# esq4/nind-denoise

Hardware: AMD Instinct MI355X
Metric: megapixels/sec denoised, UtNet cs=256 on 24 MP frames, 1/2/4/8 MI355X (higher is better)
Workload: dtype f32; 1 GPU; configs[1]: one 6000x4000 (24.0 MP) fp32 frame per step, f32 storage in the conv stack (fp32 accumulate), UtNet(funit=64,PReLU) random-init (seed 123), cs=264 (nearest valid to the named size; the reference rejects 256 / 512) ucs=200 ol=64 -> 1276 tiles/frame, tiles per conv-stack launch 256, crop->infer->stitch device resident (frame and canvas in HBM); every tile's input is the whole cs x cs cro; tiles_per_frame=1276, parallelism=single GPU

## Files before the change

### include/nind_hip.h

```cpp
#ifndef NIND_HIP_H
#define NIND_HIP_H

#include <stddef.h>
#include <stdint.h>

#ifdef __cplusplus
extern "C" {
#endif

typedef enum nd_status {
    ND_OK = 0,
    ND_EINVAL = -1,
    ND_ENOMEM = -2,
    ND_EHIP = -3
} nd_status;

typedef enum nd_act {
    ND_ACT_NONE = 0,
    ND_ACT_PRELU = 1,
    ND_ACT_ELU = 2,
    ND_ACT_HARDSWISH = 3
} nd_act;

typedef enum nd_layer_kind {
    ND_CONV3 = 0,
    ND_CONVT3 = 1,
    ND_CONVT2S2 = 2,
    ND_CONV1 = 3,
    ND_CONV2S2 = 4
} nd_layer_kind;

typedef enum nd_dtype {
    ND_F32 = 0,
    ND_BF16 = 1,
    ND_F16 = 2
} nd_dtype;

typedef enum nd_flags {
    ND_FLAG_NO_SPLITK = 1,
    ND_FLAG_DIRECT_CONV = 2,
    ND_FLAG_W1D_REGS = 4,
    ND_FLAG_UNFUSED_POOL = 16,
    ND_FLAG_TILE_ENCODER = 32,
    ND_FLAG_TILE_LEVEL2 = 64,
    ND_FLAG_FIND_NOISE = 128,
    ND_FLAG_TILE_SKIPS = 256,
    ND_FLAG_FULL_TILES = 8
} nd_flags;

int nd_version(void);
const char *nd_last_error(void);

int nd_tile_grid(int width, int height, int cs, int ucs, int ol, int *cols, int *rows, int *pad);
int nd_tile_geom(int i, int width, int height, int cs, int ucs, int ol,
                 int *x0, int *y0, int usefuldim[4], int usefulstart[2]);

int nd_tile_gather(const float *img_chw, int width, int height, int cs, int ucs, int ol,
                   int tile_begin, int tile_count, float *tiles_nchw, void *stream);
int nd_stitch_add(float *canvas_chw, int width, int height, int cs, int ucs, int ol,
                  const float *tiles_nchw, int tile_begin, int tile_count, void *stream);

int nd_utnet_num_tensors(void);
const char *nd_utnet_tensor_name(int idx);
size_t nd_utnet_packed_bytes(int funit, int dtype);
int nd_utnet_pack_weights(int funit, int dtype, const float *const *tensors, int n_tensors,
                          void *packed_host, size_t packed_bytes);

int nd_utnet_pack_weights_device(int funit, int dtype, const float *const *dev_tensors, int n_tensors, void *packed_dev,
                                 size_t packed_bytes, void *stream);

size_t nd_utnet_workspace_bytes_hw(int funit, int h, int w, int batch, int dtype);
int nd_utnet_workspace_init_hw(void *workspace, size_t workspace_bytes, int funit, int h, int w, int batch, int dtype,
                               void *stream);
int nd_utnet_forward_hw(int funit, int act, int dtype, int flags, const void *packed_dev,
                        const float *x_nchw, float *y_nchw, int batch, int h, int w,
                        void *workspace, size_t workspace_bytes, void *stream);

int nd_utnet_denoise_tiles(int funit, int act, int dtype, int flags, const void *packed_dev,
                           const float *img_chw, float *canvas_chw, int width, int height,
                           int cs, int ucs, int ol, int tile_begin, int tile_count, int batch,
                           void *workspace, size_t workspace_bytes, void *stream);

typedef void (*nd_progress_fn)(void *ctx, int n, int tile_begin, int tile_count);
size_t nd_utnet_frame_workspace_bytes(int funit, int dtype, int flags, int width, int height, int cs, int ucs, int ol, int batch);
int nd_utnet_denoise_frame(int funit, int act, int dtype, int flags, const void *packed_dev,
                           const float *img_chw, float *canvas_chw, int width, int height,
                           int cs, int ucs, int ol, int tile_begin, int tile_count, int batch,
                           void *workspace, size_t workspace_bytes, void *frame_ws, size_t frame_ws_bytes, void *stream,
                           nd_progress_fn progress, void *progress_ctx);
int nd_utnet_frame_plan(int funit, int dtype, int flags, int width, int height, int cs, int ucs, int ol, int *out);
int nd_utnet_frame_levels(int funit, int dtype, int flags, int width, int height, int cs, int ucs, int ol, int *levels);
int nd_utnet_frame_folds(int funit, int dtype, int flags, int width, int height, int cs, int ucs, int ol, int *mask);

typedef struct nd_step_profile {
    float ms;
    float ms_xform_in;
    float ms_gemm;
    float ms_xform_out;
    int form;
    int kind;
    double flops;
    double mfma_flops;
    double bytes;
    double xform_bytes_in;
    double xform_bytes_out;
} nd_step_profile;
int nd_utnet_profile_stack(int funit, int act, int dtype, int flags, const void *packed_dev, int batch, int cs, int crop,
                           void *workspace, size_t workspace_bytes, void *stream, nd_step_profile *steps, int max_steps);
const char *nd_utnet_step_name(int i);
int nd_utnet_useful_region(int funit, int cs, int crop, int step, int *rect);

int nd_unet_num_tensors(void);
const char *nd_unet_tensor_name(int idx);
size_t nd_unet_packed_bytes(int dtype);
int nd_unet_pack_weights(int dtype, const float *const *tensors, int n_tensors, void *packed_host, size_t packed_bytes);
size_t nd_unet_workspace_bytes(int h, int w, int batch, int dtype);
int nd_unet_workspace_init(void *workspace, size_t workspace_bytes, int h, int w, int batch, int dtype, void *stream);
int nd_unet_forward(int dtype, const void *packed_dev, const float *x_nchw, float *y_nchw, int batch, int h, int w,
                    void *workspace, size_t workspace_bytes, void *stream);

int nd_unet_pack_weights_device(int dtype, const float *const *dev_tensors, int n_tensors, void *packed_dev, size_t packed_bytes,
                                void *stream);

int nd_unet_num_steps(void);
const char *nd_unet_step_name(int i);
int nd_unet_useful_region(int cs, int crop, int step, int *rect);

int nd_unet_denoise_frame(int dtype, int flags, const void *packed_dev, const float *img_chw, float *canvas_chw, int width,
                          int height, int cs, int ucs, int ol, int tile_begin, int tile_count, int batch, void *workspace,
                          size_t workspace_bytes, void *stream, nd_progress_fn progress, void *progress_ctx);

double nd_utnet_flops(int funit, int cs);

size_t nd_layer_packed_bytes(int kind, int cin, int cout, int dtype);
int nd_layer_pack(int kind, int cin, int cout, int dtype, const float *weight, const float *bias,
                  void *packed_host, size_t packed_bytes);
size_t nd_layer_workspace_bytes(int kind, int batch, int cin, int cout, int h, int w, int dtype);
int nd_layer_forward(int kind, int act, float slope, int dtype, const void *packed_dev,
                     const float *x_nchw, int batch, int cin, int h, int w, int cout, float *y_nchw,
                     void *workspace, size_t workspace_bytes, int variant, int flags, void *stream);
int nd_maxpool2_forward(const float *x_nchw, int batch, int c, int h, int w, float *y_nchw,
                        void *workspace, size_t workspace_bytes, void *stream);

size_t nd_layer_wgrad_workspace_bytes(int kind, int batch, int cin, int cout, int h, int w);
int nd_layer_wgrad(int kind, const float *x_nchw, const float *dy_nchw, int batch, int cin, int h, int w, int cout,
                   float *dw, float *db, void *workspace, size_t workspace_bytes, void *stream);

size_t nd_utnet_param_count(int funit);
int nd_utnet_param_range(int funit, int tensor_idx, size_t *offset, size_t *count);
size_t nd_utnet_train_blob_bytes(int funit);
size_t nd_utnet_train_workspace_bytes_hw(int funit, int h, int w, int batch);
int nd_utnet_train_workspace_init_hw(void *workspace, size_t workspace_bytes, int funit, int h, int w, int batch, void *stream);
int nd_utnet_train_step_hw(int funit, int flags, const float *params, float *grads, void *blobs, const float *x_nchw,
                           const float *target_nchw, float *y_out_nchw, float w_l1, float w_mse, float w_ssim, float w_msssim,
                           float *loss_out, int batch, int h, int w, int loss_cs, void *workspace, size_t workspace_bytes,
                           void *stream, void *const *bucket_events, int n_events);
int nd_utnet_train_forward_hw(int funit, int act, int flags, const float *params, void *blobs, const float *x_nchw,
                              float *y_out_nchw, int batch, int h, int w, void *workspace, size_t workspace_bytes, void *stream);
int nd_utnet_train_backward_hw(int funit, int act, int flags, const float *params, float *grads, void *blobs, const float *gy_nchw,
                               float *dx_nchw, int batch, int h, int w, void *workspace, size_t workspace_bytes, void *stream,
                               void *const *bucket_events, int n_events);
int nd_utnet_grad_buckets(int funit, size_t *offsets, size_t *counts, int max);
int nd_adam_step(float *params, const float *grads, float *m, float *v, float *vmax, size_t n, float lr, float beta1,
                 float beta2, float eps, int step, int amsgrad, void *stream);

size_t nd_ssim_workspace_bytes(int n, int c, int h, int w);
int nd_ssim(const float *x, const float *y, int n, int c, int h, int w, float *out, void *workspace, size_t workspace_bytes,
            void *stream);
int nd_ms_ssim(const float *x, const float *y, int n, int c, int h, int w, float *out, void *workspace,
               size_t workspace_bytes, void *stream);
int nd_mse(const float *x, const float *y, size_t count, float *out, void *workspace, size_t workspace_bytes, void *stream);

size_t nd_ssim_loss_workspace_bytes(int n, int c, int h, int w);
int nd_ssim_loss_grad(const float *x, const float *y, int n, int c, int h, int w, int multiscale, float weight,
                      float *loss_acc, float *gx, int accumulate, void *workspace, size_t workspace_bytes, void *stream);

size_t nd_ssim_padded_workspace_bytes(int n, int c, int h, int w, int window);
int nd_ssim_padded(const float *x, const float *y, int n, int c, int h, int w, int window, float *out, void *workspace,
                   size_t workspace_bytes, void *stream);
int nd_ssim_padded_grad(const float *x, const float *y, int n, int c, int h, int w, int window, const float *gout, float *gx,
                        void *workspace, size_t workspace_bytes, void *stream);

size_t nd_winograd_packed_bytes(int tile, int cin, int cout);
int nd_winograd_pack(int tile, int kind, int cin, int cout, const float *w, const float *bias, void *packed,
                     size_t packed_bytes);
size_t nd_layer_winograd_workspace_bytes(int tile, int kind, int batch, int cin, int cout, int h, int w);
int nd_layer_forward_winograd(int tile, int kind, int act, float slope, const void *packed, const float *x, int batch,
                              int cin, int h, int w, int cout, float *y, void *workspace, size_t workspace_bytes, int flags,
                              void *stream);

int nd_conv_bench(int kind, int dtype, int batch, int cin, int cout, int h, int w, int variant, int iters,
                  void *workspace, size_t workspace_bytes, void *stream, float *mean_ms);

int nd_winograd_bench(int tile, int kind, int batch, int cin, int cout, int h, int w, int iters, void *workspace,
                      size_t workspace_bytes, void *stream, float *mean_ms);

int nd_num_conv_variants(void);
const char *nd_conv_variant_name(int variant);

#ifdef __cplusplus
}
#endif
#endif
```

### nind_denoise_amd/_lib.py

```python
import ctypes
import os
from ctypes import POINTER, c_char_p, c_double, c_float, c_int, c_size_t, c_void_p

_HERE = os.path.dirname(os.path.abspath(__file__))
LIB_PATH = os.path.join(_HERE, "libnind_hip.so")

ND_F32, ND_BF16, ND_F16 = 0, 1, 2
DTYPE = {"f32": 0, "fp32": 0, "float32": 0, "bf16": 1, "bfloat16": 1, "f16": 2, "fp16": 2, "float16": 2}
ACT = {"none": 0, "PReLU": 1, "ELU": 2, "Hardswish": 3}
KIND = {"conv3": 0, "convT3": 1, "convT2s2": 2, "conv1": 3, "conv2s2": 4}
FLAG_NO_SPLITK, FLAG_DIRECT_CONV, FLAG_W1D_REGS, FLAG_FULL_TILES, FLAG_UNFUSED_POOL, FLAG_TILE_ENCODER, FLAG_TILE_LEVEL2 = 1, 2, 4, 8, 16, 32, 64
FLAG_FIND_NOISE = 128
FLAG_TILE_SKIPS = 256
PROGRESS_FN = ctypes.CFUNCTYPE(None, c_void_p, c_int, c_int, c_int)


class StepProfile(ctypes.Structure):
    _fields_ = [("ms", c_float), ("ms_xform_in", c_float), ("ms_gemm", c_float), ("ms_xform_out", c_float),
                ("form", c_int), ("kind", c_int), ("flops", c_double), ("mfma_flops", c_double), ("bytes", c_double),
                ("xform_bytes_in", c_double), ("xform_bytes_out", c_double)]


FORM_NAMES = {-1: "pool", 0: "direct", 1: "w1d_f43", 2: "w1d_f23", 3: "wino3p_f6x6"}


class NindHipError(RuntimeError):
    pass


class NindHipMissing(ImportError):
    pass


_lib = None

_SIGNATURES = {
    "nd_version": (c_int, []),
    "nd_last_error": (c_char_p, []),
    "nd_tile_grid": (c_int, [c_int] * 5 + [POINTER(c_int)] * 3),
    "nd_tile_geom": (c_int, [c_int] * 6 + [POINTER(c_int)] * 4),
    "nd_tile_gather": (c_int, [c_void_p] + [c_int] * 7 + [c_void_p, c_void_p]),
    "nd_stitch_add": (c_int, [c_void_p] + [c_int] * 5 + [c_void_p, c_int, c_int, c_void_p]),
    "nd_utnet_num_tensors": (c_int, []),
    "nd_utnet_tensor_name": (c_char_p, [c_int]),
    "nd_utnet_packed_bytes": (c_size_t, [c_int, c_int]),
    "nd_utnet_pack_weights": (c_int, [c_int, c_int, POINTER(c_void_p), c_int, c_void_p, c_size_t]),
    "nd_utnet_pack_weights_device": (c_int, [c_int, c_int, POINTER(c_void_p), c_int, c_void_p, c_size_t, c_void_p]),
    "nd_utnet_workspace_bytes_hw": (c_size_t, [c_int] * 5),
    "nd_utnet_workspace_init_hw": (c_int, [c_void_p, c_size_t] + [c_int] * 5 + [c_void_p]),
    "nd_utnet_forward_hw": (c_int, [c_int] * 4 + [c_void_p] * 3 + [c_int, c_int, c_int, c_void_p, c_size_t, c_void_p]),
    "nd_utnet_denoise_tiles": (c_int, [c_int] * 4 + [c_void_p] * 3 + [c_int] * 8 + [c_void_p, c_size_t, c_void_p]),
    "nd_unet_num_tensors": (c_int, []),
    "nd_unet_tensor_name": (c_char_p, [c_int]),
    "nd_unet_packed_bytes": (c_size_t, [c_int]),
    "nd_unet_pack_weights": (c_int, [c_int, POINTER(c_void_p), c_int, c_void_p, c_size_t]),
    "nd_unet_workspace_bytes": (c_size_t, [c_int] * 4),
    "nd_unet_workspace_init": (c_int, [c_void_p, c_size_t] + [c_int] * 4 + [c_void_p]),
    "nd_unet_forward": (c_int, [c_int, c_void_p, c_void_p, c_void_p, c_int, c_int, c_int, c_void_p, c_size_t, c_void_p]),
    "nd_unet_pack_weights_device": (c_int, [c_int, POINTER(c_void_p), c_int, c_void_p, c_size_t, c_void_p]),
    "nd_unet_num_steps": (c_int, []),
    "nd_unet_step_name": (c_char_p, [c_int]),
    "nd_unet_useful_region": (c_int, [c_int, c_int, c_int, POINTER(c_int)]),
    "nd_unet_denoise_frame": (c_int, [c_int, c_int] + [c_void_p] * 3 + [c_int] * 8 + [c_void_p, c_size_t, c_void_p, PROGRESS_FN, c_void_p]),
    "nd_utnet_flops": (c_double, [c_int, c_int]),
    "nd_utnet_profile_stack": (c_int, [c_int] * 4 + [c_void_p, c_int, c_int, c_int, c_void_p, c_size_t, c_void_p, c_void_p, c_int]),
    "nd_utnet_step_name": (c_char_p, [c_int]),
    "nd_utnet_useful_region": (c_int, [c_int, c_int, c_int, c_int, POINTER(c_int)]),
    "nd_utnet_frame_workspace_bytes": (c_size_t, [c_int] * 9),
    "nd_utnet_frame_plan": (c_int, [c_int] * 8 + [POINTER(c_int)]),
    "nd_utnet_frame_levels": (c_int, [c_int] * 8 + [POINTER(c_int)]),
    "nd_utnet_frame_folds": (c_int, [c_int] * 8 + [POINTER(c_int)]),
    "nd_utnet_denoise_frame": (c_int, [c_int] * 4 + [c_void_p] * 3 + [c_int] * 8 + [c_void_p, c_size_t, c_void_p, c_size_t, c_void_p,
                                                                                    PROGRESS_FN, c_void_p]),
    "nd_layer_packed_bytes": (c_size_t, [c_int] * 4),
    "nd_layer_pack": (c_int, [c_int] * 4 + [c_void_p, c_void_p, c_void_p, c_size_t]),
    "nd_layer_workspace_bytes": (c_size_t, [c_int] * 7),
    "nd_layer_forward": (c_int, [c_int, c_int, c_float, c_int, c_void_p, c_void_p] + [c_int] * 5
                         + [c_void_p, c_void_p, c_size_t, c_int, c_int, c_void_p]),
    "nd_winograd_packed_bytes": (c_size_t, [c_int] * 3),
    "nd_winograd_pack": (c_int, [c_int] * 4 + [c_void_p, c_void_p, c_void_p, c_size_t]),
    "nd_layer_winograd_workspace_bytes": (c_size_t, [c_int] * 7),
    "nd_layer_forward_winograd": (c_int, [c_int, c_int, c_int, c_float, c_void_p, c_void_p] + [c_int] * 5
                                  + [c_void_p, c_void_p, c_size_t, c_int, c_void_p]),
    "nd_maxpool2_forward": (c_int, [c_void_p] + [c_int] * 4 + [c_void_p, c_void_p, c_size_t, c_void_p]),
    "nd_layer_wgrad_workspace_bytes": (c_size_t, [c_int] * 6),
    "nd_layer_wgrad": (c_int, [c_int, c_void_p, c_void_p] + [c_int] * 5 + [c_void_p, c_void_p, c_void_p, c_size_t, c_void_p]),
    "nd_utnet_param_count": (c_size_t, [c_int]),
    "nd_utnet_param_range": (c_int, [c_int, c_int, POINTER(c_size_t), POINTER(c_size_t)]),
    "nd_utnet_train_blob_bytes": (c_size_t, [c_int]),
    "nd_utnet_grad_buckets": (c_int, [c_int, POINTER(c_size_t), POINTER(c_size_t), c_int]),
    "nd_utnet_train_workspace_bytes_hw": (c_size_t, [c_int] * 4),
    "nd_utnet_train_workspace_init_hw": (c_int, [c_void_p, c_size_t, c_int, c_int, c_int, c_int, c_void_p]),
    "nd_utnet_train_forward_hw": (c_int, [c_int, c_int, c_int, c_void_p, c_void_p, c_void_p, c_void_p, c_int, c_int, c_int, c_void_p,
                                          c_size_t, c_void_p]),
    "nd_utnet_train_backward_hw": (c_int, [c_int, c_int, c_int, c_void_p, c_void_p, c_void_p, c_void_p, c_void_p, c_int, c_int, c_int,
                                           c_void_p, c_size_t, c_void_p, POINTER(c_void_p), c_int]),
    "nd_utnet_train_step_hw": (c_int, [c_int, c_int, c_void_p, c_void_p, c_void_p, c_void_p, c_void_p, c_void_p, c_float, c_float,
                                       c_float, c_float, c_void_p, c_int, c_int, c_int, c_int, c_void_p, c_size_t, c_void_p,
                                       POINTER(c_void_p), c_int]),
    "nd_adam_step": (c_int, [c_void_p] * 5 + [c_size_t, c_float, c_float, c_float, c_float, c_int, c_int, c_void_p]),
    "nd_ssim_workspace_bytes": (c_size_t, [c_int] * 4),
    "nd_ssim": (c_int, [c_void_p, c_void_p] + [c_int] * 4 + [c_void_p, c_void_p, c_size_t, c_void_p]),
    "nd_ms_ssim": (c_int, [c_void_p, c_void_p] + [c_int] * 4 + [c_void_p, c_void_p, c_size_t, c_void_p]),
    "nd_ssim_loss_workspace_bytes": (c_size_t, [c_int] * 4),
    "nd_ssim_loss_grad": (c_int, [c_void_p, c_void_p] + [c_int] * 5 + [c_float, c_void_p, c_void_p, c_int, c_void_p, c_size_t,
                                  c_void_p]),
    "nd_ssim_padded_workspace_bytes": (c_size_t, [c_int] * 5),
    "nd_ssim_padded": (c_int, [c_void_p, c_void_p] + [c_int] * 5 + [c_void_p, c_void_p, c_size_t, c_void_p]),
    "nd_ssim_padded_grad": (c_int, [c_void_p, c_void_p] + [c_int] * 5 + [c_void_p, c_void_p, c_void_p, c_size_t, c_void_p]),
    "nd_mse": (c_int, [c_void_p, c_void_p, c_size_t, c_void_p, c_void_p, c_size_t, c_void_p]),
    "nd_conv_bench": (c_int, [c_int] * 9 + [c_void_p, c_size_t, c_void_p, POINTER(c_float)]),
    "nd_winograd_bench": (c_int, [c_int] * 8 + [c_void_p, c_size_t, c_void_p, POINTER(c_float)]),
    "nd_num_conv_variants": (c_int, []),
    "nd_conv_variant_name": (c_char_p, [c_int]),
}

EXPORTS = tuple(_SIGNATURES)


def load():
    global _lib
    if _lib is not None:
        return _lib
    if not os.path.isfile(LIB_PATH):
        raise NindHipMissing(
            f"{LIB_PATH} not found: build it with `make -C nind_denoise_amd/csrc` (or __graft_entry__.build()). "
            "nind_denoise_amd has no CPU fallback for the denoise hot path.")
    import torch
    lib = ctypes.CDLL(LIB_PATH)
    for name, (res, args) in _SIGNATURES.items():
        fn = getattr(lib, name)
        fn.restype = res
        fn.argtypes = args
    _lib = lib
    return lib


def check(rc, what=""):
    if rc != 0:
        msg = load().nd_last_error().decode(errors="replace")
        exc = ValueError if rc == -1 else (MemoryError if rc == -2 else NindHipError)
        raise exc(f"{what}: {msg}" if what else msg)


def stream_ptr(device=None):
    import torch
    return c_void_p(torch.cuda.current_stream(device).cuda_stream)


def ptr(t):
    assert t.is_contiguous(), "tensor must be contiguous"
    return c_void_p(t.data_ptr())



def tile_grid(width, height, cs, ucs, ol):
    cols, rows, pad = c_int(), c_int(), c_int()
    check(load().nd_tile_grid(width, height, cs, ucs, ol, cols, rows, pad), "nd_tile_grid")
    return cols.value, rows.value, pad.value


def tile_geom(i, width, height, cs, ucs, ol):
    x0, y0 = c_int(), c_int()
    ud = (c_int * 4)()
    us = (c_int * 2)()
    check(load().nd_tile_geom(i, width, height, cs, ucs, ol, x0, y0, ud, us), "nd_tile_geom")
    return x0.value, y0.value, tuple(ud), tuple(us)


def utnet_tensor_names():
    lib = load()
    return [lib.nd_utnet_tensor_name(i).decode() for i in range(lib.nd_utnet_num_tensors())]
```

### nind_denoise_amd/csrc/nd_common.h

```cpp
#pragma once
#include <hip/hip_runtime.h>

#include <stdarg.h>
#include <stdint.h>
#include <stdio.h>

#include "nind_hip.h"

void nd_set_error(const char *fmt, ...);
#define ND_FAIL(code, ...)        \
    do {                          \
        nd_set_error(__VA_ARGS__); \
        return (code);            \
    } while (0)
#define ND_HIP(call)                                                                         \
    do {                                                                                     \
        hipError_t e_ = (call);                                                              \
        if (e_ != hipSuccess) ND_FAIL(ND_EHIP, "%s failed: %s", #call, hipGetErrorString(e_)); \
    } while (0)
#define ND_TRY(call)        \
    do {                    \
        int r_ = (call);    \
        if (r_ != 0) return r_; \
    } while (0)

static inline int nd_cpp(int dt) { return dt == ND_F32 ? 4 : 8; }
struct QpBuf {
    float *base;
    int planes;
    int B, Hb, Wb;
    int pad;
    long pstride;
    int dt = ND_F32;
    long np() const { return pstride; }
    long used() const { return (long)B * Hb * Wb; }
};

struct ConvDesc {
    int kind = ND_CONV3;
    int act = ND_ACT_NONE;
    float slope = 1.f;
    const float *slope_dev = nullptr;
    const float *wpk = nullptr;
    const float *bias = nullptr;
    int cin = 0, cout = 0;
    QpBuf in = {};
    QpBuf out = {};
    int out_plane0 = 0;
    int variant = -1;
    int in_plane0 = 0;
    float *pre = nullptr;
    long pre_plane = 0;
    float *part = nullptr;
    size_t part_bytes = 0;
    bool nosplit = false;
    int nbatch = 1;
    long in_bs = 0, out_bs = 0;
    size_t w_bs = 0;
    const QpBuf *pool = nullptr;
    int roi_r0 = 0, roi_c0 = 0, roi_rows = 0, roi_cols = 0;
    QpBuf in2 = {};
    int in2_plane0 = 0, in2_from = 0;
    const int *in2_origin = nullptr;
    long in2_origin_max = 0;
    int w_kb = 0, w_kb0 = 0;
    QpBuf add = {};
    int add_plane0 = 0;
    const int *add_origin = nullptr;
    long add_origin_max = 0;
};
int nd_check_in2(const char *who, const ConvDesc &d, int KB, long reach);
int nd_check_add(const char *who, const ConvDesc &d, long reach);
static const size_t kSplitScratchBytes = (size_t)512 * 64 * 1024 * 4;
int nd_launch_conv(const ConvDesc &d, hipStream_t stream);
bool nd_conv_pool_fits(const ConvDesc &d);
bool nd_conv_roi_fits(const ConvDesc &d);
int nd_conv_variant_count();
int nd_conv_variant_gemm(int cin, int cout);
size_t nd_wino_packed_floats(int T, int cin, int cout);
int nd_wino_pack(int T, int kind, int cin, int cout, const float *w, const float *bias, float *packed);
size_t nd_wino_scratch_bytes(int T, const QpBuf &in, int cin, int cout);
int nd_launch_conv_wino(int T, const ConvDesc &d, void *scratch, size_t scratch_bytes, hipStream_t s, hipEvent_t *ev2 = nullptr);
void nd_wino_xform_bytes(int T, const QpBuf &in, int cin, int cout, double *bytes_in, double *bytes_out);
size_t nd_w1d_packed_floats(int T, int cin, int cout);
int nd_w1d_pack(int T, int kind, int cin, int cout, const float *w, const float *bias, float *packed);
bool nd_w1d_fits(int T, const QpBuf &in);
int nd_launch_conv_w1d(int T, const ConvDesc &d, hipStream_t stream);
bool nd_w2d_ok(const QpBuf &in);
long nd_w2d_tiles(const QpBuf &in, int cout);
int nd_launch_conv_w2d(const ConvDesc &d, hipStream_t stream);
bool nd_f43_w2d(const QpBuf &in, int cout, bool pre, int flags);
int nd_launch_conv_f43(const ConvDesc &d, int flags, hipStream_t stream);
static inline size_t nd_buf_slack(int Wb) { return (size_t)10 * Wb + 8 + 2048; }
int nd_device(int *dev, int *ncus = nullptr);
int nd_raise_lds(int dev, const void *fn, size_t bytes);
int nd_once_per_device(int dev, int (*init)());
int nd_check_in_planes(const char *who, const ConvDesc &d, int KB, bool takes_in2 = false, bool takes_add = false);
int nd_check_out(const char *who, const ConvDesc &d, int oh, int ow, bool at_least);
int nd_check_int32(const char *who, const QpBuf &in);
int nd_check_roi(const char *who, const ConvDesc &d, int Hv, int Wv, bool refused, const char *why);
static inline int nd_check_flags(int flags, bool frame_loop = false, bool unet_frame = false) {
    const int known = ND_FLAG_NO_SPLITK | ND_FLAG_DIRECT_CONV | ND_FLAG_W1D_REGS | ND_FLAG_FULL_TILES | ND_FLAG_UNFUSED_POOL |
                      ND_FLAG_TILE_ENCODER | (frame_loop ? ND_FLAG_TILE_LEVEL2 | ND_FLAG_TILE_SKIPS : 0) | (unet_frame ? ND_FLAG_FIND_NOISE : 0);
    if (flags & ~known) ND_FAIL(ND_EINVAL, "unknown flag bits 0x%x", flags);
    return ND_OK;
}
const char *nd_conv_variant_label(int v);

static inline int nd_mtiles(int kind, int cout) {
    return kind == ND_CONVT2S2 ? (4 * cout + 255) / 256 * 8 : (cout + 127) / 128 * 4;
}
struct NdUpRow { int a, b, co; };
__host__ __device__ static inline NdUpRow nd_up_row(int m, int cout, int dt) {
    NdUpRow r;
    const int cpp = dt == ND_F32 ? 4 : 8, q = cout / cpp;
    const int G = m / (2 * cpp), e = m % cpp;
    r.b = (m / cpp) & 1;
    r.a = G / q;
    r.co = cpp * (G % q) + e;
    return r;
}
static inline int nd_taps(int kind) { return (kind == ND_CONV3 || kind == ND_CONVT3) ? 9 : (kind == ND_CONV2S2 ? 4 : 1); }
static inline int nd_kblocks(int cin, int dt = ND_F32) { return (cin + 2 * nd_cpp(dt) - 1) / (2 * nd_cpp(dt)); }
static inline size_t nd_bias_offset(int kind, int cin, int cout, int dt = ND_F32, int w1d_T = 0) {
    return (size_t)nd_mtiles(kind, cout) * nd_kblocks(cin, dt) * (w1d_T ? 3 * (w1d_T + 2) : nd_taps(kind)) * 256;
}
static inline size_t nd_packed_floats(int kind, int cin, int cout, int dt = ND_F32) {
    return nd_bias_offset(kind, cin, cout, dt) + (size_t)nd_mtiles(kind, cout) * 32;
}
void nd_pack_layer(int kind, int cin, int cout, int dt, const float *w, const float *bias, float *packed);

int nd_pack_layer_device(int kind, int cin, int cout, int dt, const float *w, const float *bias, float *packed, hipStream_t s,
                         const float *scale = nullptr);
int nd_launch_bn_fold(int cout, const float *b, const float *g, const float *be, const float *rm, const float *rv, float *scale,
                      float *fbias, hipStream_t s);
int nd_pack_w1d_device(int T, int kind, int cin, int cout, const float *w, const float *bias, float *packed, hipStream_t s);
int nd_pack_wino_device(int T, int kind, int cin, int cout, const float *w, const float *bias, float *packed, hipStream_t s);

int nd_launch_nchw_to_qp(const float *x, int C, const QpBuf &dst, int plane0, hipStream_t s);
int nd_launch_qp_to_nchw(const QpBuf &src, int plane0, float *y, int C, hipStream_t s);
int nd_launch_reflect_pack(const float *x_nchw, int B, int H, int W, const QpBuf &dst, hipStream_t s);
int nd_launch_maxpool2(const QpBuf &src, int src_plane0, int planes, const QpBuf &dst, hipStream_t s);
int nd_launch_final1x1(const QpBuf &src, int cin, const float *w, const float *bias, int crop, float *y_nchw, int H,
                       int W, hipStream_t s, int sigmoid = 0);
int nd_launch_final1x1_stitch(const QpBuf &src, int cin, const float *w, const float *bias, int crop, float *canvas,
                              int width, int height, int cs, int ucs, int ol, int tile_begin, int tile_count,
                              hipStream_t s, int sigmoid = 0, const float *noise_img = nullptr);
int nd_launch_gather_pack(const float *img, int width, int height, int cs, int ucs, int ol, int tile_begin,
                          int tile_count, const QpBuf &dst, hipStream_t s, int border = 2, bool reflect = true);
int nd_launch_gather_band(const float *img, int width, int height, int cs, int ucs, int ol, int band_row0, const QpBuf &dst,
                          hipStream_t s);
enum nd_edge_set { ND_EDGE_ROWS = 0, ND_EDGE_COLS = 1, ND_EDGE_CORNERS = 2 };
int nd_launch_gather_edges(const float *img, int width, int height, int cs, int ucs, int ol, int set, int first, int count,
                           const QpBuf &dst, hipStream_t s);
int nd_launch_skip_origins(const QpBuf &src, int dst_pad, int tile_begin, int tile_count, int cols, int band_rows, int step, long slot_elems,
                           int *table, long *origin_max, hipStream_t s);
struct SpliceMap {
    int step_y = 0, step_x = 0, img_t = 0, img_y = 0, img_x = 0, img_add = 0, oy = 0, ox = 0;
};
int nd_launch_splice(const QpBuf &src, int src_p0, const QpBuf &dst, int dst_p0, int planes, int tile_begin, int tile_count, int cols,
                     int row0, const SpliceMap &m, int r0, int r1, int c0, int c1, hipStream_t s, int band_rows = 0,
                     long slot_elems = 0, int dst_img0 = 0);
```

### nind_denoise_amd/csrc/pack.hip

```cpp
#include <string.h>

#include "nd_common.h"

static thread_local char g_err[512] = "";

void nd_set_error(const char *fmt, ...) {
    va_list ap;
    va_start(ap, fmt);
    vsnprintf(g_err, sizeof(g_err), fmt, ap);
    va_end(ap);
}

extern "C" const char *nd_last_error(void) { return g_err; }
extern "C" int nd_version(void) { return 111; }

static inline uint16_t f32_to_bf16_rne(float f) {
    uint32_t u;
    memcpy(&u, &f, 4);
    if ((u & 0x7fffffffu) > 0x7f800000u) return (uint16_t)((u >> 16) | 0x40);
    return (uint16_t)((u + 0x7fffu + ((u >> 16) & 1u)) >> 16);
}
static inline uint16_t f32_to_f16_rne(float f) {
    const _Float16 h = (_Float16)f;
    uint16_t u;
    memcpy(&u, &h, 2);
    return u;
}

void nd_pack_layer(int kind, int cin, int cout, int dt, const float *w, const float *bias, float *packed) {
    const int taps = nd_taps(kind);
    const int KB = nd_kblocks(cin, dt);
    const int MT = nd_mtiles(kind, cout);
    const int M = kind == ND_CONVT2S2 ? 4 * cout : cout;
    const int cpp = nd_cpp(dt);
    float *bp = packed + nd_bias_offset(kind, cin, cout, dt);
    auto weff = [&](int m, int ci, int t) -> float {
        if (m >= M || ci >= cin) return 0.f;
        switch (kind) {
            case ND_CONV3: return w[((size_t)m * cin + ci) * 9 + t];
            case ND_CONVT3: return w[((size_t)ci * cout + m) * 9 + (8 - t)];
            case ND_CONVT2S2: {
                const NdUpRow r = nd_up_row(m, cout, dt);
                return w[((size_t)ci * cout + r.co) * 4 + 2 * r.a + r.b];
            }
            case ND_CONV2S2: return w[((size_t)m * cin + ci) * 4 + t];
            default: return w[(size_t)m * cin + ci];
        }
    };
    for (int mt = 0; mt < MT; ++mt)
        for (int kb = 0; kb < KB; ++kb)
            for (int t = 0; t < taps; ++t) {
                float *dst = packed + (((size_t)mt * KB + kb) * taps + t) * 256;
                uint16_t *dst16 = (uint16_t *)dst;
                for (int lane = 0; lane < 64; ++lane) {
                    const int i = lane & 31, h = lane >> 5;
                    const int m = 32 * mt + i;
                    for (int s = 0; s < cpp; ++s) {
                        const float v = weff(m, 2 * cpp * kb + cpp * h + s, t);
                        if (dt == ND_F32)
                            dst[lane * 4 + s] = v;
                        else
                            dst16[lane * 8 + s] = dt == ND_BF16 ? f32_to_bf16_rne(v) : f32_to_f16_rne(v);
                    }
                }
            }
    for (int m = 0; m < MT * 32; ++m) {
        float v = 0.f;
        if (m < M && bias) v = bias[kind == ND_CONVT2S2 ? nd_up_row(m, cout, dt).co : m];
        bp[m] = v;
    }
}

extern "C" size_t nd_layer_packed_bytes(int kind, int cin, int cout, int dtype) {
    if (dtype < ND_F32 || dtype > ND_F16 || kind < 0 || kind > 4 || cin <= 0 || cout <= 0) return 0;
    return nd_packed_floats(kind, cin, cout, dtype) * sizeof(float);
}

extern "C" int nd_layer_pack(int kind, int cin, int cout, int dtype, const float *weight, const float *bias,
                             void *packed_host, size_t packed_bytes) {
    if (dtype < ND_F32 || dtype > ND_F16) ND_FAIL(ND_EINVAL, "nd_layer_pack: unsupported dtype %d", dtype);
    if (kind < 0 || kind > 4 || cin <= 0 || cout <= 0 || !weight || !packed_host)
        ND_FAIL(ND_EINVAL, "nd_layer_pack: bad arguments");
    if (packed_bytes < nd_layer_packed_bytes(kind, cin, cout, dtype))
        ND_FAIL(ND_ENOMEM, "nd_layer_pack: packed buffer too small");
    nd_pack_layer(kind, cin, cout, dtype, weight, bias, (float *)packed_host);
    return ND_OK;
}
```

### nind_denoise_amd/csrc/utnet.hip

```cpp
#include <string.h>

#include <string>
#include <vector>

#include "nd_common.h"

#include "utnet_net.h"

extern "C" int nd_utnet_num_tensors(void) { return (int)tensor_names().size(); }
extern "C" const char *nd_utnet_tensor_name(int idx) {
    const auto &n = tensor_names();
    return (idx >= 0 && idx < (int)n.size()) ? n[idx].c_str() : nullptr;
}

extern "C" size_t nd_utnet_packed_bytes(int funit, int dtype) {
    if (check_funit(funit, dtype) != ND_OK) return 0;
    return blob_layout(funit, dtype).total * sizeof(float);
}

extern "C" int nd_utnet_pack_weights(int funit, int dtype, const float *const *tensors, int n_tensors, void *packed_host,
                                     size_t packed_bytes) {
    ND_TRY(check_funit(funit, dtype));
    if (n_tensors != nd_utnet_num_tensors()) ND_FAIL(ND_EINVAL, "nd_utnet_pack_weights: expected %d tensors, got %d", nd_utnet_num_tensors(), n_tensors);
    const BlobLayout bl = blob_layout(funit, dtype);
    if (packed_bytes < bl.total * sizeof(float)) ND_FAIL(ND_ENOMEM, "nd_utnet_pack_weights: packed buffer too small");
    float *blob = (float *)packed_host;
    memset(blob, 0, bl.total * sizeof(float));
    for (int i = 0; i < kNumLayers; ++i) {
        const LayerSpec &l = kLayers[i];
        const int wi = tensor_index(std::string(l.key) + ".weight"), bi = tensor_index(std::string(l.key) + ".bias");
        if (wi < 0 || bi < 0 || !tensors[wi] || !tensors[bi]) ND_FAIL(ND_EINVAL, "nd_utnet_pack_weights: missing tensor %s.{weight,bias}", l.key);
        const int ci = lcin(l, funit), co = lcout(l, funit);
        if (i == kNumLayers - 1) {
            memcpy(blob + bl.off[i], tensors[wi], sizeof(float) * 3 * ci);
            memcpy(blob + bl.off[i] + 3 * ci, tensors[bi], sizeof(float) * 3);
        } else {
            nd_pack_layer(l.kind, ci, co, dtype, tensors[wi], tensors[bi], blob + bl.off[i]);
            if (bl.woff[i]) ND_TRY(nd_wino_pack(kWinoTile, l.kind, ci, co, tensors[wi], tensors[bi], blob + bl.woff[i]));
            if (bl.w1off[i]) ND_TRY(nd_w1d_pack(kW1dTile, l.kind, ci, co, tensors[wi], tensors[bi], blob + bl.w1off[i]));
            if (bl.w1off2[i]) ND_TRY(nd_w1d_pack(2, l.kind, ci, co, tensors[wi], tensors[bi], blob + bl.w1off2[i]));
        }
        if (l.prelu >= 0) {
            std::string k(l.key);
            const size_t dot = k.rfind('.');
            const std::string an = k.substr(0, dot + 1) + std::to_string(atoi(k.c_str() + dot + 1) + 1) + ".weight";
            const int ai = tensor_index(an);
            blob[l.prelu] = (ai >= 0 && tensors[ai]) ? tensors[ai][0] : 0.25f;
        }
    }
    return ND_OK;
}

extern "C" int nd_utnet_pack_weights_device(int funit, int dtype, const float *const *tensors, int n_tensors, void *packed_dev,
                                            size_t packed_bytes, void *stream) {
    ND_TRY(check_funit(funit, dtype));
    if (n_tensors != nd_utnet_num_tensors()) ND_FAIL(ND_EINVAL, "nd_utnet_pack_weights_device: expected %d tensors, got %d", nd_utnet_num_tensors(), n_tensors);
    const BlobLayout bl = blob_layout(funit, dtype);
    if (!packed_dev || packed_bytes < bl.total * sizeof(float)) ND_FAIL(ND_ENOMEM, "nd_utnet_pack_weights_device: packed buffer too small");
    hipStream_t s = (hipStream_t)stream;
    float *blob = (float *)packed_dev;
    ND_HIP(hipMemsetAsync(blob, 0, bl.total * sizeof(float), s));
    for (int i = 0; i < kNumLayers; ++i) {
        const LayerSpec &l = kLayers[i];
        const int wi = tensor_index(std::string(l.key) + ".weight"), bi = tensor_index(std::string(l.key) + ".bias");
        if (wi < 0 || bi < 0 || !tensors[wi] || !tensors[bi]) ND_FAIL(ND_EINVAL, "nd_utnet_pack_weights_device: missing tensor %s.{weight,bias}", l.key);
        const int ci = lcin(l, funit), co = lcout(l, funit);
        if (i == kNumLayers - 1) {
            ND_HIP(hipMemcpyAsync(blob + bl.off[i], tensors[wi], sizeof(float) * 3 * ci, hipMemcpyDeviceToDevice, s));
            ND_HIP(hipMemcpyAsync(blob + bl.off[i] + 3 * ci, tensors[bi], sizeof(float) * 3, hipMemcpyDeviceToDevice, s));
        } else {
            ND_TRY(nd_pack_layer_device(l.kind, ci, co, dtype, tensors[wi], tensors[bi], blob + bl.off[i], s));
            if (bl.woff[i]) ND_TRY(nd_pack_wino_device(kWinoTile, l.kind, ci, co, tensors[wi], tensors[bi], blob + bl.woff[i], s));
            if (bl.w1off[i]) ND_TRY(nd_pack_w1d_device(kW1dTile, l.kind, ci, co, tensors[wi], tensors[bi], blob + bl.w1off[i], s));
            if (bl.w1off2[i]) ND_TRY(nd_pack_w1d_device(2, l.kind, ci, co, tensors[wi], tensors[bi], blob + bl.w1off2[i], s));
        }
        if (l.prelu >= 0) {
            std::string k(l.key);
            const size_t dot = k.rfind('.');
            const std::string an = k.substr(0, dot + 1) + std::to_string(atoi(k.c_str() + dot + 1) + 1) + ".weight";
            const int ai = tensor_index(an);
            if (ai >= 0 && tensors[ai]) {
                ND_HIP(hipMemcpyAsync(blob + l.prelu, tensors[ai], sizeof(float), hipMemcpyDeviceToDevice, s));
            } else {
                const float dflt = 0.25f;
                ND_HIP(hipMemcpyAsync(blob + l.prelu, &dflt, sizeof(float), hipMemcpyHostToDevice, s));
                ND_HIP(hipStreamSynchronize(s));
            }
        }
    }
    return ND_OK;
}

extern "C" size_t nd_utnet_workspace_bytes_hw(int funit, int h, int w, int batch, int dtype) {
    if (check_net(funit, h, w, batch, dtype) != ND_OK) return 0;
    return make_plan(funit, h, w, batch, batch, nullptr, dtype).bytes;
}

extern "C" int nd_utnet_workspace_init_hw(void *ws, size_t ws_bytes, int funit, int h, int w, int batch, int dtype,
                                          void *stream) {
    ND_TRY(check_net(funit, h, w, batch, dtype));
    const size_t need = make_plan(funit, h, w, batch, batch, nullptr, dtype).bytes;
    if (!ws || ws_bytes < need) ND_FAIL(ND_ENOMEM, "UtNet workspace: %zu B given, %zu B needed", ws_bytes, need);
    ND_HIP(hipMemsetAsync(ws, 0, need, (hipStream_t)stream));
    return ND_OK;
}

static int forward_common(int funit, int act, int dtype, const void *packed, int batch_cap, int nimg, int h, int w,
                          void *ws, size_t ws_bytes, Plan *out_plan) {
    ND_TRY(check_net(funit, h, w, batch_cap, dtype));
    if (act < ND_ACT_PRELU || act > ND_ACT_HARDSWISH) ND_FAIL(ND_EINVAL, "UtNet: unknown activation %d", act);
    if (nimg <= 0 || nimg > batch_cap) ND_FAIL(ND_EINVAL, "UtNet: %d images with a workspace batch of %d", nimg, batch_cap);
    if (!packed || !ws) ND_FAIL(ND_EINVAL, "UtNet: null pointer");
    if (((uintptr_t)ws & 15) || ((uintptr_t)packed & 15)) ND_FAIL(ND_EINVAL, "UtNet: workspace / weights must be 16-byte aligned");
    *out_plan = make_plan(funit, h, w, batch_cap, nimg, (char *)ws, dtype);
    if (ws_bytes < out_plan->bytes) ND_FAIL(ND_ENOMEM, "UtNet workspace: %zu B given, %zu B needed", ws_bytes, out_plan->bytes);
    return ND_OK;
}

extern "C" int nd_utnet_forward_hw(int funit, int act, int dtype, int flags, const void *packed, const float *x, float *y,
                                   int batch, int h, int w, void *ws, size_t ws_bytes, void *stream) {
    ND_TRY(nd_check_flags(flags));
    Plan pl;
    ND_TRY(forward_common(funit, act, dtype, packed, batch, batch, h, w, ws, ws_bytes, &pl));
    if (!x || !y) ND_FAIL(ND_EINVAL, "UtNet: null tensor");
    hipStream_t s = (hipStream_t)stream;
    const float *blob = (const float *)packed;
    ND_TRY(nd_launch_reflect_pack(x, batch, h, w, pl.buf[X0], s));
    StackOpts o;
    o.flags = flags;
    ND_TRY(run_stack(funit, act, dtype, blob, pl, s, o));
    const BlobLayout bl = blob_layout(funit, dtype);
    const float *fw = blob + bl.off[kNumLayers - 1];
    ND_TRY(nd_launch_final1x1(pl.buf[T4B], funit, fw, fw + 3 * funit, 2, y, h, w, s));
    return ND_OK;
}

extern "C" int nd_utnet_denoise_tiles(int funit, int act, int dtype, int flags, const void *packed, const float *img,
                                      float *canvas, int width, int height, int cs, int ucs, int ol, int tile_begin,
                                      int tile_count, int batch, void *ws, size_t ws_bytes, void *stream) {
    ND_TRY(nd_check_flags(flags));
    Plan pl;
    ND_TRY(forward_common(funit, act, dtype, packed, batch, tile_count, cs, cs, ws, ws_bytes, &pl));
    if (!img || !canvas) ND_FAIL(ND_EINVAL, "UtNet: null image");
    hipStream_t s = (hipStream_t)stream;
    const float *blob = (const float *)packed;
    ND_TRY(nd_launch_gather_pack(img, width, height, cs, ucs, ol, tile_begin, tile_count, pl.buf[X0], s));
    const BlobLayout bl = blob_layout(funit, dtype);
    Roi rois[kNumSteps];
    StackOpts o;
    o.flags = flags;
    const int crop = (cs - ucs) / 2;
    if (!(flags & ND_FLAG_FULL_TILES) && plan_rois(pl, crop, crop, rois) && rois_supported(funit, dtype, flags, pl, bl, rois)) o.rois = rois;
    ND_TRY(run_stack(funit, act, dtype, blob, pl, s, o));
    const float *fw = blob + bl.off[kNumLayers - 1];
    ND_TRY(nd_launch_final1x1_stitch(pl.buf[T4B], funit, fw, fw + 3 * funit, 2, canvas, width, height, cs, ucs, ol,
                                     tile_begin, tile_count, s));
    return ND_OK;
}

extern "C" size_t nd_utnet_frame_workspace_bytes(int funit, int dtype, int flags, int width, int height, int cs, int ucs, int ol,
                                                 int batch) {
    FramePlan fp;
    if (nd_check_flags(flags, true) != ND_OK || frame_plan(funit, dtype, flags, width, height, cs, ucs, ol, batch, &fp) != ND_OK) return 0;
    return fp.bytes;
}

extern "C" int nd_utnet_frame_plan(int funit, int dtype, int flags, int width, int height, int cs, int ucs, int ol, int *out) {
    ND_TRY(nd_check_flags(flags, true));
    if (!out) ND_FAIL(ND_EINVAL, "nd_utnet_frame_plan: null output");
    FramePlan fp;
    ND_TRY(frame_plan(funit, dtype, flags, width, height, cs, ucs, ol, 1, &fp));
    const int v[8] = {fp.D, fp.aligned, fp.R, fp.nbands, fp.S, fp.cols, fp.rows, fp.hx};
    memcpy(out, v, sizeof(v));
    return ND_OK;
}

extern "C" int nd_utnet_frame_levels(int funit, int dtype, int flags, int width, int height, int cs, int ucs, int ol, int *levels) {
    ND_TRY(nd_check_flags(flags, true));
    if (!levels) ND_FAIL(ND_EINVAL, "nd_utnet_frame_levels: null output");
    FramePlan fp;
    ND_TRY(frame_plan(funit, dtype, flags, width, height, cs, ucs, ol, 1, &fp));
    *levels = fp.levels;
    return ND_OK;
}

extern "C" int nd_utnet_frame_folds(int funit, int dtype, int flags, int width, int height, int cs, int ucs, int ol, int *mask) {
    ND_TRY(nd_check_flags(flags, true));
    if (!mask) ND_FAIL(ND_EINVAL, "nd_utnet_frame_folds: null output");
    FramePlan fp;
    ND_TRY(frame_plan(funit, dtype, flags, width, height, cs, ucs, ol, 1, &fp));
    *mask = fp.folds;
    return ND_OK;
}

extern "C" int nd_utnet_denoise_frame(int funit, int act, int dtype, int flags, const void *packed, const float *img, float *canvas,
                                      int width, int height, int cs, int ucs, int ol, int tile_begin, int tile_count, int batch,
                                      void *ws, size_t ws_bytes, void *fws, size_t fws_bytes, void *stream, nd_progress_fn progress,
                                      void *progress_ctx) {
    ND_TRY(nd_check_flags(flags, true));
    FramePlan fp;
    ND_TRY(frame_plan(funit, dtype, flags, width, height, cs, ucs, ol, batch, &fp));
    if (tile_begin < 0 || tile_count < 0 || tile_begin + tile_count > fp.cols * fp.rows)
        ND_FAIL(ND_EINVAL, "nd_utnet_denoise_frame: tiles [%d,+%d) outside the grid of %d", tile_begin, tile_count, fp.cols * fp.rows);
    const int end = tile_begin + tile_count;
    Plan pl;
    ND_TRY(forward_common(funit, act, dtype, packed, batch, batch, cs, cs, ws, ws_bytes, &pl));
    const BlobLayout bl = blob_layout(funit, dtype);
    Roi rois[kNumSteps];
    const int crop = (cs - ucs) / 2;
    if (fp.D && !(plan_rois(pl, crop, crop, rois) && rois_supported(funit, dtype, flags, pl, bl, rois))) fp.D = 0;
    if (fp.D == 0) {
        int n = 0;
        for (int t0 = tile_begin; t0 < end; t0 += batch, ++n) {
            const int cnt = end - t0 < batch ? end - t0 : batch;
            if (progress) progress(progress_ctx, n, t0, cnt);
            ND_TRY(nd_utnet_denoise_tiles(funit, act, dtype, flags & ~(ND_FLAG_TILE_LEVEL2 | ND_FLAG_TILE_SKIPS), packed, img, canvas, width, height, cs, ucs, ol, t0, cnt, batch, ws,
                                          ws_bytes, stream));
        }
        return ND_OK;
    }
    if (!img || !canvas) ND_FAIL(ND_EINVAL, "UtNet: null image");
    if (!fws || fws_bytes < fp.bytes || ((uintptr_t)fws & 255))
        ND_FAIL(ND_ENOMEM, "nd_utnet_denoise_frame: frame workspace %zu B given, %zu B needed (256-byte aligned)", fws_bytes, fp.bytes);
    hipStream_t s = (hipStream_t)stream;
    const float *blob = (const float *)packed;
    const float *fw = blob + bl.off[kNumLayers - 1];
    char *const band_base = (char *)fws, *const rows_base = band_base + fp.band_bytes, *const cols_base = rows_base + fp.row_edge_bytes;
    char *const corner_base = cols_base + fp.col_edge_bytes;
    int *const origins = (int *)(corner_base + fp.corner_bytes);
    const bool l2 = fp.levels == 3;
    char *const l2_band_base = (char *)origins + 3 * fp.origin_bytes, *const l2_rows_base = l2_band_base + fp.l2_band_bytes;
    char *const l2_cols_base = l2_rows_base + fp.l2_row_bytes, *const l2_corner_base = l2_cols_base + fp.l2_col_bytes;
    char *const l2_wino = l2_corner_base + fp.l2_corner_bytes;
    const int f4 = funit / 4, cols = fp.cols, S = fp.S;
    const int n2 = enc_extent(cs + 4, P2), n3 = l2_extent(n2, P3);
    StackOpts enc, enc2, dec;
    enc.flags = enc2.flags = dec.flags = flags;
    enc.step_end = enc2.step_begin = kSharedSteps;
    enc2.step_end = kLevel2End;
    dec.step_begin = l2 ? kLevel2End : kSharedSteps;
    dec.rois = rois;
    auto l2_scratch = [&](Plan p) {
        p.split = pl.split;
        p.wino = l2_wino;
        p.wino_bytes = fp.l2_wino_bytes;
        return p;
    };
    struct Skip { Buf cat; int planes, step, tstep; const int *win; int *table; bool in_place, fold; Form form; } skips[3] = {
        {CAT4, f4, -1, S, fp.win4, origins, false, false, FORM_DIRECT},
        {CAT3, 2 * f4, -1, S / 2, fp.win3, origins + fp.origin_bytes / sizeof(int), false, false, FORM_DIRECT},
        {CAT2, 4 * f4, -1, S / 4, fp.win2, origins + 2 * fp.origin_bytes / sizeof(int), false, false, FORM_DIRECT}};
    char *const fold_wino = (char *)fws + fp.bytes - fp.fold_wino_bytes;
    const int nskips = l2 ? 3 : 2;
    for (int ki = 0; ki < 3; ++ki)
        for (int i = kSharedSteps; i < kNumSteps; ++i) {
            Skip &k = skips[ki];
            if (kSteps[i].layer >= 0 && kSteps[i].src == k.cat) {
                const Form form = step_form(kSteps[i], funit, dtype, flags, pl, bl);
                k.step = i;
                k.in_place = form_takes_src2(kSteps[i], form, funit, flags, pl);
                k.form = form;
                k.fold = ki < nskips && ((fp.folds >> ki) & 1) && k.in_place;
            }
        }
    StepSrc2 src2[3];
    dec.src2 = src2;
    const int per_band = fp.R * cols;
    const Plan bf = make_enc_plan(funit, fp.hx, fp.wx, 1, fp.hx, fp.wx, 1, band_base, dtype, fp.slots);
    const Plan bf2 = l2 ? l2_band_plan(fp, funit, dtype, fp.R, cs, l2_band_base) : Plan();
    int band_done = tile_begin / per_band - 1;
    for (int t0 = tile_begin, n = 0; t0 < end; ++n) {
        const int b0 = t0 / per_band;
        int cnt = end - t0 < batch ? end - t0 : batch;
        if (t0 + cnt > (b0 + 2) * per_band) cnt = (b0 + 2) * per_band - t0;
        for (int b = band_done + 1; b <= (t0 + cnt - 1) / per_band; ++b) {
            const int row0 = b * fp.R, nrows = fp.rows - row0 < fp.R ? fp.rows - row0 : fp.R;
            Plan bp = band_slot(make_enc_plan(funit, band_hx(fp, nrows, cs), fp.wx, 1, fp.hx, fp.wx, 1, band_base, dtype, fp.slots), b & 1, fp.slots);
            bp.split = pl.split;
            ND_TRY(nd_launch_gather_band(img, width, height, cs, ucs, ol, row0, bp.buf[X0], s));
            ND_TRY(run_stack(funit, act, dtype, blob, bp, s, enc));
            for (int ki = 0; ki < 2; ++ki)
                if (skips[ki].fold)
                    ND_TRY(launch_skip_fold(funit, flags, blob, bl, skips[ki].step, skips[ki].form, bp.buf[skips[ki].cat], skips[ki].planes,
                                            rois[skips[ki].step], skips[ki].tstep, nrows, cols, pl.split, fold_wino, fp.fold_wino_bytes, s));
            Plan re = band_slot(row_edge_plan(fp, funit, dtype, nrows, rows_base), b & 1, fp.slots, P2);
            Plan ce = band_slot(col_edge_plan(fp, funit, dtype, nrows, cs, cols_base), b & 1, fp.slots, P2);
            re.split = ce.split = pl.split;
            ND_TRY(nd_launch_gather_edges(img, width, height, cs, ucs, ol, ND_EDGE_ROWS, row0, nrows, re.buf[X0], s));
            ND_TRY(nd_launch_gather_edges(img, width, height, cs, ucs, ol, ND_EDGE_COLS, row0, nrows, ce.buf[X0], s));
            ND_TRY(run_stack(funit, act, dtype, blob, re, s, enc));
            ND_TRY(run_stack(funit, act, dtype, blob, ce, s, enc));
            if (l2) {
                Plan b2 = l2_scratch(l2_slot(l2_band_plan(fp, funit, dtype, nrows, cs, l2_band_base), b & 1, fp.slots));
                b2.buf[P2] = bp.buf[P2];
                ND_TRY(run_stack(funit, act, dtype, blob, b2, s, enc2));
                if (skips[2].fold)
                    ND_TRY(launch_skip_fold(funit, flags, blob, bl, skips[2].step, skips[2].form, b2.buf[CAT2], skips[2].planes, rois[skips[2].step],
                                            skips[2].tstep, nrows, cols, pl.split, fold_wino, fp.fold_wino_bytes, s));
                const Plan r2 = l2_scratch(l2_slot(l2_row_plan(fp, funit, dtype, nrows, l2_rows_base), b & 1, fp.slots, P3));
                const Plan c2 = l2_scratch(l2_slot(l2_col_plan(fp, funit, dtype, nrows, cs, l2_cols_base), b & 1, fp.slots, P3));
                const int h2 = bp.buf[P2].Hb, w2 = bp.buf[P2].Wb;
                for (int side = 0; side < 2; ++side) {
                    const int at = side * (kStrip2 - 1), in0 = 1 - side, in1 = kStrip2 - side;
                    SpliceMap br, lr, bc, lc;
                    br.step_y = bc.step_x = S / 4;
                    br.oy = bc.ox = side * (n2 - kStrip2);
                    lr.img_y = lc.img_x = 2;
                    lr.img_add = lc.img_add = side;
                    lr.oy = lc.ox = -at;
                    ND_TRY(nd_launch_splice(bp.buf[P2], 0, r2.buf[P2], 0, 2 * f4, 0, nrows, 1, 0, br, in0, in1, 0, w2, s, 0, 0, side * nrows));
                    ND_TRY(nd_launch_splice(re.buf[P2], 0, r2.buf[P2], 0, 2 * f4, 0, nrows, 1, 0, lr, at, at + 1, 0, w2, s, 0, 0, side * nrows));
                    ND_TRY(nd_launch_splice(bp.buf[P2], 0, c2.buf[P2], 0, 2 * f4, 0, cols, cols, 0, bc, 0, h2, in0, in1, s, 0, 0, side * cols));
                    ND_TRY(nd_launch_splice(ce.buf[P2], 0, c2.buf[P2], 0, 2 * f4, 0, cols, cols, 0, lc, 0, h2, at, at + 1, s, 0, 0, side * cols));
                }
                ND_TRY(run_stack(funit, act, dtype, blob, r2, s, enc2));
                ND_TRY(run_stack(funit, act, dtype, blob, c2, s, enc2));
            }
            band_done = b;
        }
        if (progress) progress(progress_ctx, n, t0, cnt);
        Plan cp = corner_plan(funit, dtype, cnt, batch, corner_base);
        cp.split = pl.split;
        ND_TRY(nd_launch_gather_edges(img, width, height, cs, ucs, ol, ND_EDGE_CORNERS, t0, cnt, cp.buf[X0], s));
        ND_TRY(run_stack(funit, act, dtype, blob, cp, s, enc));
        const Plan tp = make_plan(funit, cs, cs, batch, cnt, (char *)ws, dtype);
        dec.nsrc2 = 0;
        for (int ki = 0; ki < nskips; ++ki) {
            const Skip &k = skips[ki];
            const QpBuf &src = k.cat == CAT2 ? bf2.buf[k.cat] : bf.buf[k.cat];
            if (!k.in_place && !k.fold) {
                SpliceMap m;
                m.step_y = m.step_x = k.tstep;
                ND_TRY(nd_launch_splice(src, k.planes, tp.buf[k.cat], k.planes, k.planes, t0, cnt, cols, 0, m, k.win[0], k.win[1], k.win[0],
                                        k.win[1], s, fp.R, slot_elems(src, fp.slots)));
                continue;
            }
            StepSrc2 &q = src2[dec.nsrc2++];
            q.step = k.step;
            q.buf = src;
            q.plane0 = q.from = k.planes;
            q.addend = k.fold;
            if (k.fold) {
                q.plane0 = 0;
                q.buf.pad = 1;
            }
            q.origin = k.table;
            ND_TRY(nd_launch_skip_origins(src, tp.buf[k.cat].pad, t0, cnt, cols, fp.R, k.tstep, slot_elems(src, fp.slots), k.table,
                                          &q.origin_max, s));
        }
        SpliceMap whole;
        whole.step_y = whole.step_x = S / 4;
        ND_TRY(nd_launch_splice(bf.buf[P2], 0, tp.buf[P2], 0, 2 * f4, t0, cnt, cols, 0, whole, 0, n2, 0, n2, s, fp.R,
                                slot_elems(bf.buf[P2], fp.slots)));
        for (int b = b0; b <= (t0 + cnt - 1) / per_band; ++b) {
            const int lo = t0 > b * per_band ? t0 : b * per_band, hi = t0 + cnt < (b + 1) * per_band ? t0 + cnt : (b + 1) * per_band;
            const int row0 = b * fp.R, nrows = fp.rows - row0 < fp.R ? fp.rows - row0 : fp.R;
            const QpBuf rl = band_slot(row_edge_plan(fp, funit, dtype, nrows, rows_base), b & 1, fp.slots, P2).buf[P2];
            const QpBuf cl = band_slot(col_edge_plan(fp, funit, dtype, nrows, cs, cols_base), b & 1, fp.slots, P2).buf[P2];
            for (int side = 0; side < 2; ++side) {
                const int at = side * (n2 - 1);
                SpliceMap mr, mc;
                mr.step_x = mc.step_y = S / 4;
                mr.img_y = mc.img_x = 2;
                mr.img_add = mc.img_add = side;
                mr.oy = mc.ox = -at;
                ND_TRY(nd_launch_splice(rl, 0, tp.buf[P2], 0, 2 * f4, lo, hi - lo, cols, row0, mr, at, at + 1, 0, n2, s, 0, 0, lo - t0));
                ND_TRY(nd_launch_splice(cl, 0, tp.buf[P2], 0, 2 * f4, lo, hi - lo, cols, row0, mc, 0, n2, at, at + 1, s, 0, 0, lo - t0));
            }
        }
        for (int k = 0; k < 4; ++k) {
            const int r = (k >> 1) * (n2 - 1), c = (k & 1) * (n2 - 1);
            SpliceMap m;
            m.img_t = 4;
            m.img_add = k;
            m.oy = -r;
            m.ox = -c;
            ND_TRY(nd_launch_splice(cp.buf[P2], 0, tp.buf[P2], 0, 2 * f4, t0, cnt, cols, 0, m, r, r + 1, c, c + 1, s));
        }
        if (l2) {
            const Plan k2 = l2_scratch(l2_corner_plan(funit, dtype, cnt, batch, l2_corner_base));
            for (int k = 0; k < 4; ++k) {
                SpliceMap m;
                m.img_t = 1;
                m.oy = (k >> 1) * (n2 - kStrip2);
                m.ox = (k & 1) * (n2 - kStrip2);
                ND_TRY(nd_launch_splice(tp.buf[P2], 0, k2.buf[P2], 0, 2 * f4, 0, cnt, cnt, 0, m, 0, kStrip2, 0, kStrip2, s, 0, 0, k * cnt));
            }
            ND_TRY(run_stack(funit, act, dtype, blob, k2, s, enc2));
            SpliceMap whole3;
            whole3.step_y = whole3.step_x = S / 8;
            ND_TRY(nd_launch_splice(bf2.buf[P3], 0, tp.buf[P3], 0, 4 * f4, t0, cnt, cols, 0, whole3, 0, n3, 0, n3, s, fp.R,
                                    slot_elems(bf2.buf[P3], fp.slots)));
            for (int b = b0; b <= (t0 + cnt - 1) / per_band; ++b) {
                const int lo = t0 > b * per_band ? t0 : b * per_band, hi = t0 + cnt < (b + 1) * per_band ? t0 + cnt : (b + 1) * per_band;
                const int row0 = b * fp.R, nrows = fp.rows - row0 < fp.R ? fp.rows - row0 : fp.R;
                const QpBuf rl = l2_slot(l2_row_plan(fp, funit, dtype, nrows, l2_rows_base), b & 1, fp.slots, P3).buf[P3];
                const QpBuf cl = l2_slot(l2_col_plan(fp, funit, dtype, nrows, cs, l2_cols_base), b & 1, fp.slots, P3).buf[P3];
                for (int side = 0; side < 2; ++side) {
                    const int at = side * (n3 - 1);
                    SpliceMap mr, mc;
                    mr.step_x = mc.step_y = S / 8;
                    mr.img_y = mc.img_x = 1;
                    mr.img_add = side * nrows;
                    mc.img_add = side * cols;
                    mr.oy = mc.ox = -at;
                    ND_TRY(nd_launch_splice(rl, 0, tp.buf[P3], 0, 4 * f4, lo, hi - lo, cols, row0, mr, at, at + 1, 0, n3, s, 0, 0, lo - t0));
                    ND_TRY(nd_launch_splice(cl, 0, tp.buf[P3], 0, 4 * f4, lo, hi - lo, cols, row0, mc, 0, n3, at, at + 1, s, 0, 0, lo - t0));
                }
            }
            for (int k = 0; k < 4; ++k) {
                const int r = (k >> 1) * (n3 - 1), c = (k & 1) * (n3 - 1);
                SpliceMap m;
                m.img_t = 1;
                m.img_add = k * cnt;
                m.oy = -r;
                m.ox = -c;
                ND_TRY(nd_launch_splice(k2.buf[P3], 0, tp.buf[P3], 0, 4 * f4, t0, cnt, cols, 0, m, r, r + 1, c, c + 1, s));
            }
        }
        ND_TRY(run_stack(funit, act, dtype, blob, tp, s, dec));
        ND_TRY(nd_launch_final1x1_stitch(tp.buf[T4B], funit, fw, fw + 3 * funit, 2, canvas, width, height, cs, ucs, ol, t0, cnt, s));
        t0 += cnt;
    }
    return ND_OK;
}

namespace {
template <int N>
struct Events {
    hipEvent_t ev[N];
    int n = 0;
    int create() {
        for (; n < N; ++n) ND_HIP(hipEventCreate(&ev[n]));
        return ND_OK;
    }
    ~Events() { for (int i = 0; i < n; ++i) (void)hipEventDestroy(ev[i]); }
};
}

extern "C" int nd_utnet_profile_stack(int funit, int act, int dtype, int flags, const void *packed, int batch, int cs, int crop,
                                      void *ws, size_t ws_bytes, void *stream, nd_step_profile *steps, int max_steps) {
    ND_TRY(nd_check_flags(flags));
    Plan pl;
    ND_TRY(forward_common(funit, act, dtype, packed, batch, batch, cs, cs, ws, ws_bytes, &pl));
    if (max_steps < kNumSteps || !steps) ND_FAIL(ND_EINVAL, "nd_utnet_profile_stack: need room for %d steps", kNumSteps);
    if (crop < 0 || 2 * crop >= cs) ND_FAIL(ND_EINVAL, "nd_utnet_profile_stack: crop %d", crop);
    hipStream_t s = (hipStream_t)stream;
    Events<kNumSteps + 1 + 2 * kNumSteps> evs;
    ND_TRY(evs.create());
    hipEvent_t *const ev = evs.ev, *const evx = evs.ev + kNumSteps + 1;
    const BlobLayout bl = blob_layout(funit, dtype);
    Roi rois[kNumSteps];
    StackOpts opts;
    opts.flags = flags;
    opts.ev = ev;
    opts.ev_x = evx;
    if (!(flags & ND_FLAG_FULL_TILES) && plan_rois(pl, crop, crop, rois) && rois_supported(funit, dtype, flags, pl, bl, rois)) opts.rois = rois;
    int rc = run_stack(funit, act, dtype, (const float *)packed, pl, s, opts);
    if (rc == ND_OK) {
        hipError_t e = hipStreamSynchronize(s);
        if (e != hipSuccess) {
            nd_set_error("hipStreamSynchronize failed: %s", hipGetErrorString(e));
            rc = ND_EHIP;
        }
    }
    for (int i = 0; i < kNumSteps && rc == ND_OK; ++i) {
        nd_step_profile &o = steps[i];
        memset(&o, 0, sizeof(o));
        if (hipEventElapsedTime(&o.ms, ev[i], ev[i + 1]) != hipSuccess) {
            nd_set_error("hipEventElapsedTime failed");
            rc = ND_EHIP;
            break;
        }
        const Step &st = kSteps[i];
        const Form form = step_form(st, funit, dtype, flags, pl, bl);
        o.form = (int)form;
        o.kind = st.layer >= 0 ? kLayers[st.layer].kind : -1;
        const QpBuf &in = pl.buf[st.src], &out = pl.buf[st.dst];
        const double B = batch, esz = 16.0 / nd_cpp(dtype);
        double hin = in.Hb - 2 * in.pad, win = in.Wb - 2 * in.pad;
        if (opts.rois && opts.rois[i].rows > 0) {
            const bool t3 = kLayers[st.layer].kind == ND_CONVT3;
            hin = opts.rois[i].rows - (t3 ? 2 : 0);
            win = opts.rois[i].cols - (t3 ? 2 : 0);
        }
        if (st.layer < 0) {
            const double c = st.dst_plane0_mul * funit;
            o.bytes = B * c * esz * (hin * win + (hin / 2) * (win / 2));
            continue;
        }
        const LayerSpec &l = kLayers[st.layer];
        const double ci = lcin(l, funit), co = lcout(l, funit);
        const double cip = nd_kblocks((int)ci, dtype) * 2.0 * nd_cpp(dtype);
        double hout, wout;
        switch (l.kind) {
            case ND_CONV3: hout = hin - 2; wout = win - 2; o.flops = 2.0 * hout * wout * ci * co * 9; break;
            case ND_CONVT3: hout = hin + 2; wout = win + 2; o.flops = 2.0 * hin * win * ci * co * 9; break;
            case ND_CONVT2S2: hout = 2 * hin; wout = 2 * win; o.flops = 2.0 * hin * win * ci * co * 4; break;
            default: hout = hin; wout = win; o.flops = 2.0 * hin * win * ci * co; break;
        }
        o.flops *= B;
        o.bytes = B * esz * (ci * hin * win + co * hout * wout) + 4.0 * ci * co * nd_taps(l.kind);
        auto cdiv = [](double a, double b) { return (double)(long)((a + b - 1) / b); };
        switch (form) {
            case FORM_W1D4: o.mfma_flops = 2.0 * 3 * 6 * cip * co * hout * cdiv(wout, 4) * B; break;
            case FORM_W1D2: o.mfma_flops = 2.0 * 3 * 4 * cip * co * hout * cdiv(wout, 2) * B; break;
            case FORM_WINO3P: o.mfma_flops = 2.0 * (kWinoTile + 2) * (kWinoTile + 2) * cip * co * cdiv(hout, kWinoTile) * cdiv(wout, kWinoTile) * B; break;
            default:
                o.mfma_flops = l.kind == ND_CONVT2S2 ? 2.0 * 4 * cip * co * hin * win * B
                                                     : 2.0 * nd_taps(l.kind) * cip * co * hout * wout * B;
                break;
        }
        if (form == FORM_WINO3P && batch <= kWinoChunk) {
            float a = 0, b = 0, c = 0;
            if (hipEventElapsedTime(&a, ev[i], evx[2 * i]) == hipSuccess && hipEventElapsedTime(&b, evx[2 * i], evx[2 * i + 1]) == hipSuccess &&
                hipEventElapsedTime(&c, evx[2 * i + 1], ev[i + 1]) == hipSuccess) {
                o.ms_xform_in = a;
                o.ms_gemm = b;
                o.ms_xform_out = c;
            }
            QpBuf v = in;
            if (opts.rois && opts.rois[i].rows > 0) {
                v.Hb = opts.rois[i].rows + 2;
                v.Wb = opts.rois[i].cols + 2;
            }
            nd_wino_xform_bytes(kWinoTile, v, (int)ci, (int)co, &o.xform_bytes_in, &o.xform_bytes_out);
        }
    }
    return rc;
}

extern "C" int nd_utnet_useful_region(int funit, int cs, int crop, int step, int *rect) {
    if (!valid_cs(cs) || funit <= 0 || step < 0 || step >= kNumSteps || !rect || crop < 0 || 2 * crop >= cs)
        ND_FAIL(ND_EINVAL, "nd_utnet_useful_region: bad arguments");
    const Plan pl = make_plan(funit, cs, cs, 1, 1, nullptr, ND_F32);
    Roi rois[kNumSteps];
    plan_rois(pl, crop, crop, rois);
    int n = 0;
    for (int i = 0; i < kNumSteps; ++i) n += rois[i].rows > 0;
    rect[0] = rois[step].r0;
    rect[1] = rois[step].c0;
    rect[2] = rois[step].rows;
    rect[3] = rois[step].cols;
    return n;
}

extern "C" const char *nd_utnet_step_name(int i) {
    if (i < 0 || i >= kNumSteps) return nullptr;
    return kSteps[i].layer >= 0 ? kLayers[kSteps[i].layer].key : "maxpool";
}

extern "C" double nd_utnet_flops(int funit, int cs) {
    if (!valid_cs(cs) || funit <= 0) return 0.0;
    const double f = funit;
    double mac = 0;
    int h = cs + 4;
    const double ch[4][2] = {{3, f}, {f, 2 * f}, {2 * f, 4 * f}, {4 * f, 8 * f}};
    for (int i = 0; i < 4; ++i) {
        mac += (double)(h - 2) * (h - 2) * ch[i][0] * ch[i][1] * 9;
        mac += (double)(h - 4) * (h - 4) * ch[i][1] * ch[i][1] * 9;
        h = (h - 4) / 2;
    }
    mac += (double)(h - 2) * (h - 2) * 8 * f * 16 * f * 9;
    mac += (double)(h - 2) * (h - 2) * 16 * f * 16 * f * 9;
    double c = 16 * f;
    for (int i = 0; i < 4; ++i) {
        mac += (double)h * h * c * (c / 2) * 4;
        h *= 2;
        mac += (double)h * h * c * (c / 2) * 9;
        mac += (double)(h + 2) * (h + 2) * (c / 2) * (c / 2) * 9;
        h += 4;
        c /= 2;
    }
    mac += (double)h * h * f * 3;
    return 2 * mac;
}

namespace {
struct LayerPlan {
    QpBuf in, out;
    float *split;
    size_t bytes;
};
LayerPlan layer_plan(int kind, int B, int cin, int cout, int h, int w, char *base, int dt = ND_F32) {
    LayerPlan p;
    const int ipad = kind == ND_CONVT3 ? 2 : 0;
    p.in.dt = p.out.dt = dt;
    p.in.planes = 2 * nd_kblocks(cin, dt);
    p.in.B = B;
    p.in.Hb = h + 2 * ipad;
    p.in.Wb = w + 2 * ipad;
    p.in.pad = ipad;
    p.in.pstride = (long)B * p.in.Hb * p.in.Wb;
    p.in.base = (float *)base;
    size_t off = ((size_t)p.in.planes * p.in.pstride + nd_buf_slack(p.in.Wb)) * 16;
    off = (off + 255) & ~(size_t)255;
    int oh, ow;
    switch (kind) {
        case ND_CONV3: oh = h - 2; ow = w - 2; break;
        case ND_CONVT3: oh = h + 2; ow = w + 2; break;
        case ND_CONVT2S2: oh = 2 * h; ow = 2 * w; break;
        case ND_CONV2S2: oh = h / 2; ow = w / 2; break;
        default: oh = h; ow = w; break;
    }
    p.out.planes = (cout + nd_cpp(dt) - 1) / nd_cpp(dt);
    p.out.B = B;
    p.out.Hb = oh;
    p.out.Wb = ow;
    p.out.pad = 0;
    p.out.pstride = (long)B * oh * ow;
    p.out.base = (float *)(base + off);
    off += ((size_t)p.out.planes * p.out.pstride + 64) * 16;
    off = (off + 255) & ~(size_t)255;
    p.split = (float *)(base + off);
    off += kSplitScratchBytes;
    p.bytes = off;
    return p;
}

enum LayerFamily { LF_NONE, LF_DIRECT, LF_W1D, LF_W2D, LF_WINO3P };
struct LayerForm {
    LayerFamily fam;
    int T;
};
constexpr LayerForm kDirect = {LF_DIRECT, 0};
LayerForm wino_form(int tile) {
    if (tile < 1 || tile > 6) return {LF_NONE, 0};
    if (tile == 5) return {LF_W2D, 4};
    return (tile & 1) ? LayerForm{LF_W1D, tile + 1} : LayerForm{LF_WINO3P, tile};
}
size_t wino_packed_floats(const LayerForm &fm, int cin, int cout) {
    return fm.fam == LF_WINO3P ? nd_wino_packed_floats(fm.T, cin, cout) : nd_w1d_packed_floats(fm.T, cin, cout);
}

ConvDesc layer_desc(const LayerForm &fm, int kind, int cin, int cout, int dt, const float *wpk, const LayerPlan &pl) {
    ConvDesc d;
    d.kind = kind;
    d.cin = cin;
    d.cout = cout;
    d.wpk = wpk;
    if (fm.fam != LF_WINO3P) d.bias = wpk + nd_bias_offset(kind, cin, cout, dt, fm.T);
    d.in = pl.in;
    d.out = pl.out;
    d.part = pl.split;
    d.part_bytes = kSplitScratchBytes;
    return d;
}
int launch_form(const LayerForm &fm, const ConvDesc &d, void *scratch, size_t scratch_bytes, hipStream_t s) {
    switch (fm.fam) {
        case LF_W1D: return nd_launch_conv_w1d(fm.T, d, s);
        case LF_W2D: return nd_launch_conv_w2d(d, s);
        case LF_WINO3P: return nd_launch_conv_wino(fm.T, d, scratch, scratch_bytes, s);
        default: return nd_launch_conv(d, s);
    }
}

int layer_forward(const LayerForm &fm, int kind, int act, float slope, int dt, const void *packed, const float *x, int batch,
                  int cin, int h, int w, int cout, float *y, void *ws, size_t ws_bytes, int variant, int flags, hipStream_t s) {
    const LayerPlan pl = layer_plan(kind, batch, cin, cout, h, w, (char *)ws, dt);
    ND_HIP(hipMemsetAsync(ws, 0, pl.bytes, s));
    ND_TRY(nd_launch_nchw_to_qp(x, cin, pl.in, 0, s));
    ConvDesc d = layer_desc(fm, kind, cin, cout, dt, (const float *)packed, pl);
    d.act = act;
    d.slope = slope;
    d.variant = variant;
    d.nosplit = (flags & ND_FLAG_NO_SPLITK) != 0;
    ND_TRY(launch_form(fm, d, (char *)ws + pl.bytes, ws_bytes - pl.bytes, s));
    return nd_launch_qp_to_nchw(pl.out, 0, y, cout, s);
}
}

extern "C" size_t nd_layer_workspace_bytes(int kind, int batch, int cin, int cout, int h, int w, int dtype) {
    if (dtype < ND_F32 || dtype > ND_F16 || kind < 0 || kind > 4 || batch <= 0 || cin <= 0 || cout <= 0 || h <= 0 || w <= 0) return 0;
    if (kind == ND_CONV3 && (h < 3 || w < 3)) return 0;
    return layer_plan(kind, batch, cin, cout, h, w, nullptr, dtype).bytes;
}

extern "C" int nd_layer_forward(int kind, int act, float slope, int dtype, const void *packed, const float *x, int batch,
                                int cin, int h, int w, int cout, float *y, void *ws, size_t ws_bytes, int variant, int flags,
                                void *stream) {
    ND_TRY(nd_check_flags(flags));
    if (dtype < ND_F32 || dtype > ND_F16) ND_FAIL(ND_EINVAL, "nd_layer_forward: unsupported dtype %d", dtype);
    const size_t need = nd_layer_workspace_bytes(kind, batch, cin, cout, h, w, dtype);
    if (!need) ND_FAIL(ND_EINVAL, "nd_layer_forward: bad shape");
    if (!ws || ws_bytes < need) ND_FAIL(ND_ENOMEM, "nd_layer_forward: workspace %zu B given, %zu B needed", ws_bytes, need);
    if (cout % nd_cpp(dtype)) ND_FAIL(ND_EINVAL, "nd_layer_forward: cout must be a multiple of %d", nd_cpp(dtype));
    return layer_forward(kDirect, kind, act, slope, dtype, packed, x, batch, cin, h, w, cout, y, ws, ws_bytes, variant, flags,
                         (hipStream_t)stream);
}

extern "C" size_t nd_winograd_packed_bytes(int tile, int cin, int cout) {
    const LayerForm fm = wino_form(tile);
    if (fm.fam == LF_NONE || cin <= 0 || cout <= 0) return 0;
    return wino_packed_floats(fm, cin, cout) * sizeof(float);
}
extern "C" int nd_winograd_pack(int tile, int kind, int cin, int cout, const float *w, const float *bias, void *packed,
                                size_t packed_bytes) {
    const size_t need = nd_winograd_packed_bytes(tile, cin, cout);
    if (!need) ND_FAIL(ND_EINVAL, "nd_winograd_pack: bad shape");
    if (!packed || packed_bytes < need) ND_FAIL(ND_ENOMEM, "nd_winograd_pack: %zu B given, %zu B needed", packed_bytes, need);
    const LayerForm fm = wino_form(tile);
    if (fm.fam == LF_WINO3P) return nd_wino_pack(fm.T, kind, cin, cout, w, bias, (float *)packed);
    return nd_w1d_pack(fm.T, kind, cin, cout, w, bias, (float *)packed);
}
extern "C" size_t nd_layer_winograd_workspace_bytes(int tile, int kind, int batch, int cin, int cout, int h, int w) {
    const LayerForm fm = wino_form(tile);
    if (fm.fam == LF_NONE || (kind != ND_CONV3 && kind != ND_CONVT3)) return 0;
    const size_t base = nd_layer_workspace_bytes(kind, batch, cin, cout, h, w, ND_F32);
    if (!base || fm.fam != LF_WINO3P) return base;
    const LayerPlan pl = layer_plan(kind, batch, cin, cout, h, w, nullptr, ND_F32);
    return base + nd_wino_scratch_bytes(fm.T, pl.in, cin, cout);
}
extern "C" int nd_layer_forward_winograd(int tile, int kind, int act, float slope, const void *packed, const float *x, int batch,
                                         int cin, int h, int w, int cout, float *y, void *ws, size_t ws_bytes, int flags,
                                         void *stream) {
    ND_TRY(nd_check_flags(flags));
    const size_t need = nd_layer_winograd_workspace_bytes(tile, kind, batch, cin, cout, h, w);
    if (!need) ND_FAIL(ND_EINVAL, "nd_layer_forward_winograd: bad shape / kind / tile");
    if (!ws || ws_bytes < need) ND_FAIL(ND_ENOMEM, "nd_layer_forward_winograd: workspace %zu B given, %zu B needed", ws_bytes, need);
    return layer_forward(wino_form(tile), kind, act, slope, ND_F32, packed, x, batch, cin, h, w, cout, y, ws, ws_bytes, -1, flags,
                         (hipStream_t)stream);
}

extern "C" int nd_maxpool2_forward(const float *x, int batch, int c, int h, int w, float *y, void *ws, size_t ws_bytes,
                                   void *stream) {
    if (batch <= 0 || c <= 0 || h < 2 || w < 2) ND_FAIL(ND_EINVAL, "nd_maxpool2_forward: bad shape");
    QpBuf in, out;
    in.planes = out.planes = (c + 3) / 4;
    in.B = out.B = batch;
    in.Hb = h; in.Wb = w; in.pad = 0; in.pstride = (long)batch * h * w;
    out.Hb = h / 2; out.Wb = w / 2; out.pad = 0; out.pstride = (long)batch * (h / 2) * (w / 2);
    const size_t ib = ((size_t)in.planes * in.pstride * 16 + 255) & ~(size_t)255;
    const size_t need = ib + (size_t)out.planes * out.pstride * 16;
    if (!ws || ws_bytes < need) ND_FAIL(ND_ENOMEM, "nd_maxpool2_forward: workspace %zu B given, %zu B needed", ws_bytes, need);
    in.base = (float *)ws;
    out.base = (float *)((char *)ws + ib);
    hipStream_t s = (hipStream_t)stream;
    ND_TRY(nd_launch_nchw_to_qp(x, c, in, 0, s));
    ND_TRY(nd_launch_maxpool2(in, 0, in.planes, out, s));
    ND_TRY(nd_launch_qp_to_nchw(out, 0, y, c, s));
    return ND_OK;
}

__global__ void k_fill_random(float *p, size_t n, unsigned seed) {
    size_t i = (size_t)blockIdx.x * blockDim.x + threadIdx.x;
    const size_t stride = (size_t)gridDim.x * blockDim.x;
    for (; i < n; i += stride) {
        unsigned h = (unsigned)i * 2654435761u ^ seed;
        h ^= h >> 15; h *= 2246822519u; h ^= h >> 13;
        p[i] = ((h & 0xFFFF) - 32768.f) * (1.f / 65536.f);
    }
}

__global__ void k_fill_random16(unsigned short *p, size_t n, unsigned seed, int dt) {
    size_t i = (size_t)blockIdx.x * blockDim.x + threadIdx.x;
    const size_t stride = (size_t)gridDim.x * blockDim.x;
    for (; i < n; i += stride) {
        unsigned h = (unsigned)i * 2654435761u ^ seed;
        h ^= h >> 15; h *= 2246822519u; h ^= h >> 13;
        const float f = ((h & 0xFFFF) - 32768.f) * (1.f / 65536.f);
        if (dt == ND_BF16) {
            const __bf16 v = (__bf16)f;
            p[i] = *(const unsigned short *)&v;
        } else {
            const _Float16 v = (_Float16)f;
            p[i] = *(const unsigned short *)&v;
        }
    }
}

namespace {
void fill_random(void *ws, size_t bytes, float *wpk, size_t wfloats, int dt, int kind, int cin, int cout, hipStream_t s) {
    if (dt == ND_F32) {
        hipLaunchKernelGGL(k_fill_random, dim3(2048), dim3(256), 0, s, (float *)ws, bytes / 4, 12345u);
        hipLaunchKernelGGL(k_fill_random, dim3(1024), dim3(256), 0, s, wpk, wfloats, 777u);
        return;
    }
    hipLaunchKernelGGL(k_fill_random16, dim3(2048), dim3(256), 0, s, (unsigned short *)ws, bytes / 2, 12345u, dt);
    hipLaunchKernelGGL(k_fill_random16, dim3(1024), dim3(256), 0, s, (unsigned short *)wpk, wfloats * 2, 777u, dt);
    hipLaunchKernelGGL(k_fill_random, dim3(64), dim3(256), 0, s, wpk + nd_bias_offset(kind, cin, cout, dt), (size_t)nd_mtiles(kind, cout) * 32, 99u);
}

int time_form(const char *what, const LayerForm &fm, const ConvDesc &d, void *scratch, size_t scratch_bytes, int iters,
              hipStream_t s, float *mean_ms) {
    ND_TRY(launch_form(fm, d, scratch, scratch_bytes, s));
    Events<2> ev;
    ND_TRY(ev.create());
    ND_HIP(hipEventRecord(ev.ev[0], s));
    int rc = ND_OK;
    for (int i = 0; i < iters && rc == ND_OK; ++i) rc = launch_form(fm, d, scratch, scratch_bytes, s);
    (void)hipEventRecord(ev.ev[1], s);
    if (hipStreamSynchronize(s) != hipSuccess && rc == ND_OK) {
        nd_set_error("%s: stream failed", what);
        rc = ND_EHIP;
    }
    float ms = 0;
    (void)hipEventElapsedTime(&ms, ev.ev[0], ev.ev[1]);
    if (mean_ms) *mean_ms = ms / (iters > 0 ? iters : 1);
    return rc;
}
}

extern "C" int nd_conv_bench(int kind, int dtype, int batch, int cin, int cout, int h, int w, int variant, int iters, void *ws,
                             size_t ws_bytes, void *stream, float *mean_ms) {
    const size_t need = nd_layer_workspace_bytes(kind, batch, cin, cout, h, w, dtype);
    if (!need) ND_FAIL(ND_EINVAL, "nd_conv_bench: bad shape");
    const size_t wfloats = nd_packed_floats(kind, cin, cout, dtype);
    const size_t total = need + ((wfloats * 4 + 255) & ~(size_t)255);
    if (!ws || ws_bytes < total) ND_FAIL(ND_ENOMEM, "nd_conv_bench: workspace %zu B given, %zu B needed", ws_bytes, total);
    hipStream_t s = (hipStream_t)stream;
    LayerPlan pl = layer_plan(kind, batch, cin, cout, h, w, (char *)ws, dtype);
    float *wpk = (float *)((char *)ws + need);
    fill_random(ws, need, wpk, wfloats, dtype, kind, cin, cout, s);
    ConvDesc d = layer_desc(kDirect, kind, cin, cout, dtype, wpk, pl);
    d.act = ND_ACT_PRELU;
    d.slope = 0.2f;
    d.variant = variant;
    return time_form("nd_conv_bench", kDirect, d, nullptr, 0, iters, s, mean_ms);
}

extern "C" int nd_num_conv_variants(void) { return nd_conv_variant_count(); }
extern "C" const char *nd_conv_variant_name(int v) { return nd_conv_variant_label(v); }

extern "C" int nd_winograd_bench(int tile, int kind, int batch, int cin, int cout, int h, int w, int iters, void *ws,
                                 size_t ws_bytes, void *stream, float *mean_ms) {
    const size_t need = nd_layer_winograd_workspace_bytes(tile, kind, batch, cin, cout, h, w);
    if (!need) ND_FAIL(ND_EINVAL, "nd_winograd_bench: bad shape / kind / tile");
    const LayerForm fm = wino_form(tile);
    const size_t wfloats = wino_packed_floats(fm, cin, cout);
    const size_t total = ((need + 255) & ~(size_t)255) + wfloats * 4;
    if (!ws || ws_bytes < total) ND_FAIL(ND_ENOMEM, "nd_winograd_bench: workspace %zu B given, %zu B needed", ws_bytes, total);
    hipStream_t s = (hipStream_t)stream;
    LayerPlan pl = layer_plan(kind, batch, cin, cout, h, w, (char *)ws, ND_F32);
    float *wpk = (float *)((char *)ws + ((need + 255) & ~(size_t)255));
    fill_random(ws, pl.bytes, wpk, wfloats, ND_F32, kind, cin, cout, s);
    ConvDesc d = layer_desc(fm, kind, cin, cout, ND_F32, wpk, pl);
    d.act = ND_ACT_PRELU;
    d.slope = 0.2f;
    return time_form("nd_winograd_bench", fm, d, (char *)ws + pl.bytes, need - pl.bytes, iters, s, mean_ms);
}
```

### nind_denoise_amd/csrc/utnet_net.h

```cpp
#pragma once
#include <string.h>

#include <string>
#include <vector>

#include "nd_common.h"

namespace {

struct LayerSpec {
    const char *key;
    int kind;
    int cin_mul, cout_mul;
    int prelu;
};

const LayerSpec kLayers[] = {
    {"convs1.0", ND_CONV3, 0, 1, 0},    {"convs1.2", ND_CONV3, 1, 1, 1},    {"convs2.0", ND_CONV3, 1, 2, 2},
    {"convs2.2", ND_CONV3, 2, 2, 3},    {"convs3.0", ND_CONV3, 2, 4, 4},    {"convs3.2", ND_CONV3, 4, 4, 5},
    {"convs4.0", ND_CONV3, 4, 8, 6},    {"convs4.2", ND_CONV3, 8, 8, 7},    {"bottom.0", ND_CONV3, 8, 16, 8},
    {"bottom.2", ND_CONVT3, 16, 16, 9}, {"up1", ND_CONVT2S2, 16, 8, -1},    {"tconvs1.0", ND_CONVT3, 16, 8, 10},
    {"tconvs1.2", ND_CONVT3, 8, 8, 11}, {"up2", ND_CONVT2S2, 8, 4, -1},     {"tconvs2.0", ND_CONVT3, 8, 4, 12},
    {"tconvs2.2", ND_CONVT3, 4, 4, 13}, {"up3", ND_CONVT2S2, 4, 2, -1},     {"tconvs3.0", ND_CONVT3, 4, 2, 14},
    {"tconvs3.2", ND_CONVT3, 2, 2, 15}, {"up4", ND_CONVT2S2, 2, 1, -1},     {"tconvs4.0", ND_CONVT3, 2, 1, 16},
    {"tconvs4.2", ND_CONVT3, 1, 1, 17}, {"tconvs4.4", ND_CONV1, 1, 0, -1},
};
constexpr int kNumLayers = (int)(sizeof(kLayers) / sizeof(kLayers[0]));
constexpr int kNumSlopes = 18;
constexpr int kHeaderFloats = 32;

std::vector<std::string> build_tensor_names() {
    std::vector<std::string> n;
    auto seq = [&](const std::string &p, int n_act_pairs, bool final1x1) {
        for (int k = 0; k < n_act_pairs; ++k) {
            n.push_back(p + "." + std::to_string(2 * k) + ".weight");
            n.push_back(p + "." + std::to_string(2 * k) + ".bias");
            n.push_back(p + "." + std::to_string(2 * k + 1) + ".weight");
        }
        if (final1x1) {
            n.push_back(p + ".4.weight");
            n.push_back(p + ".4.bias");
        }
    };
    for (int i = 1; i <= 4; ++i) seq("convs" + std::to_string(i), 2, false);
    seq("bottom", 2, false);
    for (int i = 1; i <= 4; ++i) {
        n.push_back("up" + std::to_string(i) + ".weight");
        n.push_back("up" + std::to_string(i) + ".bias");
        seq("tconvs" + std::to_string(i), 2, i == 4);
    }
    return n;
}
const std::vector<std::string> &tensor_names() {
    static const std::vector<std::string> n = build_tensor_names();
    return n;
}
int tensor_index(const std::string &name) {
    const auto &n = tensor_names();
    for (size_t i = 0; i < n.size(); ++i)
        if (n[i] == name) return (int)i;
    return -1;
}

inline int lcin(const LayerSpec &l, int f) { return l.cin_mul ? l.cin_mul * f : 3; }
inline int lcout(const LayerSpec &l, int f) { return l.cout_mul ? l.cout_mul * f : 3; }

constexpr int kWinoTile = 6;
constexpr int kW1dTile = 4;
constexpr int kWinoChunk = 256;
inline bool wino_layer(const LayerSpec &l, int f, int dt) {
    return dt == ND_F32 && (l.kind == ND_CONV3 || l.kind == ND_CONVT3) && l.cin_mul * f >= 128 && l.cout_mul * f >= 128 &&
           ((long)l.cin_mul * f * l.cout_mul * f >= 128L * 256 || l.kind == ND_CONVT3) && (l.cin_mul * f) % 16 == 0;
}

struct BlobLayout {
    size_t off[kNumLayers];
    size_t woff[kNumLayers];
    size_t w1off[kNumLayers];
    size_t w1off2[kNumLayers];
    size_t total;
};
inline size_t layer_floats(const LayerSpec &l, int f, int dt, bool train) {
    const size_t direct = nd_packed_floats(l.kind, lcin(l, f), lcout(l, f), dt);
    if (!train || dt != ND_F32 || (l.kind != ND_CONV3 && l.kind != ND_CONVT3)) return direct;
    const size_t w1 = nd_w1d_packed_floats(kW1dTile, lcin(l, f), lcout(l, f));
    return w1 > direct ? w1 : direct;
}
BlobLayout blob_layout(int f, int dt, bool train = false) {
    BlobLayout b;
    size_t o = kHeaderFloats;
    for (int i = 0; i < kNumLayers; ++i) {
        b.off[i] = o;
        const LayerSpec &l = kLayers[i];
        if (i == kNumLayers - 1)
            o += ((size_t)3 * lcin(l, f) + 3 + 3) / 4 * 4;
        else
            o += layer_floats(l, f, dt, train);
    }
    for (int i = 0; i < kNumLayers; ++i) {
        b.woff[i] = 0;
        if (!train && wino_layer(kLayers[i], f, dt)) {
            b.woff[i] = o;
            o += (nd_wino_packed_floats(kWinoTile, lcin(kLayers[i], f), lcout(kLayers[i], f)) + 63) / 64 * 64;
        }
        b.w1off[i] = b.w1off2[i] = 0;
        const LayerSpec &l = kLayers[i];
        if (!train && dt == ND_F32 && (l.kind == ND_CONV3 || l.kind == ND_CONVT3) && !b.woff[i]) {
            b.w1off[i] = o;
            o += (nd_w1d_packed_floats(kW1dTile, lcin(l, f), lcout(l, f)) + 63) / 64 * 64;
            b.w1off2[i] = o;
            o += (nd_w1d_packed_floats(2, lcin(l, f), lcout(l, f)) + 63) / 64 * 64;
        }
    }
    b.total = o;
    return b;
}

bool valid_cs(int cs) { return cs >= 104 && (cs - 56) % 16 == 0; }

int check_funit(int funit, int dtype) {
    if (dtype < ND_F32 || dtype > ND_F16) ND_FAIL(ND_EINVAL, "UtNet: unsupported dtype %d", dtype);
    const int q = 2 * nd_cpp(dtype);
    if (funit < q || funit % q) ND_FAIL(ND_EINVAL, "UtNet: funit=%d must be a positive multiple of %d for dtype %d", funit, q, dtype);
    return ND_OK;
}

int check_net(int funit, int h, int w, int batch, int dtype) {
    ND_TRY(check_funit(funit, dtype));
    for (int cs : {h, w})
        if (!valid_cs(cs))
            ND_FAIL(ND_EINVAL, "UtNet: tile size %d is not of the form 16k+56 (104, 120, ..., 248, 264, ..., 504, 520); "
                               "the reference network rejects it too (sizes of the skip concats do not match)", cs);
    if (batch <= 0) ND_FAIL(ND_EINVAL, "UtNet: batch=%d", batch);
    return ND_OK;
}

enum Buf { X0, A1, CAT4, P1, A2, CAT3, P2, A3, CAT2, P3, A4, CAT1, P4, BT0, BT1, T1A, T1B, T2A, T2B, T3A, T3B, T4A, T4B, NBUF };

struct Step {
    int layer;
    Buf src, dst;
    int dst_plane0_mul;
};
constexpr int kNumSteps = 26;
const Step kSteps[kNumSteps] = {
    {0, X0, A1, 0},     {1, A1, CAT4, 1},   {-1, CAT4, P1, 1},  {2, P1, A2, 0},    {3, A2, CAT3, 2},  {-1, CAT3, P2, 2},
    {4, P2, A3, 0},     {5, A3, CAT2, 4},   {-1, CAT2, P3, 4},  {6, P3, A4, 0},    {7, A4, CAT1, 8},  {-1, CAT1, P4, 8},
    {8, P4, BT0, 0},    {9, BT0, BT1, 0},   {10, BT1, CAT1, 0}, {11, CAT1, T1A, 0}, {12, T1A, T1B, 0}, {13, T1B, CAT2, 0},
    {14, CAT2, T2A, 0}, {15, T2A, T2B, 0},  {16, T2B, CAT3, 0}, {17, CAT3, T3A, 0}, {18, T3A, T3B, 0}, {19, T3B, CAT4, 0},
    {20, CAT4, T4A, 0}, {21, T4A, T4B, 0},
};

struct Plan {
    QpBuf buf[NBUF];
    float *split;
    char *wino;
    size_t wino_bytes;
    size_t bytes;
};

Plan make_plan(int f, int ch_, int cw_, int cap, int nimg, char *base, int dt) {
    Plan p;
    size_t off = 0;
    auto chain = [](int cs, int which) {
        const int l1 = cs, l2 = cs / 2 - 4, l3 = l2 / 2 - 4, l4 = l3 / 2 - 4, p4 = l4 / 2;
        const int v[] = {cs + 4, cs + 2, l1, l1 / 2, l1 / 2 - 2, l2, l2 / 2, l2 / 2 - 2, l3, l3 / 2, l3 / 2 - 2, l4, p4,
                         p4 - 2, p4, l4 + 2, l4 + 4, l3 + 2, l3 + 4, l2 + 2, l2 + 4, l1 + 2, l1 + 4};
        return v[which];
    };
    auto add = [&](Buf id, int ch, int , int pad) {
        QpBuf &q = p.buf[id];
        q.planes = (ch + nd_cpp(dt) - 1) / nd_cpp(dt);
        if (id == X0) q.planes = 2;
        q.dt = dt;
        q.B = nimg;
        q.Hb = chain(ch_, (int)id) + 2 * pad;
        q.Wb = chain(cw_, (int)id) + 2 * pad;
        q.pad = pad;
        q.pstride = (long)cap * q.Hb * q.Wb;
        q.base = (float *)(base + off);
        const size_t slack = nd_buf_slack(q.Wb);
        off += ((size_t)q.planes * q.pstride + slack) * 16;
        off = (off + 255) & ~(size_t)255;
    };
    const int cs = ch_;
    const int l1 = cs, l2 = cs / 2 - 4, l3 = l2 / 2 - 4, l4 = l3 / 2 - 4, p4 = l4 / 2;
    add(X0, 8, cs + 4, 0);
    add(A1, f, cs + 2, 0);
    add(CAT4, 2 * f, l1, 2);
    add(P1, f, l1 / 2, 0);
    add(A2, 2 * f, l1 / 2 - 2, 0);
    add(CAT3, 4 * f, l2, 2);
    add(P2, 2 * f, l2 / 2, 0);
    add(A3, 4 * f, l2 / 2 - 2, 0);
    add(CAT2, 8 * f, l3, 2);
    add(P3, 4 * f, l3 / 2, 0);
    add(A4, 8 * f, l3 / 2 - 2, 0);
    add(CAT1, 16 * f, l4, 2);
    add(P4, 8 * f, p4, 0);
    add(BT0, 16 * f, p4 - 2, 2);
    add(BT1, 16 * f, p4, 0);
    add(T1A, 8 * f, l4 + 2, 2);
    add(T1B, 8 * f, l4 + 4, 0);
    add(T2A, 4 * f, l3 + 2, 2);
    add(T2B, 4 * f, l3 + 4, 0);
    add(T3A, 2 * f, l2 + 2, 2);
    add(T3B, 2 * f, l2 + 4, 0);
    add(T4A, f, l1 + 2, 2);
    add(T4B, f, l1 + 4, 0);
    p.split = (float *)(base + off);
    off += kSplitScratchBytes;
    p.wino = base + off;
    p.wino_bytes = 0;
    for (const Step &st : kSteps) {
        if (st.layer < 0 || !wino_layer(kLayers[st.layer], f, dt)) continue;
        QpBuf v = p.buf[st.src];
        v.B = cap < kWinoChunk ? cap : kWinoChunk;
        const size_t need = nd_wino_scratch_bytes(kWinoTile, v, lcin(kLayers[st.layer], f), lcout(kLayers[st.layer], f));
        if (need > p.wino_bytes) p.wino_bytes = need;
    }
    off += (p.wino_bytes + 255) & ~(size_t)255;
    p.bytes = off;
    return p;
}

enum Form { FORM_POOL = -1, FORM_DIRECT = 0, FORM_W1D4 = 1, FORM_W1D2 = 2, FORM_WINO3P = 3 };
inline Form step_form(const Step &st, int f, int dt, int flags, const Plan &pl, const BlobLayout &bl,
                      const unsigned char *train_w1 = nullptr) {
    if (st.layer < 0) return FORM_POOL;
    const LayerSpec &l = kLayers[st.layer];
    if (l.kind != ND_CONV3 && l.kind != ND_CONVT3) return FORM_DIRECT;
    if (train_w1) return train_w1[st.layer] ? FORM_W1D4 : FORM_DIRECT;
    if (flags & ND_FLAG_DIRECT_CONV) return FORM_DIRECT;
    if (bl.w1off[st.layer]) {
        if (nd_f43_w2d(pl.buf[st.src], lcout(l, f), false, flags)) return FORM_W1D4;
        if (nd_w1d_fits(kW1dTile, pl.buf[st.src])) return FORM_W1D4;
        if (nd_w1d_fits(2, pl.buf[st.src])) return FORM_W1D2;
        return FORM_DIRECT;
    }
    return bl.woff[st.layer] ? FORM_WINO3P : FORM_DIRECT;
}

struct Roi { int r0, c0, rows, cols; };
inline bool plan_rois(const Plan &pl, int crop_h, int crop_w, Roi *roi) {
    for (int i = 0; i < kNumSteps; ++i) roi[i] = Roi{0, 0, 0, 0};
    if (crop_h <= 0 && crop_w <= 0) return false;
    bool any = false;
    int lo[2][NBUF], hi[2][NBUF];
    for (int dim = 0; dim < 2; ++dim) {
        for (int b = 0; b < NBUF; ++b) {
            lo[dim][b] = 1 << 30;
            hi[dim][b] = -1;
        }
        const QpBuf &last = pl.buf[T4B];
        const int size = (dim ? last.Wb : last.Hb) - 2 * last.pad, crop = dim ? crop_w : crop_h;
        lo[dim][T4B] = crop + 2;
        hi[dim][T4B] = size - 2 - crop;
        for (int i = kNumSteps - 1; i >= 0; --i) {
            const Step &st = kSteps[i];
            if (st.layer < 0) continue;
            const int kind = kLayers[st.layer].kind;
            if (kind != ND_CONVT3 && kind != ND_CONVT2S2) continue;
            if (hi[dim][st.dst] < 0) continue;
            const QpBuf &src = pl.buf[st.src];
            const int si = (dim ? src.Wb : src.Hb) - 2 * src.pad;
            int a = lo[dim][st.dst], b = hi[dim][st.dst];
            if (kind == ND_CONVT3) {
                a = a - 2 < 0 ? 0 : a - 2;
                b = b > si ? si : b;
            } else {
                a = a >> 1;
                b = (b + 1) >> 1;
                b = b > si ? si : b;
            }
            if (a < lo[dim][st.src]) lo[dim][st.src] = a;
            if (b > hi[dim][st.src]) hi[dim][st.src] = b;
        }
    }
    for (int i = 0; i < kNumSteps; ++i) {
        const Step &st = kSteps[i];
        if (st.layer < 0) continue;
        const int kind = kLayers[st.layer].kind;
        if (kind != ND_CONVT3 && kind != ND_CONVT2S2) continue;
        const Buf b = kind == ND_CONVT3 ? st.dst : st.src;
        const QpBuf &q = pl.buf[b];
        const int H = q.Hb - 2 * q.pad, W = q.Wb - 2 * q.pad;
        int r0 = 0, r1 = H, c0 = 0, c1 = W;
        if (kind == ND_CONVT3) {
            if (hi[0][b] >= 0) { r0 = lo[0][b]; r1 = hi[0][b]; }
            if (hi[1][b] >= 0) { c0 = lo[1][b]; c1 = hi[1][b]; }
        } else {
            if (hi[0][st.dst] >= 0) { r0 = lo[0][st.dst] >> 1; r1 = (hi[0][st.dst] + 1) >> 1; }
            if (hi[1][st.dst] >= 0) { c0 = lo[1][st.dst] >> 1; c1 = (hi[1][st.dst] + 1) >> 1; }
        }
        r0 = r0 < 0 ? 0 : r0; c0 = c0 < 0 ? 0 : c0;
        r1 = r1 > H ? H : r1; c1 = c1 > W ? W : c1;
        if (r0 == 0 && c0 == 0 && r1 == H && c1 == W) continue;
        if (r1 <= r0 || c1 <= c0) continue;
        roi[i] = Roi{r0, c0, r1 - r0, c1 - c0};
        any = true;
    }
    return any;
}

inline bool rois_supported(int f, int dt, int flags, const Plan &pl, const BlobLayout &bl, const Roi *rois) {
    for (int i = 0; i < kNumSteps; ++i) {
        if (rois[i].rows <= 0) continue;
        const Form form = step_form(kSteps[i], f, dt, flags, pl, bl);
        if (form == FORM_DIRECT) {
            const LayerSpec &l = kLayers[kSteps[i].layer];
            ConvDesc d;
            d.kind = l.kind;
            d.cin = lcin(l, f);
            d.cout = lcout(l, f);
            d.in = pl.buf[kSteps[i].src];
            d.out = pl.buf[kSteps[i].dst];
            d.roi_r0 = rois[i].r0;
            d.roi_c0 = rois[i].c0;
            d.roi_rows = rois[i].rows;
            d.roi_cols = rois[i].cols;
            if (!nd_conv_roi_fits(d)) return false;
            continue;
        }
        if (form == FORM_WINO3P) continue;
        if (form == FORM_W1D4 && !(flags & ND_FLAG_W1D_REGS)) continue;
        return false;
    }
    return true;
}

struct StepSrc2 {
    int step = -1;
    QpBuf buf = {};
    int plane0 = 0, from = 0;
    const int *origin = nullptr;
    long origin_max = 0;
    bool addend = false;
};
inline bool form_takes_src2(const Step &st, Form form, int f, int flags, const Plan &pl) {
    if (form == FORM_WINO3P) return kWinoTile == 6;
    return form == FORM_W1D4 && nd_f43_w2d(pl.buf[st.src], lcout(kLayers[st.layer], f), false, flags);
}

struct StackOpts {
    int flags = 0;
    const Roi *rois = nullptr;
    int step_begin = 0, step_end = kNumSteps;
    const StepSrc2 *src2 = nullptr;
    int nsrc2 = 0;
    hipEvent_t *ev = nullptr;
    hipEvent_t *ev_x = nullptr;
    const QpBuf *pre = nullptr;
    const unsigned char *train_w1 = nullptr;
};
int run_stack(int f, int act, int dt, const float *blob, const Plan &pl, hipStream_t s, const StackOpts &o) {
    const QpBuf *const pre = o.pre;
    const int flags = o.flags, step_begin = o.step_begin, step_end = o.step_end;
    const BlobLayout bl = blob_layout(f, dt, pre != nullptr);
    const int cpp = nd_cpp(dt);
    int si = step_begin;
    bool pool_done = false;
    QpBuf pool_view;
    for (int k = step_begin; k < step_end; ++k) {
        const Step &st = kSteps[k];
        if (o.ev) ND_HIP(hipEventRecord(o.ev[si], s));
        const int this_step = si++;
        if (st.layer < 0) {
            if (pool_done) {
                pool_done = false;
                continue;
            }
            ND_TRY(nd_launch_maxpool2(pl.buf[st.src], st.dst_plane0_mul * f / cpp, st.dst_plane0_mul * f / cpp, pl.buf[st.dst], s));
            continue;
        }
        const LayerSpec &l = kLayers[st.layer];
        ConvDesc d;
        d.kind = l.kind;
        d.act = l.prelu >= 0 ? act : ND_ACT_NONE;
        d.slope = 0.25f;
        d.slope_dev = (l.prelu >= 0 && act == ND_ACT_PRELU) ? blob + l.prelu : nullptr;
        if (pre && l.prelu >= 0) {
            d.pre = pre[l.prelu].base;
            d.pre_plane = pre[l.prelu].np();
        }
        const int cin = lcin(l, f);
        d.cin = cin;
        d.cout = lcout(l, f);
        d.wpk = blob + bl.off[st.layer];
        d.bias = d.wpk + nd_bias_offset(l.kind, d.cin, d.cout, dt);
        d.in = pl.buf[st.src];
        d.out = pl.buf[st.dst];
        d.out_plane0 = st.dst_plane0_mul * f / cpp;
        d.part = pl.split;
        d.part_bytes = kSplitScratchBytes;
        d.nosplit = (flags & ND_FLAG_NO_SPLITK) != 0;
        const Form form = step_form(st, f, dt, flags, pl, bl, o.train_w1);
        if (o.rois && o.rois[this_step].rows > 0) {
            d.roi_r0 = o.rois[this_step].r0;
            d.roi_c0 = o.rois[this_step].c0;
            d.roi_rows = o.rois[this_step].rows;
            d.roi_cols = o.rois[this_step].cols;
        }
        for (int i = 0; i < o.nsrc2; ++i)
            if (o.src2[i].step == k && o.src2[i].addend) {
                d.add = o.src2[i].buf;
                d.add_plane0 = o.src2[i].plane0;
                d.add_origin = o.src2[i].origin;
                d.add_origin_max = o.src2[i].origin_max;
                d.w_kb = nd_kblocks(cin, dt);
                d.cin = o.src2[i].from * cpp;
            } else if (o.src2[i].step == k) {
                d.in2 = o.src2[i].buf;
                d.in2_plane0 = o.src2[i].plane0;
                d.in2_from = o.src2[i].from;
                d.in2_origin = o.src2[i].origin;
                d.in2_origin_max = o.src2[i].origin_max;
            }
        const bool next_is_pool = this_step + 1 < step_end && kSteps[this_step + 1].layer < 0;
        const bool w2d = form == FORM_W1D4 && nd_f43_w2d(d.in, d.cout, pre != nullptr, flags);
        if (next_is_pool && !pre && !(flags & ND_FLAG_UNFUSED_POOL)) {
            pool_view = pl.buf[kSteps[this_step + 1].dst];
            d.pool = &pool_view;
            pool_done = w2d || form == FORM_WINO3P || (form == FORM_DIRECT && dt != ND_F32 && nd_conv_pool_fits(d));
            if (!pool_done) d.pool = nullptr;
        }
        if (form == FORM_W1D4 || form == FORM_W1D2) {
            const int T = form == FORM_W1D4 ? kW1dTile : 2;
            if (!pre) d.wpk = blob + (T == kW1dTile ? bl.w1off[st.layer] : bl.w1off2[st.layer]);
            d.bias = d.wpk + nd_bias_offset(d.kind, cin, d.cout, ND_F32, T);
            ND_TRY(form == FORM_W1D4 ? nd_launch_conv_f43(d, flags, s) : nd_launch_conv_w1d(T, d, s));
            continue;
        }
        if (form == FORM_WINO3P) {
            d.wpk = blob + bl.woff[st.layer];
            d.bias = nullptr;
            const int nimg = d.in.B;
            for (int b0 = 0; b0 < nimg; b0 += kWinoChunk) {
                ConvDesc c = d;
                c.in.B = c.out.B = nimg - b0 < kWinoChunk ? nimg - b0 : kWinoChunk;
                c.in.base = d.in.base + (size_t)b0 * d.in.Hb * d.in.Wb * 4;
                c.out.base = d.out.base + (size_t)b0 * d.out.Hb * d.out.Wb * 4;
                QpBuf pv;
                if (d.pool) {
                    pv = *d.pool;
                    pv.B = c.in.B;
                    pv.base = d.pool->base + (size_t)b0 * pv.Hb * pv.Wb * 4;
                    c.pool = &pv;
                }
                if (d.in2_origin) c.in2_origin = d.in2_origin + b0;
                if (d.add_origin) c.add_origin = d.add_origin + b0;
                ND_TRY(nd_launch_conv_wino(kWinoTile, c, pl.wino, pl.wino_bytes, s, (o.ev_x && nimg <= kWinoChunk) ? o.ev_x + 2 * this_step : nullptr));
            }
            continue;
        }
        ND_TRY(nd_launch_conv(d, s));
    }
    if (o.ev) ND_HIP(hipEventRecord(o.ev[si], s));
    return ND_OK;
}

constexpr int kSharedSteps = 6;
constexpr int kStrip = 16;
constexpr double kBandBytes = 8.0 * (1 << 30);

inline int enc_extent(int x, int b) {
    const int p1 = (x - 4) / 2;
    switch (b) {
        case X0: return x;
        case A1: return x - 2;
        case CAT4: return x - 4;
        case P1: return p1;
        case A2: return p1 - 2;
        case CAT3: return p1 - 4;
        default: return (p1 - 4) / 2;
    }
}
Plan make_enc_plan(int f, int hx, int wx, int B, int hcap, int wcap, int cap, char *base, int dt, int slots = 1, Buf slotted = CAT4) {
    Plan p = {};
    size_t off = 0;
    auto add = [&](Buf id, int ch, int pad) {
        QpBuf &q = p.buf[id];
        q.planes = id == X0 ? 2 : (ch + nd_cpp(dt) - 1) / nd_cpp(dt);
        q.dt = dt;
        q.B = B;
        q.Hb = enc_extent(hx, id) + 2 * pad;
        q.Wb = enc_extent(wx, id) + 2 * pad;
        q.pad = pad;
        q.pstride = (long)cap * (enc_extent(hcap, id) + 2 * pad) * (enc_extent(wcap, id) + 2 * pad);
        if ((id == CAT4 || id == CAT3 || id == P2) && id >= slotted) q.pstride *= slots;
        q.base = (float *)(base + off);
        off += ((size_t)q.planes * q.pstride + nd_buf_slack(enc_extent(wcap, id) + 2 * pad)) * 16;
        off = (off + 255) & ~(size_t)255;
    };
    add(X0, 8, 0);
    add(A1, f, 0);
    add(CAT4, 2 * f, 2);
    add(P1, f, 0);
    add(A2, 2 * f, 0);
    add(CAT3, 4 * f, 2);
    add(P2, 2 * f, 0);
    p.split = nullptr;
    p.wino = nullptr;
    p.bytes = off;
    return p;
}

inline long slot_elems(const QpBuf &q, int slots) { return q.pstride / slots; }
inline Plan band_slot(Plan p, int slot, int slots, Buf slotted = CAT4) {
    for (Buf id : {CAT4, CAT3, P2})
        if (id >= slotted) p.buf[id].base += (size_t)slot * slot_elems(p.buf[id], slots) * 4;
    return p;
}

struct FramePlan {
    int D = 0;
    int aligned = 0;
    int S = 0, cols = 0, rows = 0, pad = 0;
    int R = 0, nbands = 0;
    int slots = 1;
    int hx = 0, wx = 0;
    int win4[2] = {0, 0}, win3[2] = {0, 0};
    size_t band_bytes = 0, row_edge_bytes = 0, col_edge_bytes = 0, corner_bytes = 0, origin_bytes = 0, bytes = 0;
    int levels = 0;
    int h2 = 0, w2 = 0;
    int win2[2] = {0, 0};
    size_t l2_band_bytes = 0, l2_row_bytes = 0, l2_col_bytes = 0, l2_corner_bytes = 0, l2_wino_bytes = 0;
    int folds = 0;
    size_t fold_wino_bytes = 0;
};
inline int band_hx(const FramePlan &fp, int nrows, int cs) { return (nrows - 1) * fp.S + cs + 4; }
inline Plan row_edge_plan(const FramePlan &fp, int f, int dt, int nrows, char *base) {
    return make_enc_plan(f, kStrip, fp.wx, 2 * nrows, kStrip, fp.wx, 2 * fp.R, base, dt, fp.slots, P2);
}
inline Plan col_edge_plan(const FramePlan &fp, int f, int dt, int nrows, int cs, char *base) {
    return make_enc_plan(f, band_hx(fp, nrows, cs), kStrip, 2 * fp.cols, fp.hx, kStrip, 2 * fp.cols, base, dt, fp.slots, P2);
}
inline Plan corner_plan(int f, int dt, int ntiles, int cap, char *base) {
    return make_enc_plan(f, kStrip, kStrip, 4 * ntiles, kStrip, kStrip, 4 * cap, base, dt);
}

constexpr int kLevel2End = 9;
constexpr int kStrip2 = 6;

inline int l2_extent(int x, int b) {
    switch (b) {
        case P2: return x;
        case A3: return x - 2;
        case CAT2: return x - 4;
        default: return (x - 4) / 2;
    }
}
Plan make_l2_plan(int f, int h2, int w2, int B, int hcap, int wcap, int cap, char *base, int dt, int slots = 1, Buf slotted = CAT2,
                  bool own_p2 = true) {
    Plan p = {};
    size_t off = 0;
    auto add = [&](Buf id, int ch, int pad) {
        QpBuf &q = p.buf[id];
        q.planes = (ch + nd_cpp(dt) - 1) / nd_cpp(dt);
        q.dt = dt;
        q.B = B;
        q.Hb = l2_extent(h2, id) + 2 * pad;
        q.Wb = l2_extent(w2, id) + 2 * pad;
        q.pad = pad;
        q.pstride = (long)cap * (l2_extent(hcap, id) + 2 * pad) * (l2_extent(wcap, id) + 2 * pad);
        if ((id == CAT2 || id == P3) && id >= slotted) q.pstride *= slots;
        q.base = (float *)(base + off);
        off += ((size_t)q.planes * q.pstride + nd_buf_slack(l2_extent(wcap, id) + 2 * pad)) * 16;
        off = (off + 255) & ~(size_t)255;
    };
    if (own_p2) add(P2, 2 * f, 0);
    add(A3, 4 * f, 0);
    add(CAT2, 8 * f, 2);
    add(P3, 4 * f, 0);
    p.split = nullptr;
    p.wino = nullptr;
    p.bytes = off;
    return p;
}
inline Plan l2_slot(Plan p, int slot, int slots, Buf slotted = CAT2) {
    for (Buf id : {CAT2, P3})
        if (id >= slotted) p.buf[id].base += (size_t)slot * slot_elems(p.buf[id], slots) * 4;
    return p;
}

extern "C" int nd_tile_grid(int W, int H, int cs, int ucs, int ol, int *cols, int *rows, int *pad);

inline int band_h2(const FramePlan &fp, int nrows, int cs) { return enc_extent(band_hx(fp, nrows, cs), P2); }
inline Plan l2_band_plan(const FramePlan &fp, int f, int dt, int nrows, int cs, char *base) {
    return make_l2_plan(f, band_h2(fp, nrows, cs), fp.w2, 1, fp.h2, fp.w2, 1, base, dt, fp.slots, CAT2, false);
}
inline Plan l2_row_plan(const FramePlan &fp, int f, int dt, int nrows, char *base) {
    return make_l2_plan(f, kStrip2, fp.w2, 2 * nrows, kStrip2, fp.w2, 2 * fp.R, base, dt, fp.slots, P3);
}
inline Plan l2_col_plan(const FramePlan &fp, int f, int dt, int nrows, int cs, char *base) {
    return make_l2_plan(f, band_h2(fp, nrows, cs), kStrip2, 2 * fp.cols, fp.h2, kStrip2, 2 * fp.cols, base, dt, fp.slots, P3);
}
inline Plan l2_corner_plan(int f, int dt, int ntiles, int cap, char *base) {
    return make_l2_plan(f, kStrip2, kStrip2, 4 * ntiles, kStrip2, kStrip2, 4 * cap, base, dt);
}

inline void frame_plan_level2(int f, int dt, int flags, int cs, int batch, const BlobLayout &bl, const Roi *rois, FramePlan *fp) {
    fp->levels = fp->D;
    if ((flags & ND_FLAG_TILE_LEVEL2) || fp->S % 8) return;
    const int n2 = enc_extent(cs + 4, P2), n = l2_extent(n2, CAT2);
    if (n2 < kStrip2 + 2 || l2_extent(n2, P3) < 3) return;
    bool reads_cat2 = false;
    for (int i = kLevel2End; i < kNumSteps; ++i) {
        const Step &st = kSteps[i];
        if (st.layer < 0 || st.src != CAT2 || kLayers[st.layer].kind != ND_CONVT3) continue;
        if (rois[i].rows <= 0 || rois[i].r0 != rois[i].c0 || rois[i].rows != rois[i].cols) return;
        fp->win2[0] = rois[i].r0 - 2 < 0 ? 0 : rois[i].r0 - 2;
        fp->win2[1] = rois[i].r0 + rois[i].rows > n ? n : rois[i].r0 + rois[i].rows;
        if (fp->win2[0] < 1 || fp->win2[1] > n - 1 || fp->win2[1] <= fp->win2[0]) return;
        reads_cat2 = true;
    }
    if (!reads_cat2) return;
    fp->h2 = enc_extent(fp->hx, P2);
    fp->w2 = enc_extent(fp->wx, P2);
    Plan plans[4] = {l2_band_plan(*fp, f, dt, fp->R, cs, nullptr), l2_row_plan(*fp, f, dt, fp->R, nullptr),
                     l2_col_plan(*fp, f, dt, fp->R, cs, nullptr), l2_corner_plan(f, dt, batch, batch, nullptr)};
    plans[0].buf[P2] = make_enc_plan(f, fp->hx, fp->wx, 1, fp->hx, fp->wx, 1, nullptr, dt).buf[P2];
    size_t wino = 0;
    for (const Plan &pp : plans)
        for (int i = kSharedSteps; i < kLevel2End; ++i) {
            const Step &st = kSteps[i];
            if (st.layer < 0) continue;
            const LayerSpec &l = kLayers[st.layer];
            const Form form = step_form(st, f, dt, flags, pp, bl);
            if (form == FORM_WINO3P) {
                QpBuf v = pp.buf[st.src];
                v.B = v.B < kWinoChunk ? v.B : kWinoChunk;
                const size_t need = nd_wino_scratch_bytes(kWinoTile, v, lcin(l, f), lcout(l, f));
                wino = need > wino ? need : wino;
            } else if (form != FORM_W1D4 || !nd_f43_w2d(pp.buf[st.src], lcout(l, f), false, flags)) {
                return;
            }
        }
    fp->l2_band_bytes = plans[0].bytes;
    fp->l2_row_bytes = plans[1].bytes;
    fp->l2_col_bytes = plans[2].bytes;
    fp->l2_corner_bytes = plans[3].bytes;
    fp->l2_wino_bytes = (wino + 255) & ~(size_t)255;
    fp->bytes += fp->origin_bytes + fp->l2_band_bytes + fp->l2_row_bytes + fp->l2_col_bytes + fp->l2_corner_bytes + fp->l2_wino_bytes;
    fp->levels = 3;
}

constexpr int kFoldRows = 48;
inline void frame_plan_folds(int f, int dt, int flags, const Plan &tp, const BlobLayout &bl, FramePlan *fp) {
    fp->folds = 0;
    fp->fold_wino_bytes = 0;
    if (!fp->D || (flags & ND_FLAG_TILE_SKIPS)) return;
    const Buf cats[3] = {CAT4, CAT3, CAT2};
    for (int k = 0; k < (fp->levels == 3 ? 3 : 2); ++k)
        for (int i = kSharedSteps; i < kNumSteps; ++i) {
            const Step &st = kSteps[i];
            if (st.layer < 0 || st.src != cats[k] || kLayers[st.layer].kind != ND_CONVT3) continue;
            const Form form = step_form(st, f, dt, flags, tp, bl);
            if (!form_takes_src2(st, form, f, flags, tp)) continue;
            fp->folds |= 1 << k;
            if (form != FORM_WINO3P) continue;
            QpBuf v = {};
            v.B = 1;
            v.Hb = kFoldRows + 2;
            v.Wb = (k == 2 ? l2_extent(fp->w2, CAT2) : enc_extent(fp->wx, cats[k])) + 4;
            const size_t need = nd_wino_scratch_bytes(kWinoTile, v, lcin(kLayers[st.layer], f) / 2, lcout(kLayers[st.layer], f));
            if (need > fp->fold_wino_bytes) fp->fold_wino_bytes = need;
        }
    fp->fold_wino_bytes = (fp->fold_wino_bytes + 255) & ~(size_t)255;
    fp->bytes += fp->fold_wino_bytes;
}
inline int launch_skip_fold(int f, int flags, const float *blob, const BlobLayout &bl, int step, Form form, const QpBuf &cat, int planes,
                            const Roi &roi, int tstep, int nrows, int cols, float *split, char *wino, size_t wino_bytes, hipStream_t s) {
    const LayerSpec &l = kLayers[kSteps[step].layer];
    const int cin = lcin(l, f);
    ConvDesc d;
    d.kind = l.kind;
    d.act = ND_ACT_NONE;
    d.cin = planes * 4;
    d.cout = lcout(l, f);
    d.wpk = blob + bl.w1off[kSteps[step].layer];
    d.bias = d.wpk + nd_bias_offset(l.kind, cin, d.cout, ND_F32, kW1dTile);
    d.w_kb = nd_kblocks(cin);
    d.w_kb0 = planes / 2;
    d.in = cat;
    d.in_plane0 = planes;
    d.out = cat;
    d.out.pad = 1;
    d.out_plane0 = 0;
    d.part = split;
    d.part_bytes = split ? kSplitScratchBytes : 0;
    d.nosplit = (flags & ND_FLAG_NO_SPLITK) != 0;
    d.roi_r0 = roi.r0;
    d.roi_c0 = roi.c0;
    d.roi_rows = (nrows - 1) * tstep + roi.rows;
    d.roi_cols = (cols - 1) * tstep + roi.cols;
    if (form != FORM_WINO3P) return nd_launch_conv_w2d(d, s);
    d.wpk = blob + bl.woff[kSteps[step].layer];
    d.bias = nullptr;
    const int r_end = d.roi_r0 + d.roi_rows;
    for (int r0 = d.roi_r0; r0 < r_end; r0 += kFoldRows) {
        ConvDesc c = d;
        const int rows = r_end - r0 < kFoldRows ? r_end - r0 : kFoldRows;
        c.in.base = c.out.base = cat.base + (size_t)r0 * cat.Wb * 4;
        c.in.Hb = c.out.Hb = rows + 2;
        c.roi_r0 = 0;
        c.roi_rows = rows;
        ND_TRY(nd_launch_conv_wino(kWinoTile, c, wino, wino_bytes, s));
    }
    return ND_OK;
}

int frame_plan(int f, int dt, int flags, int W, int H, int cs, int ucs, int ol, int batch, FramePlan *fp) {
    *fp = FramePlan();
    ND_TRY(check_funit(f, dt));
    if (!valid_cs(cs)) ND_FAIL(ND_EINVAL, "frame plan: tile size %d", cs);
    ND_TRY(nd_tile_grid(W, H, cs, ucs, ol, &fp->cols, &fp->rows, &fp->pad));
    fp->S = ucs - ol;
    fp->aligned = 1;
    while (fp->aligned < 4 && fp->S % (1 << fp->aligned) == 0) ++fp->aligned;
    if (dt != ND_F32 || (flags & (ND_FLAG_FULL_TILES | ND_FLAG_TILE_ENCODER | ND_FLAG_DIRECT_CONV | ND_FLAG_W1D_REGS)) ||
        fp->S % 4 || W < cs || H < cs || batch <= 0)
        return ND_OK;
    const Plan tp = make_plan(f, cs, cs, 1, 1, nullptr, dt);
    const BlobLayout bl = blob_layout(f, dt);
    Roi rois[kNumSteps];
    const int crop = (cs - ucs) / 2;
    if (!plan_rois(tp, crop, crop, rois)) return ND_OK;
    for (int i = 0; i < kNumSteps; ++i) {
        const Step &st = kSteps[i];
        if (st.layer < 0 || (st.src != CAT4 && st.src != CAT3) || kLayers[st.layer].kind != ND_CONVT3) continue;
        const int n = enc_extent(cs + 4, st.src), edge = st.src == CAT4 ? 2 : 1;
        if (rois[i].rows <= 0 || rois[i].r0 != rois[i].c0 || rois[i].rows != rois[i].cols) return ND_OK;
        int *w = st.src == CAT4 ? fp->win4 : fp->win3;
        w[0] = rois[i].r0 - 2 < 0 ? 0 : rois[i].r0 - 2;
        w[1] = rois[i].r0 + rois[i].rows > n ? n : rois[i].r0 + rois[i].rows;
        if (w[0] < edge || w[1] > n - edge) return ND_OK;
    }
    if (fp->win4[1] <= fp->win4[0] || fp->win3[1] <= fp->win3[0]) return ND_OK;
    fp->wx = (fp->cols - 1) * fp->S + cs + 4;
    for (int R = fp->rows; R >= 1; --R) {
        const int hx = band_hx(*fp, R, cs);
        const size_t b = make_enc_plan(f, hx, fp->wx, 1, hx, fp->wx, 1, nullptr, dt).bytes;
        if (b <= kBandBytes || R == 1) {
            fp->R = R;
            fp->hx = hx;
            fp->band_bytes = b;
            break;
        }
    }
    fp->nbands = (fp->rows + fp->R - 1) / fp->R;
    fp->R = (fp->rows + fp->nbands - 1) / fp->nbands;
    fp->hx = band_hx(*fp, fp->R, cs);
    fp->slots = fp->nbands > 1 ? 2 : 1;
    fp->band_bytes = make_enc_plan(f, fp->hx, fp->wx, 1, fp->hx, fp->wx, 1, nullptr, dt, fp->slots).bytes;
    if ((long)fp->hx * fp->wx >= (1L << 26)) return ND_OK;
    const Plan plans[4] = {make_enc_plan(f, fp->hx, fp->wx, 1, fp->hx, fp->wx, 1, nullptr, dt), row_edge_plan(*fp, f, dt, fp->R, nullptr),
                           col_edge_plan(*fp, f, dt, fp->R, cs, nullptr), corner_plan(f, dt, batch, batch, nullptr)};
    for (const Plan &pp : plans)
        for (int i = 0; i < kSharedSteps; ++i) {
            const Step &st = kSteps[i];
            if (st.layer < 0) continue;
            if (step_form(st, f, dt, flags, pp, bl) != FORM_W1D4 || !nd_f43_w2d(pp.buf[st.src], lcout(kLayers[st.layer], f), false, flags))
                return ND_OK;
        }
    fp->row_edge_bytes = plans[1].bytes;
    fp->col_edge_bytes = plans[2].bytes;
    fp->corner_bytes = plans[3].bytes;
    fp->origin_bytes = ((size_t)batch * sizeof(int) + 255) & ~(size_t)255;
    fp->bytes = fp->band_bytes + fp->row_edge_bytes + fp->col_edge_bytes + fp->corner_bytes + 2 * fp->origin_bytes;
    fp->D = 2;
    frame_plan_level2(f, dt, flags, cs, batch, bl, rois, fp);
    frame_plan_folds(f, dt, flags, tp, bl, fp);
    return ND_OK;
}

}
```

### nind_denoise_amd/csrc/winograd.hip

```cpp
#include <stdlib.h>

#include <algorithm>
#include <atomic>
#include <thread>
#include <vector>

#include "nd_common.h"

typedef float f32x4 __attribute__((ext_vector_type(4)));

namespace {

__device__ __forceinline__ void tile_pos(long t, int TX, int TY, int &tx, int &ty, int &b) {
    const unsigned u = (unsigned)t, row = u / (unsigned)TX;
    tx = (int)(u - row * (unsigned)TX);
    b = (int)(row / (unsigned)TY);
    ty = (int)(row - (unsigned)b * (unsigned)TY);
}

template <int T> struct Wino;
template <> struct Wino<2> {
    static constexpr int A = 4;
    template <typename V> __host__ __device__ static void bt(const V *d, V *o) {
        o[0] = d[0] - d[2];
        o[1] = d[1] + d[2];
        o[2] = d[2] - d[1];
        o[3] = d[1] - d[3];
    }
    template <typename V> __host__ __device__ static void at(const V *m, V *o) {
        o[0] = m[0] + m[1] + m[2];
        o[1] = m[1] - m[2] - m[3];
    }
    static void g(const double *w, double *o) {
        o[0] = w[0];
        o[1] = 0.5 * (w[0] + w[1] + w[2]);
        o[2] = 0.5 * (w[0] - w[1] + w[2]);
        o[3] = w[2];
    }
};
template <> struct Wino<4> {
    static constexpr int A = 6;
    template <typename V> __host__ __device__ static void bt(const V *d, V *o) {
        o[0] = 4.f * d[0] - 5.f * d[2] + d[4];
        o[1] = -4.f * (d[1] + d[2]) + d[3] + d[4];
        o[2] = 4.f * (d[1] - d[2]) - d[3] + d[4];
        o[3] = -2.f * d[1] - d[2] + 2.f * d[3] + d[4];
        o[4] = 2.f * d[1] - d[2] - 2.f * d[3] + d[4];
        o[5] = 4.f * d[1] - 5.f * d[3] + d[5];
    }
    template <typename V> __host__ __device__ static void at(const V *m, V *o) {
        o[0] = m[0] + m[1] + m[2] + m[3] + m[4];
        o[1] = m[1] - m[2] + 2.f * (m[3] - m[4]);
        o[2] = m[1] + m[2] + 4.f * (m[3] + m[4]);
        o[3] = m[1] - m[2] + 8.f * (m[3] - m[4]) + m[5];
    }
    static void g(const double *w, double *o) {
        o[0] = w[0] / 4;
        o[1] = -(w[0] + w[1] + w[2]) / 6;
        o[2] = -(w[0] - w[1] + w[2]) / 6;
        o[3] = w[0] / 24 + w[1] / 12 + w[2] / 6;
        o[4] = w[0] / 24 - w[1] / 12 + w[2] / 6;
        o[5] = w[2];
    }
};

template <> struct Wino<6> {
    static constexpr int A = 8;
    template <typename V> __host__ __device__ static void bt(const V *d, V *o) {
        o[0] = d[0] - d[6] + 5.25f * (d[4] - d[2]);
        o[7] = d[7] - d[1] + 5.25f * (d[3] - d[5]);
        V p = d[2] + d[6] - 4.25f * d[4], q = d[1] + d[5] - 4.25f * d[3];
        o[1] = p + q;
        o[2] = p - q;
        p = 0.25f * d[2] - 1.25f * d[4] + d[6];
        q = 0.5f * d[1] - 2.5f * d[3] + 2.f * d[5];
        o[3] = p + q;
        o[4] = p - q;
        p = 4.f * d[2] - 5.f * d[4] + d[6];
        q = 2.f * d[1] - 2.5f * d[3] + 0.5f * d[5];
        o[5] = p + q;
        o[6] = p - q;
    }
    template <typename V> __host__ __device__ static void at(const V *m, V *o) {
        const V s1 = m[1] + m[2], d1 = m[1] - m[2], s2 = m[3] + m[4], d2 = m[3] - m[4], s3 = m[5] + m[6], d3 = m[5] - m[6];
        o[0] = m[0] + s1 + s2 + s3;
        o[1] = d1 + 2.f * d2 + 0.5f * d3;
        o[2] = s1 + 4.f * s2 + 0.25f * s3;
        o[3] = d1 + 8.f * d2 + 0.125f * d3;
        o[4] = s1 + 16.f * s2 + 0.0625f * s3;
        o[5] = d1 + 32.f * d2 + 0.03125f * d3 + m[7];
    }
    static void g(const double *w, double *o) {
        o[0] = w[0];
        o[1] = -2.0 / 9 * (w[0] + w[1] + w[2]);
        o[2] = -2.0 / 9 * (w[0] - w[1] + w[2]);
        o[3] = w[0] / 90 + w[1] / 45 + w[2] * 2 / 45;
        o[4] = w[0] / 90 - w[1] / 45 + w[2] * 2 / 45;
        o[5] = w[0] * 32 / 45 + w[1] * 16 / 45 + w[2] * 8 / 45;
        o[6] = w[0] * 32 / 45 - w[1] * 16 / 45 + w[2] * 8 / 45;
        o[7] = w[2];
    }
};

template <int T>
__global__ __launch_bounds__(256) void k_wino_input(const f32x4 *__restrict__ x, long xnp, int Hb, int Wb, int B, int TY, int TX,
                                                    f32x4 *__restrict__ v, long vnp, long vbs) {
    constexpr int A = Wino<T>::A;
    const long t = (long)blockIdx.x * 256 + threadIdx.x;
    const long tiles = (long)B * TY * TX;
    if (t >= tiles) return;
    const int q = blockIdx.y;
    int tx, ty, b;
    tile_pos(t, TX, TY, tx, ty, b);
    const f32x4 *src = x + (long)q * xnp + ((long)b * Hb + T * ty) * Wb + T * tx;
    const f32x4 zero = {0.f, 0.f, 0.f, 0.f};
    f32x4 d[A][A], r[A][A];
#pragma unroll
    for (int i = 0; i < A; ++i)
#pragma unroll
        for (int j = 0; j < A; ++j) d[i][j] = (T * ty + i < Hb && T * tx + j < Wb) ? src[(long)i * Wb + j] : zero;
#pragma unroll
    for (int j = 0; j < A; ++j) {
        f32x4 c[A], o[A];
#pragma unroll
        for (int i = 0; i < A; ++i) c[i] = d[i][j];
        Wino<T>::bt(c, o);
#pragma unroll
        for (int i = 0; i < A; ++i) r[i][j] = o[i];
    }
    f32x4 *dst = v + (long)q * vnp + t;
#pragma unroll
    for (int i = 0; i < A; ++i) {
        f32x4 o[A];
        Wino<T>::bt(r[i], o);
#pragma unroll
        for (int j = 0; j < A; ++j) dst[(long)(i * A + j) * vbs] = o[j];
    }
}

template <int T>
__global__ __launch_bounds__(128) void k_wino_output(const f32x4 *__restrict__ m, long mnp, long mbs, int B, int TY, int TX, int Hv,
                                                     int Wv, const float *__restrict__ bias, int act, float slope_imm,
                                                     const float *__restrict__ slope_dev, f32x4 *__restrict__ out, long onp,
                                                     int out_plane0, int Ho, int Wo, int opad, f32x4 *__restrict__ pool, long pnp,
                                                     int Hp, int Wp, int ppad) {
    constexpr int A = Wino<T>::A;
    constexpr int NT = 128;
    __shared__ f32x4 sm[T][NT * T];
    const long t0 = (long)blockIdx.x * NT;
    const long t = t0 + threadIdx.x;
    const long tiles = (long)B * TY * TX;
    const int q = blockIdx.y;
    const f32x4 bv = *(const f32x4 *)(bias + 4 * q);
    const float slope = act == ND_ACT_NONE ? 1.f : (slope_dev ? *slope_dev : slope_imm);
    if (t < tiles) {
        const f32x4 *src = m + (long)q * mnp + t;
        f32x4 r[A][T], yv[T][T];
#pragma unroll
        for (int i = 0; i < A; ++i) {
            f32x4 row[A];
#pragma unroll
            for (int j = 0; j < A; ++j) row[j] = src[(long)(i * A + j) * mbs];
            Wino<T>::at(row, r[i]);
        }
#pragma unroll
        for (int j = 0; j < T; ++j) {
            f32x4 c[A], o[T];
#pragma unroll
            for (int i = 0; i < A; ++i) c[i] = r[i][j];
            Wino<T>::at(c, o);
#pragma unroll
            for (int i = 0; i < T; ++i) {
                f32x4 y = o[i] + bv;
#pragma unroll
                for (int e = 0; e < 4; ++e) {
                    const float u = y[e];
                    switch (act) {
                        case ND_ACT_ELU: y[e] = u > 0.f ? u : expm1f(u); break;
                        case ND_ACT_HARDSWISH: y[e] = u * fminf(fmaxf(u + 3.f, 0.f), 6.f) / 6.f; break;
                        default: y[e] = u > 0.f ? u : u * slope; break;
                    }
                }
                sm[i][threadIdx.x * T + j] = y;
                yv[i][j] = y;
            }
        }
        if (pool) {
            int tx, ty, b;
    tile_pos(t, TX, TY, tx, ty, b);
            f32x4 *pd = pool + (long)q * pnp + (long)b * Hp * Wp;
#pragma unroll
            for (int a = 0; a < T / 2; ++a)
#pragma unroll
                for (int c = 0; c < T / 2; ++c) {
                    const int py = ty * (T / 2) + a, px = tx * (T / 2) + c;
                    if (2 * py + 1 < Hv && 2 * px + 1 < Wv) {
                        f32x4 v;
#pragma unroll
                        for (int e = 0; e < 4; ++e)
                            v[e] = fmaxf(fmaxf(yv[2 * a][2 * c][e], yv[2 * a][2 * c + 1][e]), fmaxf(yv[2 * a + 1][2 * c][e], yv[2 * a + 1][2 * c + 1][e]));
                        pd[(long)(py + ppad) * Wp + px + ppad] = v;
                    }
                }
        }
    }
    __syncthreads();
    f32x4 *dst = out + (long)(out_plane0 + q) * onp;
    for (int p = threadIdx.x; p < NT * T; p += NT) {
        const long tt = t0 + p / T;
        if (tt >= tiles) break;
        const int j = p % T;
        int tx, ty, b;
        tile_pos(tt, TX, TY, tx, ty, b);
        const int x = T * tx + j;
        if (x >= Wv) continue;
#pragma unroll
        for (int i = 0; i < T; ++i)
            if (T * ty + i < Hv) dst[((long)b * Ho + T * ty + i + opad) * Wo + x + opad] = sm[i][p];
    }
}

template <int T, int NTL>
__global__ __launch_bounds__(NTL * (T + 2)) void k_wino_in2(const f32x4 *__restrict__ x, long xnp, int Hb, int Wb, long img_stride, int row_stride, int B,
                                                            int TY, int TX, f32x4 *__restrict__ v, long vnp, long vbs, const f32x4 *__restrict__ x2,
                                                            long x2np, int row_stride2, const int *__restrict__ origin2, int q2) {
    constexpr int A = Wino<T>::A, RS = A * A + 1;
    __shared__ f32x4 sm[NTL * RS];
    const long tiles = (long)B * TY * TX;
    const long t0 = (long)blockIdx.x * NTL;
    const int q = blockIdx.y;
    const f32x4 zero = {0.f, 0.f, 0.f, 0.f};
    {
        const int tl = threadIdx.x / A, j = threadIdx.x % A;
        const long t = t0 + tl;
        if (t < tiles) {
            int tx, ty, b;
    tile_pos(t, TX, TY, tx, ty, b);
            const bool s2 = q >= q2;
            const long rs = s2 ? row_stride2 : row_stride;
            const f32x4 *src = (s2 ? x2 + (long)(q - q2) * x2np + origin2[b] : x + (long)q * xnp + (long)b * img_stride) + (long)(T * ty) * rs + T * tx + j;
            f32x4 d[A], o[A];
            const bool okj = T * tx + j < Wb;
#pragma unroll
            for (int i = 0; i < A; ++i) d[i] = (okj && T * ty + i < Hb) ? src[(long)i * rs] : zero;
            Wino<T>::bt(d, o);
#pragma unroll
            for (int i = 0; i < A; ++i) sm[tl * RS + i * A + j] = o[i];
        }
    }
    __syncthreads();
    {
        const int i = threadIdx.x / NTL, tl = threadIdx.x % NTL;
        const long t = t0 + tl;
        if (t < tiles) {
            f32x4 r[A], o[A];
#pragma unroll
            for (int j = 0; j < A; ++j) r[j] = sm[tl * RS + i * A + j];
            Wino<T>::bt(r, o);
            f32x4 *dst = v + (long)q * vnp + t;
#pragma unroll
            for (int j = 0; j < A; ++j) dst[(long)(i * A + j) * vbs] = o[j];
        }
    }
}

template <int T, int NTL, bool ADD = false>
__global__ __launch_bounds__(NTL * (T + 2)) void k_wino_out2(const f32x4 *__restrict__ m, long mnp, long mbs, int B, int TY, int TX, int Hv,
                                                             int Wv, const float *__restrict__ bias, int act, float slope_imm,
                                                             const float *__restrict__ slope_dev, f32x4 *__restrict__ out, long onp,
                                                             int out_plane0, long out_img_stride, int Wo, int opad, f32x4 *__restrict__ pool, long pnp,
                                                             int Hp, int Wp, int ppad, const f32x4 *__restrict__ add = nullptr, long add_np = 0,
                                                             const int *__restrict__ origin_add = nullptr, int W_add = 0) {
    constexpr int A = Wino<T>::A, RS = T * A + 1, NTH = NTL * A;
    __shared__ f32x4 sr[NTL * RS];
    __shared__ f32x4 so[T][NTL * T];
    const long tiles = (long)B * TY * TX;
    const long t0 = (long)blockIdx.x * NTL;
    const int q = blockIdx.y;
    const f32x4 bv = ADD ? f32x4{0.f, 0.f, 0.f, 0.f} : *(const f32x4 *)(bias + 4 * q);
    const float slope = act == ND_ACT_NONE ? 1.f : (slope_dev ? *slope_dev : slope_imm);
    auto activate = [&](f32x4 y) {
#pragma unroll
        for (int e = 0; e < 4; ++e) {
            const float u = y[e];
            switch (act) {
                case ND_ACT_ELU: y[e] = u > 0.f ? u : expm1f(u); break;
                case ND_ACT_HARDSWISH: y[e] = u * fminf(fmaxf(u + 3.f, 0.f), 6.f) / 6.f; break;
                default: y[e] = u > 0.f ? u : u * slope; break;
            }
        }
        return y;
    };
    {
        const int j = threadIdx.x / NTL, tl = threadIdx.x % NTL;
        const long t = t0 + tl;
        if (t < tiles) {
            const f32x4 *src = m + (long)q * mnp + t;
            f32x4 c[A], o[T];
#pragma unroll
            for (int i = 0; i < A; ++i) c[i] = src[(long)(i * A + j) * mbs];
            Wino<T>::at(c, o);
#pragma unroll
            for (int i = 0; i < T; ++i) sr[tl * RS + i * A + j] = o[i];
        }
    }
    __syncthreads();
    if (threadIdx.x < NTL * T) {
        const int i = threadIdx.x / NTL, tl = threadIdx.x % NTL;
        if (t0 + tl < tiles) {
            f32x4 r[A], o[T];
#pragma unroll
            for (int j = 0; j < A; ++j) r[j] = sr[tl * RS + i * A + j];
            Wino<T>::at(r, o);
#pragma unroll
            for (int j = 0; j < T; ++j) {
                so[i][tl * T + j] = ADD ? o[j] : activate(o[j] + bv);
            }
        }
    }
    __syncthreads();
    f32x4 *dst = out + (long)(out_plane0 + q) * onp;
    for (int idx = threadIdx.x; idx < T * NTL * T; idx += NTH) {
        const int i = idx / (NTL * T), pp = idx - i * (NTL * T);
        const long tt = t0 + pp / T;
        if (tt >= tiles) continue;
        int tx, ty, b;
        tile_pos(tt, TX, TY, tx, ty, b);
        const int xx = T * tx + pp % T, yy = T * ty + i;
        if (xx < Wv && yy < Hv) {
            f32x4 y = so[i][pp];
            if constexpr (ADD) y = activate(y + add[(long)q * add_np + (long)origin_add[b] + (long)yy * W_add + xx]);
            dst[(long)b * out_img_stride + (long)(yy + opad) * Wo + xx + opad] = y;
        }
    }
    if (!ADD && pool) {
        f32x4 *pd = pool + (long)q * pnp;
        for (int idx = threadIdx.x; idx < (T / 2) * NTL * (T / 2); idx += NTH) {
            const int a = idx / (NTL * (T / 2)), pp = idx - a * (NTL * (T / 2));
            const int tl = pp / (T / 2), c = pp % (T / 2);
            const long tt = t0 + tl;
            if (tt >= tiles) continue;
            int tx, ty, b;
        tile_pos(tt, TX, TY, tx, ty, b);
            const int px = tx * (T / 2) + c, py = ty * (T / 2) + a;
            if (2 * px + 1 < Wv && 2 * py + 1 < Hv) {
                const f32x4 p00 = so[2 * a][tl * T + 2 * c], p01 = so[2 * a][tl * T + 2 * c + 1];
                const f32x4 p10 = so[2 * a + 1][tl * T + 2 * c], p11 = so[2 * a + 1][tl * T + 2 * c + 1];
                f32x4 v;
#pragma unroll
                for (int e = 0; e < 4; ++e) v[e] = fmaxf(fmaxf(p00[e], p01[e]), fmaxf(p10[e], p11[e]));
                pd[((long)b * Hp + py + ppad) * Wp + px + ppad] = v;
            }
        }
    }
}

constexpr int kOutNtl = 32;
int positions(int T) { return (T + 2) * (T + 2); }
size_t gemm_floats(int cin, int cout) { return nd_packed_floats(ND_CONV1, cin, cout, ND_F32); }

struct WinoGeo {
    int TY, TX, Hv, Wv;
    long tiles;
    long vnp, mnp;
    long vbs, mbs;
    size_t v_bytes, m_bytes;
};
WinoGeo wino_geo(int T, const QpBuf &in, int cin, int cout, int roi_rows = 0, int roi_cols = 0) {
    WinoGeo g;
    g.Hv = roi_rows > 0 ? roi_rows : in.Hb - 2;
    g.Wv = roi_rows > 0 ? roi_cols : in.Wb - 2;
    g.TY = (g.Hv + T - 1) / T;
    g.TX = (g.Wv + T - 1) / T;
    g.tiles = (long)in.B * g.TY * g.TX;
    g.vnp = g.mnp = g.tiles;
    const long slack = 4096;
    g.vbs = (long)(2 * nd_kblocks(cin)) * g.vnp + slack;
    g.mbs = (long)((cout + 3) / 4) * g.mnp + slack;
    g.v_bytes = (size_t)positions(T) * g.vbs * 16;
    g.m_bytes = (size_t)positions(T) * g.mbs * 16;
    return g;
}
}

size_t nd_wino_packed_floats(int T, int cin, int cout) {
    return (size_t)positions(T) * gemm_floats(cin, cout) + (size_t)(cout + 3) / 4 * 4;
}

int nd_wino_pack(int T, int kind, int cin, int cout, const float *w, const float *bias, float *packed) {
    if (T != 2 && T != 4 && T != 6) ND_FAIL(ND_EINVAL, "winograd: tile must be 2, 4 or 6");
    if (kind != ND_CONV3 && kind != ND_CONVT3) ND_FAIL(ND_EINVAL, "winograd: 3x3 layers only");
    const int A = T + 2, P = A * A;
    std::vector<float> u((size_t)P * cout * cin);
    auto parallel_for = [](int n, auto &&fn) {
        const int nt = std::max(1, std::min(n, std::min(16, (int)std::thread::hardware_concurrency())));
        std::atomic<int> next(0);
        std::vector<std::thread> th;
        for (int t = 0; t < nt; ++t)
            th.emplace_back([&] {
                for (int i = next.fetch_add(1); i < n; i = next.fetch_add(1)) fn(i);
            });
        for (auto &x : th) x.join();
    };
    parallel_for(cout, [&](int co) {
        for (int ci = 0; ci < cin; ++ci) {
            double g[3][3], tmp[8][3], U[8][8];
            for (int ky = 0; ky < 3; ++ky)
                for (int kx = 0; kx < 3; ++kx)
                    g[ky][kx] = kind == ND_CONV3 ? w[(((size_t)co * cin + ci) * 3 + ky) * 3 + kx]
                                                 : w[(((size_t)ci * cout + co) * 3 + (2 - ky)) * 3 + (2 - kx)];
            for (int kx = 0; kx < 3; ++kx) {
                double c[3] = {g[0][kx], g[1][kx], g[2][kx]}, o[8];
                if (T == 2) Wino<2>::g(c, o); else if (T == 4) Wino<4>::g(c, o); else Wino<6>::g(c, o);
                for (int i = 0; i < A; ++i) tmp[i][kx] = o[i];
            }
            for (int i = 0; i < A; ++i) {
                double o[8];
                if (T == 2) Wino<2>::g(tmp[i], o); else if (T == 4) Wino<4>::g(tmp[i], o); else Wino<6>::g(tmp[i], o);
                for (int j = 0; j < A; ++j) U[i][j] = o[j];
            }
            for (int i = 0; i < A; ++i)
                for (int j = 0; j < A; ++j) u[((size_t)(i * A + j) * cout + co) * cin + ci] = (float)U[i][j];
        }
    });
    const size_t gf = gemm_floats(cin, cout);
    parallel_for(P, [&](int p) { nd_pack_layer(ND_CONV1, cin, cout, ND_F32, u.data() + (size_t)p * cout * cin, nullptr, packed + p * gf); });
    float *b = packed + (size_t)P * gf;
    for (int co = 0; co < (cout + 3) / 4 * 4; ++co) b[co] = (bias && co < cout) ? bias[co] : 0.f;
    return ND_OK;
}

size_t nd_wino_scratch_bytes(int T, const QpBuf &in, int cin, int cout) {
    const WinoGeo g = wino_geo(T, in, cin, cout);
    return ((g.v_bytes + 255) & ~(size_t)255) + ((g.m_bytes + 255) & ~(size_t)255);
}

void nd_wino_xform_bytes(int T, const QpBuf &in, int cin, int cout, double *bytes_in, double *bytes_out) {
    const WinoGeo g = wino_geo(T, in, cin, cout);
    const double P = positions(T), px_in = (double)in.B * in.Hb * in.Wb, px_out = (double)in.B * g.Hv * g.Wv;
    *bytes_in = 4.0 * cin * px_in + 4.0 * cin * P * (double)g.tiles;
    *bytes_out = 4.0 * cout * P * (double)g.tiles + 4.0 * cout * px_out;
}

int nd_launch_conv_wino(int T, const ConvDesc &d, void *scratch, size_t scratch_bytes, hipStream_t s, hipEvent_t *ev2) {
    if (T != 2 && T != 4 && T != 6) ND_FAIL(ND_EINVAL, "winograd: tile must be 2, 4 or 6");
    if ((d.kind != ND_CONV3 && d.kind != ND_CONVT3) || d.in.dt != ND_F32 || d.out.dt != ND_F32)
        ND_FAIL(ND_EINVAL, "winograd: fp32 3x3 layers only");
    if (d.cin % 16 || d.cout % 4) ND_FAIL(ND_EINVAL, "winograd: Cin must be a multiple of 16, Cout of 4 (got %d, %d)", d.cin, d.cout);
    if (d.pre) ND_FAIL(ND_EINVAL, "winograd: inference only (no pre-activation copy)");
    const bool add = d.add.base != nullptr;
    if ((add || d.w_kb) && T != 6) ND_FAIL(ND_EINVAL, "winograd: only the F(6x6) form takes an addend source or a K-block sub-range");
    if (add && (d.pool || d.in2.base)) ND_FAIL(ND_EINVAL, "winograd: a layer with an addend source is neither pooled nor has a second input source");
    if (d.w_kb && (d.w_kb0 < 0 || d.w_kb0 + nd_kblocks(d.cin) > d.w_kb)) ND_FAIL(ND_EINVAL, "winograd: K blocks [%d,+%d) outside the %d of the packed weights", d.w_kb0, nd_kblocks(d.cin), d.w_kb);
    const int cin_w = d.w_kb ? 8 * d.w_kb : d.cin;
    ND_TRY(nd_check_roi("winograd", d, d.in.Hb - 2, d.in.Wb - 2, T != 6 || d.pool, "a layer other than an unpooled F(6x6) one"));
    const bool roi = d.roi_rows > 0;
    const WinoGeo g = wino_geo(T, d.in, d.cin, d.cout, d.roi_rows, d.roi_cols);
    const bool src2 = d.in2.base != nullptr;
    if (src2) {
        if (T != 6) ND_FAIL(ND_EINVAL, "winograd: only the F(6x6) form has a second input source");
        ND_TRY(nd_check_in2("winograd", d, nd_kblocks(d.cin), (long)(d.roi_r0 + g.Hv + 1) * d.in2.Wb + d.roi_c0 + g.Wv + 2));
    }
    if (add) ND_TRY(nd_check_add("winograd", d, (long)(d.roi_r0 + g.Hv - 1 + d.add.pad) * d.add.Wb + d.roi_c0 + g.Wv - 1 + d.add.pad + 1));
    ND_TRY(nd_check_out("winograd", d, d.in.Hb - 2, d.in.Wb - 2, false));
    const long roi_in = roi ? (long)d.roi_r0 * d.in.Wb + d.roi_c0 : 0, roi_out = roi ? (long)d.roi_r0 * d.out.Wb + d.roi_c0 : 0;
    const int vHb = g.Hv + 2, vWb = g.Wv + 2;
    const size_t need = nd_wino_scratch_bytes(T, d.in, d.cin, d.cout);
    if (!scratch || scratch_bytes < need) ND_FAIL(ND_ENOMEM, "winograd: scratch %zu B given, %zu B needed", scratch_bytes, need);
    if (g.tiles >= (1L << 31)) ND_FAIL(ND_EINVAL, "winograd: %ld tiles exceed the 32-bit tile index", g.tiles);
    const int P = positions(T);
    f32x4 *v = (f32x4 *)scratch;
    f32x4 *m = (f32x4 *)((char *)scratch + ((g.v_bytes + 255) & ~(size_t)255));
    const int in_planes = 2 * nd_kblocks(d.cin), out_planes = d.cout / 4;
    const f32x4 *x = (const f32x4 *)d.in.base + (long)d.in_plane0 * d.in.np() + roi_in;
    dim3 gi((unsigned)((g.tiles + 255) / 256), in_planes);
    constexpr int kNtl = 16;
    dim3 gi2((unsigned)((g.tiles + kNtl - 1) / kNtl), in_planes);
    if (T == 2)
        hipLaunchKernelGGL(k_wino_input<2>, gi, dim3(256), 0, s, x, d.in.np(), d.in.Hb, d.in.Wb, d.in.B, g.TY, g.TX, v, g.vnp, g.vbs);
    else if (T == 6)
        hipLaunchKernelGGL((k_wino_in2<6, kNtl>), gi2, dim3(kNtl * 8), 0, s, x, d.in.np(), vHb, vWb, (long)d.in.Hb * d.in.Wb, d.in.Wb, d.in.B, g.TY, g.TX, v, g.vnp, g.vbs,
                           src2 ? (const f32x4 *)d.in2.base + (long)d.in2_plane0 * d.in2.np() + (roi ? (long)d.roi_r0 * d.in2.Wb + d.roi_c0 : 0) : nullptr,
                           d.in2.np(), d.in2.Wb, d.in2_origin, src2 ? d.in2_from : in_planes);
    else
        hipLaunchKernelGGL(k_wino_input<4>, gi, dim3(256), 0, s, x, d.in.np(), d.in.Hb, d.in.Wb, d.in.B, g.TY, g.TX, v, g.vnp, g.vbs);
    ND_HIP(hipGetLastError());
    if (ev2) ND_HIP(hipEventRecord(ev2[0], s));

    ConvDesc e;
    e.kind = ND_CONV1;
    e.cin = d.cin;
    e.cout = d.cout;
    e.wpk = d.wpk;
    e.bias = d.wpk + nd_bias_offset(ND_CONV1, cin_w, d.cout);
    e.w_kb = d.w_kb;
    e.w_kb0 = d.w_kb0;
    e.in = {(float *)v, in_planes, d.in.B, g.TY, g.TX, 0, g.vnp, ND_F32};
    e.out = {(float *)m, out_planes, d.in.B, g.TY, g.TX, 0, g.mnp, ND_F32};
    e.variant = nd_conv_variant_gemm(d.cin, d.cout);
    e.part = d.part;
    e.part_bytes = d.part_bytes;
    e.nosplit = d.nosplit;
    e.nbatch = P;
    e.in_bs = g.vbs;
    e.out_bs = g.mbs;
    e.w_bs = gemm_floats(cin_w, d.cout);
    ND_TRY(nd_launch_conv(e, s));
    if (ev2) ND_HIP(hipEventRecord(ev2[1], s));

    const float *bias = d.wpk + (size_t)P * gemm_floats(cin_w, d.cout);
    dim3 go((unsigned)((g.tiles + 127) / 128), out_planes);
    f32x4 *out = (f32x4 *)d.out.base + roi_out;
    f32x4 *pool = nullptr;
    long pnp = 0;
    int Hp = 0, Wp = 0, ppad = 0;
    if (d.pool) {
        const QpBuf &q = *d.pool;
        if (q.dt != ND_F32 || q.B != d.in.B || q.Hb - 2 * q.pad != g.Hv / 2 || q.Wb - 2 * q.pad != g.Wv / 2 || q.planes < out_planes)
            ND_FAIL(ND_EINVAL, "winograd: pooled destination does not fit %dx%dx%d", d.cout, g.Hv / 2, g.Wv / 2);
        pool = (f32x4 *)q.base;
        pnp = q.np();
        Hp = q.Hb;
        Wp = q.Wb;
        ppad = q.pad;
    }
    if (add) {
        const f32x4 *ap = (const f32x4 *)d.add.base + (long)d.add_plane0 * d.add.np() + (long)((roi ? d.roi_r0 : 0) + d.add.pad) * d.add.Wb +
                          (roi ? d.roi_c0 : 0) + d.add.pad;
        dim3 go2((unsigned)((g.tiles + 31) / 32), out_planes);
        hipLaunchKernelGGL((k_wino_out2<6, 32, true>), go2, dim3(256), 0, s, (const f32x4 *)m, g.mnp, g.mbs, d.in.B, g.TY, g.TX, g.Hv, g.Wv, bias,
                           d.act, d.slope, d.slope_dev, out, d.out.np(), d.out_plane0, (long)d.out.Hb * d.out.Wb, d.out.Wb, d.out.pad, nullptr, 0L, 0, 0, 0,
                           ap, d.add.np(), d.add_origin, d.add.Wb);
    } else if (T == 6 && kOutNtl == 16) {
        dim3 go2((unsigned)((g.tiles + 15) / 16), out_planes);
        hipLaunchKernelGGL((k_wino_out2<6, 16>), go2, dim3(128), 0, s, (const f32x4 *)m, g.mnp, g.mbs, d.in.B, g.TY, g.TX, g.Hv, g.Wv, bias,
                           d.act, d.slope, d.slope_dev, out, d.out.np(), d.out_plane0, (long)d.out.Hb * d.out.Wb, d.out.Wb, d.out.pad, pool, pnp, Hp, Wp, ppad);
    } else if (T == 6) {
        dim3 go2((unsigned)((g.tiles + 31) / 32), out_planes);
        hipLaunchKernelGGL((k_wino_out2<6, 32>), go2, dim3(256), 0, s, (const f32x4 *)m, g.mnp, g.mbs, d.in.B, g.TY, g.TX, g.Hv, g.Wv, bias,
                           d.act, d.slope, d.slope_dev, out, d.out.np(), d.out_plane0, (long)d.out.Hb * d.out.Wb, d.out.Wb, d.out.pad, pool, pnp, Hp, Wp, ppad);
    }
    else if (T == 2)
        hipLaunchKernelGGL(k_wino_output<2>, go, dim3(128), 0, s, (const f32x4 *)m, g.mnp, g.mbs, d.in.B, g.TY, g.TX, g.Hv, g.Wv, bias,
                           d.act, d.slope, d.slope_dev, out, d.out.np(), d.out_plane0, d.out.Hb, d.out.Wb, d.out.pad, pool, pnp, Hp, Wp, ppad);
    else
        hipLaunchKernelGGL(k_wino_output<4>, go, dim3(128), 0, s, (const f32x4 *)m, g.mnp, g.mbs, d.in.B, g.TY, g.TX, g.Hv, g.Wv, bias,
                           d.act, d.slope, d.slope_dev, out, d.out.np(), d.out_plane0, d.out.Hb, d.out.Wb, d.out.pad, pool, pnp, Hp, Wp, ppad);
    ND_HIP(hipGetLastError());
    return ND_OK;
}
```

### nind_denoise_amd/networks/UtNet.py

```python
import ctypes

import torch
from torch import nn

from .. import _lib
from ..synth import utnet_layer_table, utnet_prelu_keys

_ACTIVATIONS = {"PReLU": nn.PReLU, "ELU": nn.ELU, "Hardswish": nn.Hardswish}
_SHORT_DTYPE = {_lib.ND_F32: "f32", _lib.ND_BF16: "bf16", _lib.ND_F16: "f16"}


def canonical_compute_dtype(name):
    if name not in _lib.DTYPE:
        raise ValueError(f"unknown compute dtype {name!r}; choose one of {', '.join(_lib.DTYPE)}")
    return _SHORT_DTYPE[_lib.DTYPE[name]]


def valid_cs(cs):
    return cs >= 104 and (cs - 56) % 16 == 0


def nearest_valid_cs(cs):
    k = (cs - 56 + 8) // 16
    return max(104, 16 * k + 56)


class _TrainState:

    def __init__(self, model, device):
        lib = _lib.load()
        self.device = device
        n = lib.nd_utnet_param_count(model.funit)
        if n == 0:
            raise ValueError(f"UtNet: funit={model.funit} is not supported by the HIP training path (multiple of 8)")
        self.flat = torch.zeros(n, dtype=torch.float32, device=device)
        self.grads = torch.zeros(n, dtype=torch.float32, device=device)
        self.blobs = torch.empty(lib.nd_utnet_train_blob_bytes(model.funit), dtype=torch.uint8, device=device)
        self.ranges = {}
        for i, name in enumerate(_lib.utnet_tensor_names()):
            off, cnt = ctypes.c_size_t(), ctypes.c_size_t()
            _lib.check(lib.nd_utnet_param_range(model.funit, i, off, cnt))
            self.ranges[name] = (off.value, cnt.value)
        self.ws, self.ws_key = None, None
        self.generation = 0

    def workspace(self, model, h, w, batch):
        if self.ws_key != (h, w, batch):
            lib = _lib.load()
            nbytes = lib.nd_utnet_train_workspace_bytes_hw(model.funit, h, w, batch)
            if nbytes == 0:
                _lib.check(lib.nd_utnet_train_workspace_init_hw(None, 0, model.funit, h, w, batch, None), "UtNet training")
            self.ws = None
            self.ws = torch.empty(nbytes, dtype=torch.uint8, device=self.device)
            _lib.check(lib.nd_utnet_train_workspace_init_hw(self.ws.data_ptr(), nbytes, model.funit, h, w, batch,
                                                            _lib.stream_ptr(self.device)), "nd_utnet_train_workspace_init_hw")
            self.ws_key = (h, w, batch)
        return self.ws


class _UtNetFunction(torch.autograd.Function):

    @staticmethod
    def forward(ctx, model, names, x, *params):
        st = model._train_state(x.device)
        with torch.no_grad():
            for n, p in zip(names, params):
                off, cnt = st.ranges[n]
                st.flat[off:off + cnt].copy_(p.detach().reshape(-1))
        batch, h, w = x.size(0), x.size(2), x.size(3)
        y = torch.empty_like(x)
        with torch.cuda.device(x.device):
            ws = st.workspace(model, h, w, batch)
            _lib.check(_lib.load().nd_utnet_train_forward_hw(model.funit, _lib.ACT[model.activation], model.flags,
                                                             st.flat.data_ptr(), st.blobs.data_ptr(), x.data_ptr(), y.data_ptr(),
                                                             batch, h, w, ws.data_ptr(), ws.numel(), _lib.stream_ptr(x.device)),
                       "nd_utnet_train_forward_hw")
        st.generation += 1
        ctx.model, ctx.names, ctx.geom, ctx.generation = model, names, (batch, h, w), st.generation
        ctx.shapes = [p.shape for p in params]
        return y

    @staticmethod
    def backward(ctx, gy):
        model = ctx.model
        st = model._train_state(gy.device)
        if st.generation != ctx.generation:
            raise RuntimeError("UtNet backward: another forward of this module ran under autograd since this graph was built; its "
                               "activations are gone (one forward/backward in flight per module -- as the reference's training loop runs)")
        batch, h, w = ctx.geom
        want_dx, want_p = ctx.needs_input_grad[2], ctx.needs_input_grad[3:]
        gy = gy.to(torch.float32).contiguous()
        dx = torch.empty(batch, 3, h, w, dtype=torch.float32, device=gy.device) if want_dx else None
        with torch.cuda.device(gy.device):
            _lib.check(_lib.load().nd_utnet_train_backward_hw(model.funit, _lib.ACT[model.activation], model.flags,
                                                              st.flat.data_ptr(), st.grads.data_ptr() if any(want_p) else None,
                                                              st.blobs.data_ptr(), gy.data_ptr(), dx.data_ptr() if want_dx else None,
                                                              batch, h, w, st.ws.data_ptr(), st.ws.numel(), _lib.stream_ptr(gy.device),
                                                              None, 0), "nd_utnet_train_backward_hw")
        grads = []
        for n, shape, want in zip(ctx.names, ctx.shapes, want_p):
            off, cnt = st.ranges[n]
            grads.append(st.grads[off:off + cnt].view(shape).clone() if want else None)
        return (None, None, dx) + tuple(grads)


class UtNet(nn.Module):
    split_k = True
    winograd = True
    w1d_regs = False
    useful_only = True
    fused_pool = True
    share_encoder = True
    share_level2 = True
    fold_skips = True

    def __init__(self, funit=64, activation='PReLU', compute_dtype='f32'):
        super().__init__()
        funit = int(funit)
        compute_dtype = canonical_compute_dtype(compute_dtype)
        if activation not in _ACTIVATIONS:
            exit(f'UtNet: unknown activation function: {activation}')
        self.funit, self.activation = funit, activation
        groups = {}
        for key, kind, cin, cout, k in utnet_layer_table(funit):
            if kind == "conv":
                layer = nn.Conv2d(cin, cout, k)
            elif kind == "convT":
                layer = nn.ConvTranspose2d(cin, cout, k)
            else:
                layer = nn.ConvTranspose2d(cin, cout, k, stride=2)
            if "." in key:
                seq, idx = key.split(".")
                groups.setdefault(seq, {})[int(idx)] = layer
            else:
                groups[key] = layer
        for key in utnet_prelu_keys():
            seq, idx = key.split(".")
            groups[seq][int(idx)] = _ACTIVATIONS[activation]()
        order = ["convs1", "convs2", "convs3", "convs4", "bottom"]
        for n in range(1, 5):
            order += [f"up{n}", f"tconvs{n}"]
        for name in order:
            g = groups[name]
            self.add_module(name, nn.Sequential(*[g[i] for i in sorted(g)]) if isinstance(g, dict) else g)
        self._packed = {}
        self.pack_on_device = True
        self._workspaces = {}
        self.max_cached_workspaces = 2
        self.compute_dtype = compute_dtype
        self.weights_generation = 0

    def set_compute_dtype(self, name):
        self.compute_dtype = canonical_compute_dtype(name)
        return self

    @property
    def _dt(self):
        return _lib.DTYPE[self.compute_dtype]

    @property
    def flags(self):
        return ((0 if self.split_k else _lib.FLAG_NO_SPLITK) | (0 if self.winograd else _lib.FLAG_DIRECT_CONV) |
                (_lib.FLAG_W1D_REGS if self.w1d_regs else 0) | (0 if self.useful_only else _lib.FLAG_FULL_TILES) |
                (0 if self.fused_pool else _lib.FLAG_UNFUSED_POOL) | (0 if self.share_encoder else _lib.FLAG_TILE_ENCODER))

    @property
    def frame_flags(self):
        return self.flags | (0 if self.share_level2 else _lib.FLAG_TILE_LEVEL2) | (0 if self.fold_skips else _lib.FLAG_TILE_SKIPS)

    def _weights_key(self, device):
        return (str(device), self.weights_generation) + tuple((p.data_ptr(), p._version) for p in self.parameters())

    def packed_weights(self, device):
        key = self._weights_key(device)
        hit = self._packed.get(self.compute_dtype)
        if hit is not None and hit[0] == key:
            return hit[1]
        lib = _lib.load()
        sd = self.state_dict()
        names = _lib.utnet_tensor_names()
        nbytes = lib.nd_utnet_packed_bytes(self.funit, self._dt)
        if nbytes == 0:
            raise ValueError(f"UtNet: funit={self.funit} is not supported by the HIP path for {self.compute_dtype} "
                             "(multiple of 8 for f32, of 16 for bf16 / f16)")
        on_device = self.pack_on_device
        where = device if on_device else "cpu"
        keep = []
        ptrs = (ctypes.c_void_p * len(names))()
        for i, n in enumerate(names):
            if n in sd:
                t = sd[n].detach().to(device=where, dtype=torch.float32).contiguous()
                keep.append(t)
                ptrs[i] = t.data_ptr()
            else:
                ptrs[i] = None
        if on_device:
            dev_blob = torch.empty(nbytes // 4, dtype=torch.float32, device=device)
            with torch.cuda.device(device):
                _lib.check(lib.nd_utnet_pack_weights_device(self.funit, self._dt, ptrs, len(names), dev_blob.data_ptr(), nbytes,
                                                            _lib.stream_ptr(device)), "nd_utnet_pack_weights_device")
                torch.cuda.current_stream(device).synchronize()
        else:
            blob = torch.empty(nbytes // 4, dtype=torch.float32)
            _lib.check(lib.nd_utnet_pack_weights(self.funit, self._dt, ptrs, len(names), blob.data_ptr(), nbytes),
                       "nd_utnet_pack_weights")
            dev_blob = blob.to(device)
        self._packed[self.compute_dtype] = (key, dev_blob)
        return dev_blob

    def workspace(self, cs, batch, device, width=None):
        h, w = int(cs), int(cs if width is None else width)
        key = (str(device), h, w, int(batch), self.compute_dtype)
        ws = self._workspaces.get(key)
        if ws is None:
            lib = _lib.load()
            nbytes = lib.nd_utnet_workspace_bytes_hw(self.funit, h, w, batch, self._dt)
            if nbytes == 0:
                _lib.check(lib.nd_utnet_workspace_init_hw(None, 0, self.funit, h, w, batch, self._dt, None), "UtNet")
            while len(self._workspaces) >= self.max_cached_workspaces:
                self._workspaces.pop(next(iter(self._workspaces)))
            ws = torch.empty(nbytes, dtype=torch.uint8, device=device)
            _lib.check(lib.nd_utnet_workspace_init_hw(ws.data_ptr(), nbytes, self.funit, h, w, batch, self._dt,
                                                      _lib.stream_ptr(device)), "nd_utnet_workspace_init_hw")
            self._workspaces[key] = ws
        return ws

    def frame_workspace(self, width, height, cs, ucs, ol, batch, device):
        lib = _lib.load()
        nbytes = lib.nd_utnet_frame_workspace_bytes(self.funit, self._dt, self.frame_flags, width, height, cs, ucs, ol, batch)
        if nbytes == 0:
            return None
        key = (str(device), "frame", nbytes)
        ws = self._workspaces.get(key)
        if ws is None:
            for k in [k for k in self._workspaces if k[1] == "frame"]:
                del self._workspaces[k]
            ws = torch.zeros(nbytes, dtype=torch.uint8, device=device)
            self._workspaces[key] = ws
        return ws

    def forward(self, l):
        if l.device.type != "cuda":
            raise RuntimeError("nind_denoise_amd.UtNet runs on the MI355X HIP path only (no CPU fallback); "
                               "move the module and its input to the GPU")
        if l.dim() != 4 or l.size(1) != 3:
            raise ValueError(f"UtNet expects [B,3,H,W], got {tuple(l.shape)}")
        batch, h, w = l.size(0), l.size(2), l.size(3)
        for cs in (h, w):
            if not valid_cs(cs):
                raise ValueError(f"UtNet: tile size {cs} is not of the form 16k+56 (e.g. {nearest_valid_cs(cs)}); "
                                 "the reference network fails on it too")
        trainable = self.training and any(p.requires_grad for p in self.parameters())
        if torch.is_grad_enabled() and (trainable or (l.requires_grad and self.compute_dtype == "f32")):
            if self.compute_dtype != "f32":
                raise NotImplementedError("UtNet under autograd runs in fp32 (the training step's arithmetic)")
            named = [(n, p) for n, p in self.named_parameters()]
            return _UtNetFunction.apply(self, tuple(n for n, _ in named), l.to(torch.float32).contiguous(),
                                        *[p for _, p in named])
        x = l.detach().to(torch.float32).contiguous()
        lib = _lib.load()
        with torch.cuda.device(x.device):
            blob = self.packed_weights(x.device)
            ws = self.workspace(h, batch, x.device, width=w)
            y = torch.empty_like(x)
            _lib.check(lib.nd_utnet_forward_hw(self.funit, _lib.ACT[self.activation], self._dt, self.flags, blob.data_ptr(),
                                               x.data_ptr(), y.data_ptr(), batch, h, w, ws.data_ptr(), ws.numel(),
                                               _lib.stream_ptr(x.device)), "nd_utnet_forward_hw")
        return y

    def _train_state(self, device):
        st = getattr(self, "_tstate", None)
        if st is None or st.device != device:
            st = self._tstate = _TrainState(self, device)
        return st

    def flops_per_tile(self, cs):
        return _lib.load().nd_utnet_flops(self.funit, cs)
```

Before: 87.28 MP/s.

## Pack batch images into a mosaic for Winograd F(6x6) transposed-conv tiling

For unpooled, single-source ConvT3 layers run as Winograd F(6x6), the batch of small images is laid out as a virtual bx-by-by mosaic at the image pitch. Winograd tiles then span image boundaries, which removes the per-image partial-tile waste when the image side is not a multiple of 6. The input and output transform kernels gain a MOSAIC path that maps each tile back to its image and drops out-of-range pixels. The mosaic is used only when it saves at least 10% of tiles. Tile accounting for profiling now records the launched tile count, and a new flag turns the mosaic off.

```diff
diff --git a/include/nind_hip.h b/include/nind_hip.h
--- a/include/nind_hip.h
+++ b/include/nind_hip.h
@@ -45,6 +45,7 @@
     ND_FLAG_TILE_LEVEL2 = 64,
     ND_FLAG_FIND_NOISE = 128,
     ND_FLAG_TILE_SKIPS = 256,
+    ND_FLAG_TILE_WINO = 512,
     ND_FLAG_FULL_TILES = 8
 } nd_flags;
 
@@ -181,6 +182,8 @@
 int nd_ssim_padded_grad(const float *x, const float *y, int n, int c, int h, int w, int window, const float *gout, float *gx,
                         void *workspace, size_t workspace_bytes, void *stream);
 
+int nd_wino_mosaic(int p, int B, int *bx, int *by, long *tiles, long *tiles_per_image);
+
 size_t nd_winograd_packed_bytes(int tile, int cin, int cout);
 int nd_winograd_pack(int tile, int kind, int cin, int cout, const float *w, const float *bias, void *packed,
                      size_t packed_bytes);
@@ -194,6 +197,8 @@
 
 int nd_winograd_bench(int tile, int kind, int batch, int cin, int cout, int h, int w, int iters, void *workspace,
                       size_t workspace_bytes, void *stream, float *mean_ms);
+int nd_winograd_bench_flags(int tile, int kind, int batch, int cin, int cout, int h, int w, int iters, int flags, void *workspace,
+                            size_t workspace_bytes, void *stream, float *mean_ms);
 
 int nd_num_conv_variants(void);
 const char *nd_conv_variant_name(int variant);
diff --git a/nind_denoise_amd/_lib.py b/nind_denoise_amd/_lib.py
--- a/nind_denoise_amd/_lib.py
+++ b/nind_denoise_amd/_lib.py
@@ -1,6 +1,6 @@
 import ctypes
 import os
-from ctypes import POINTER, c_char_p, c_double, c_float, c_int, c_size_t, c_void_p
+from ctypes import POINTER, c_char_p, c_double, c_float, c_int, c_long, c_size_t, c_void_p
 
 _HERE = os.path.dirname(os.path.abspath(__file__))
 LIB_PATH = os.path.join(_HERE, "libnind_hip.so")
@@ -12,6 +12,7 @@
 FLAG_NO_SPLITK, FLAG_DIRECT_CONV, FLAG_W1D_REGS, FLAG_FULL_TILES, FLAG_UNFUSED_POOL, FLAG_TILE_ENCODER, FLAG_TILE_LEVEL2 = 1, 2, 4, 8, 16, 32, 64
 FLAG_FIND_NOISE = 128
 FLAG_TILE_SKIPS = 256
+FLAG_TILE_WINO = 512
 PROGRESS_FN = ctypes.CFUNCTYPE(None, c_void_p, c_int, c_int, c_int)
 
 
@@ -111,6 +112,8 @@
     "nd_mse": (c_int, [c_void_p, c_void_p, c_size_t, c_void_p, c_void_p, c_size_t, c_void_p]),
     "nd_conv_bench": (c_int, [c_int] * 9 + [c_void_p, c_size_t, c_void_p, POINTER(c_float)]),
     "nd_winograd_bench": (c_int, [c_int] * 8 + [c_void_p, c_size_t, c_void_p, POINTER(c_float)]),
+    "nd_winograd_bench_flags": (c_int, [c_int] * 9 + [c_void_p, c_size_t, c_void_p, POINTER(c_float)]),
+    "nd_wino_mosaic": (c_int, [c_int, c_int, POINTER(c_int), POINTER(c_int), POINTER(c_long), POINTER(c_long)]),
     "nd_num_conv_variants": (c_int, []),
     "nd_conv_variant_name": (c_char_p, [c_int]),
 }
diff --git a/nind_denoise_amd/csrc/nd_common.h b/nind_denoise_amd/csrc/nd_common.h
--- a/nind_denoise_amd/csrc/nd_common.h
+++ b/nind_denoise_amd/csrc/nd_common.h
@@ -54,6 +54,7 @@
     float *part = nullptr;
     size_t part_bytes = 0;
     bool nosplit = false;
+    bool tile_wino = false;
     int nbatch = 1;
     long in_bs = 0, out_bs = 0;
     size_t w_bs = 0;
@@ -81,7 +82,8 @@
 int nd_wino_pack(int T, int kind, int cin, int cout, const float *w, const float *bias, float *packed);
 size_t nd_wino_scratch_bytes(int T, const QpBuf &in, int cin, int cout);
 int nd_launch_conv_wino(int T, const ConvDesc &d, void *scratch, size_t scratch_bytes, hipStream_t s, hipEvent_t *ev2 = nullptr);
-void nd_wino_xform_bytes(int T, const QpBuf &in, int cin, int cout, double *bytes_in, double *bytes_out);
+long nd_wino_launch_tiles(int T, const ConvDesc &d);
+void nd_wino_xform_bytes(int T, const QpBuf &in, int cin, int cout, long tiles, double *bytes_in, double *bytes_out);
 size_t nd_w1d_packed_floats(int T, int cin, int cout);
 int nd_w1d_pack(int T, int kind, int cin, int cout, const float *w, const float *bias, float *packed);
 bool nd_w1d_fits(int T, const QpBuf &in);
@@ -101,7 +103,7 @@
 int nd_check_roi(const char *who, const ConvDesc &d, int Hv, int Wv, bool refused, const char *why);
 static inline int nd_check_flags(int flags, bool frame_loop = false, bool unet_frame = false) {
     const int known = ND_FLAG_NO_SPLITK | ND_FLAG_DIRECT_CONV | ND_FLAG_W1D_REGS | ND_FLAG_FULL_TILES | ND_FLAG_UNFUSED_POOL |
-                      ND_FLAG_TILE_ENCODER | (frame_loop ? ND_FLAG_TILE_LEVEL2 | ND_FLAG_TILE_SKIPS : 0) | (unet_frame ? ND_FLAG_FIND_NOISE : 0);
+                      ND_FLAG_TILE_ENCODER | ND_FLAG_TILE_WINO | (frame_loop ? ND_FLAG_TILE_LEVEL2 | ND_FLAG_TILE_SKIPS : 0) | (unet_frame ? ND_FLAG_FIND_NOISE : 0);
     if (flags & ~known) ND_FAIL(ND_EINVAL, "unknown flag bits 0x%x", flags);
     return ND_OK;
 }
diff --git a/nind_denoise_amd/csrc/pack.hip b/nind_denoise_amd/csrc/pack.hip
--- a/nind_denoise_amd/csrc/pack.hip
+++ b/nind_denoise_amd/csrc/pack.hip
@@ -12,7 +12,7 @@
 }
 
 extern "C" const char *nd_last_error(void) { return g_err; }
-extern "C" int nd_version(void) { return 111; }
+extern "C" int nd_version(void) { return 112; }
 
 static inline uint16_t f32_to_bf16_rne(float f) {
     uint32_t u;
diff --git a/nind_denoise_amd/csrc/utnet.hip b/nind_denoise_amd/csrc/utnet.hip
--- a/nind_denoise_amd/csrc/utnet.hip
+++ b/nind_denoise_amd/csrc/utnet.hip
@@ -455,6 +455,8 @@
     opts.flags = flags;
     opts.ev = ev;
     opts.ev_x = evx;
+    long tiles_run[kNumSteps] = {};
+    opts.wino_tiles = tiles_run;
     if (!(flags & ND_FLAG_FULL_TILES) && plan_rois(pl, crop, crop, rois) && rois_supported(funit, dtype, flags, pl, bl, rois)) opts.rois = rois;
     int rc = run_stack(funit, act, dtype, (const float *)packed, pl, s, opts);
     if (rc == ND_OK) {
@@ -502,10 +504,15 @@
         o.flops *= B;
         o.bytes = B * esz * (ci * hin * win + co * hout * wout) + 4.0 * ci * co * nd_taps(l.kind);
         auto cdiv = [](double a, double b) { return (double)(long)((a + b - 1) / b); };
+        long wino_tiles = 0;
         switch (form) {
             case FORM_W1D4: o.mfma_flops = 2.0 * 3 * 6 * cip * co * hout * cdiv(wout, 4) * B; break;
             case FORM_W1D2: o.mfma_flops = 2.0 * 3 * 4 * cip * co * hout * cdiv(wout, 2) * B; break;
-            case FORM_WINO3P: o.mfma_flops = 2.0 * (kWinoTile + 2) * (kWinoTile + 2) * cip * co * cdiv(hout, kWinoTile) * cdiv(wout, kWinoTile) * B; break;
+            case FORM_WINO3P: {
+                wino_tiles = tiles_run[i];
+                o.mfma_flops = 2.0 * (kWinoTile + 2) * (kWinoTile + 2) * cip * co * (double)wino_tiles;
+                break;
+            }
             default:
                 o.mfma_flops = l.kind == ND_CONVT2S2 ? 2.0 * 4 * cip * co * hin * win * B
                                                      : 2.0 * nd_taps(l.kind) * cip * co * hout * wout * B;
@@ -524,7 +531,7 @@
                 v.Hb = opts.rois[i].rows + 2;
                 v.Wb = opts.rois[i].cols + 2;
             }
-            nd_wino_xform_bytes(kWinoTile, v, (int)ci, (int)co, &o.xform_bytes_in, &o.xform_bytes_out);
+            nd_wino_xform_bytes(kWinoTile, v, (int)ci, (int)co, wino_tiles, &o.xform_bytes_in, &o.xform_bytes_out);
         }
     }
     return rc;
@@ -665,6 +672,7 @@
     d.slope = slope;
     d.variant = variant;
     d.nosplit = (flags & ND_FLAG_NO_SPLITK) != 0;
+    d.tile_wino = (flags & ND_FLAG_TILE_WINO) != 0;
     ND_TRY(launch_form(fm, d, (char *)ws + pl.bytes, ws_bytes - pl.bytes, s));
     return nd_launch_qp_to_nchw(pl.out, 0, y, cout, s);
 }
@@ -824,6 +832,11 @@
 
 extern "C" int nd_winograd_bench(int tile, int kind, int batch, int cin, int cout, int h, int w, int iters, void *ws,
                                  size_t ws_bytes, void *stream, float *mean_ms) {
+    return nd_winograd_bench_flags(tile, kind, batch, cin, cout, h, w, iters, 0, ws, ws_bytes, stream, mean_ms);
+}
+extern "C" int nd_winograd_bench_flags(int tile, int kind, int batch, int cin, int cout, int h, int w, int iters, int flags, void *ws,
+                                       size_t ws_bytes, void *stream, float *mean_ms) {
+    ND_TRY(nd_check_flags(flags));
     const size_t need = nd_layer_winograd_workspace_bytes(tile, kind, batch, cin, cout, h, w);
     if (!need) ND_FAIL(ND_EINVAL, "nd_winograd_bench: bad shape / kind / tile");
     const LayerForm fm = wino_form(tile);
@@ -837,5 +850,7 @@
     ConvDesc d = layer_desc(fm, kind, cin, cout, ND_F32, wpk, pl);
     d.act = ND_ACT_PRELU;
     d.slope = 0.2f;
+    d.nosplit = (flags & ND_FLAG_NO_SPLITK) != 0;
+    d.tile_wino = (flags & ND_FLAG_TILE_WINO) != 0;
     return time_form("nd_winograd_bench", fm, d, (char *)ws + pl.bytes, need - pl.bytes, iters, s, mean_ms);
 }
diff --git a/nind_denoise_amd/csrc/utnet_net.h b/nind_denoise_amd/csrc/utnet_net.h
--- a/nind_denoise_amd/csrc/utnet_net.h
+++ b/nind_denoise_amd/csrc/utnet_net.h
@@ -350,6 +350,7 @@
     int nsrc2 = 0;
     hipEvent_t *ev = nullptr;
     hipEvent_t *ev_x = nullptr;
+    long *wino_tiles = nullptr;
     const QpBuf *pre = nullptr;
     const unsigned char *train_w1 = nullptr;
 };
@@ -394,6 +395,7 @@
         d.part = pl.split;
         d.part_bytes = kSplitScratchBytes;
         d.nosplit = (flags & ND_FLAG_NO_SPLITK) != 0;
+        d.tile_wino = (flags & ND_FLAG_TILE_WINO) != 0;
         const Form form = step_form(st, f, dt, flags, pl, bl, o.train_w1);
         if (o.rois && o.rois[this_step].rows > 0) {
             d.roi_r0 = o.rois[this_step].r0;
@@ -450,6 +452,7 @@
                 if (d.in2_origin) c.in2_origin = d.in2_origin + b0;
                 if (d.add_origin) c.add_origin = d.add_origin + b0;
                 ND_TRY(nd_launch_conv_wino(kWinoTile, c, pl.wino, pl.wino_bytes, s, (o.ev_x && nimg <= kWinoChunk) ? o.ev_x + 2 * this_step : nullptr));
+                if (o.wino_tiles) o.wino_tiles[this_step] += nd_wino_launch_tiles(kWinoTile, c);
             }
             continue;
         }
diff --git a/nind_denoise_amd/csrc/winograd.hip b/nind_denoise_amd/csrc/winograd.hip
--- a/nind_denoise_amd/csrc/winograd.hip
+++ b/nind_denoise_amd/csrc/winograd.hip
@@ -220,13 +220,14 @@
     }
 }
 
-template <int T, int NTL>
+template <int T, int NTL, bool MOSAIC = false>
 __global__ __launch_bounds__(NTL * (T + 2)) void k_wino_in2(const f32x4 *__restrict__ x, long xnp, int Hb, int Wb, long img_stride, int row_stride, int B,
                                                             int TY, int TX, f32x4 *__restrict__ v, long vnp, long vbs, const f32x4 *__restrict__ x2,
-                                                            long x2np, int row_stride2, const int *__restrict__ origin2, int q2) {
+                                                            long x2np, int row_stride2, const int *__restrict__ origin2, int q2, int mp = 0,
+                                                            int mbx = 0, int mby = 0) {
     constexpr int A = Wino<T>::A, RS = A * A + 1;
     __shared__ f32x4 sm[NTL * RS];
-    const long tiles = (long)B * TY * TX;
+    const long tiles = MOSAIC ? (long)TY * TX : (long)B * TY * TX;
     const long t0 = (long)blockIdx.x * NTL;
     const int q = blockIdx.y;
     const f32x4 zero = {0.f, 0.f, 0.f, 0.f};
@@ -236,6 +237,21 @@
         if (t < tiles) {
             int tx, ty, b;
     tile_pos(t, TX, TY, tx, ty, b);
+            if constexpr (MOSAIC) {
+                const unsigned X = (unsigned)(T * tx + j), cx = X / (unsigned)mp, Y = (unsigned)(T * ty), cy = Y / (unsigned)mp;
+                const int lx = (int)(X - cx * (unsigned)mp), ly = (int)(Y - cy * (unsigned)mp);
+                const f32x4 *src = x + (long)q * xnp + lx;
+                f32x4 d[A], o[A];
+#pragma unroll
+                for (int i = 0; i < A; ++i) {
+                    const bool wrap = ly + i >= mp;
+                    const int cyi = (int)cy + (wrap ? 1 : 0), lyi = ly + i - (wrap ? mp : 0), bi = cyi * mbx + (int)cx;
+                    d[i] = ((int)cx < mbx && cyi < mby && bi < B) ? src[(long)bi * img_stride + (long)lyi * row_stride] : zero;
+                }
+                Wino<T>::bt(d, o);
+#pragma unroll
+                for (int i = 0; i < A; ++i) sm[tl * RS + i * A + j] = o[i];
+            } else {
             const bool s2 = q >= q2;
             const long rs = s2 ? row_stride2 : row_stride;
             const f32x4 *src = (s2 ? x2 + (long)(q - q2) * x2np + origin2[b] : x + (long)q * xnp + (long)b * img_stride) + (long)(T * ty) * rs + T * tx + j;
@@ -246,6 +262,7 @@
             Wino<T>::bt(d, o);
 #pragma unroll
             for (int i = 0; i < A; ++i) sm[tl * RS + i * A + j] = o[i];
+            }
         }
     }
     __syncthreads();
@@ -264,17 +281,19 @@
     }
 }
 
-template <int T, int NTL, bool ADD = false>
+template <int T, int NTL, bool ADD = false, bool MOSAIC = false>
 __global__ __launch_bounds__(NTL * (T + 2)) void k_wino_out2(const f32x4 *__restrict__ m, long mnp, long mbs, int B, int TY, int TX, int Hv,
                                                              int Wv, const float *__restrict__ bias, int act, float slope_imm,
                                                              const float *__restrict__ slope_dev, f32x4 *__restrict__ out, long onp,
                                                              int out_plane0, long out_img_stride, int Wo, int opad, f32x4 *__restrict__ pool, long pnp,
                                                              int Hp, int Wp, int ppad, const f32x4 *__restrict__ add = nullptr, long add_np = 0,
-                                                             const int *__restrict__ origin_add = nullptr, int W_add = 0) {
+                                                             const int *__restrict__ origin_add = nullptr, int W_add = 0, int mp = 0,
+                                                             int mbx = 0, int mby = 0) {
+    static_assert(!(MOSAIC && ADD), "the mosaic form has no addend");
     constexpr int A = Wino<T>::A, RS = T * A + 1, NTH = NTL * A;
     __shared__ f32x4 sr[NTL * RS];
     __shared__ f32x4 so[T][NTL * T];
-    const long tiles = (long)B * TY * TX;
+    const long tiles = MOSAIC ? (long)TY * TX : (long)B * TY * TX;
     const long t0 = (long)blockIdx.x * NTL;
     const int q = blockIdx.y;
     const f32x4 bv = ADD ? f32x4{0.f, 0.f, 0.f, 0.f} : *(const f32x4 *)(bias + 4 * q);
@@ -327,13 +346,17 @@
         int tx, ty, b;
         tile_pos(tt, TX, TY, tx, ty, b);
         const int xx = T * tx + pp % T, yy = T * ty + i;
-        if (xx < Wv && yy < Hv) {
+        if constexpr (MOSAIC) {
+            const unsigned cx = (unsigned)xx / (unsigned)mp, cy = (unsigned)yy / (unsigned)mp;
+            const int lx = xx - (int)cx * mp, ly = yy - (int)cy * mp, bi = (int)cy * mbx + (int)cx;
+            if ((int)cx < mbx && (int)cy < mby && bi < B) dst[(long)bi * out_img_stride + (long)(ly + opad) * Wo + lx + opad] = so[i][pp];
+        } else if (xx < Wv && yy < Hv) {
             f32x4 y = so[i][pp];
             if constexpr (ADD) y = activate(y + add[(long)q * add_np + (long)origin_add[b] + (long)yy * W_add + xx]);
             dst[(long)b * out_img_stride + (long)(yy + opad) * Wo + xx + opad] = y;
         }
     }
-    if (!ADD && pool) {
+    if (!ADD && !MOSAIC && pool) {
         f32x4 *pd = pool + (long)q * pnp;
         for (int idx = threadIdx.x; idx < (T / 2) * NTL * (T / 2); idx += NTH) {
             const int a = idx / (NTL * (T / 2)), pp = idx - a * (NTL * (T / 2));
@@ -361,11 +384,20 @@
 
 struct WinoGeo {
     int TY, TX, Hv, Wv;
+    int mp = 0, mbx = 0, mby = 0;
     long tiles;
     long vnp, mnp;
     long vbs, mbs;
     size_t v_bytes, m_bytes;
 };
+void wino_strides(int T, int cin, int cout, WinoGeo &g) {
+    g.vnp = g.mnp = g.tiles;
+    const long slack = 4096;
+    g.vbs = (long)(2 * nd_kblocks(cin)) * g.vnp + slack;
+    g.mbs = (long)((cout + 3) / 4) * g.mnp + slack;
+    g.v_bytes = (size_t)positions(T) * g.vbs * 16;
+    g.m_bytes = (size_t)positions(T) * g.mbs * 16;
+}
 WinoGeo wino_geo(int T, const QpBuf &in, int cin, int cout, int roi_rows = 0, int roi_cols = 0) {
     WinoGeo g;
     g.Hv = roi_rows > 0 ? roi_rows : in.Hb - 2;
@@ -373,12 +405,28 @@
     g.TY = (g.Hv + T - 1) / T;
     g.TX = (g.Wv + T - 1) / T;
     g.tiles = (long)in.B * g.TY * g.TX;
-    g.vnp = g.mnp = g.tiles;
-    const long slack = 4096;
-    g.vbs = (long)(2 * nd_kblocks(cin)) * g.vnp + slack;
-    g.mbs = (long)((cout + 3) / 4) * g.mnp + slack;
-    g.v_bytes = (size_t)positions(T) * g.vbs * 16;
-    g.m_bytes = (size_t)positions(T) * g.mbs * 16;
+    wino_strides(T, cin, cout, g);
+    return g;
+}
+bool wino_mosaic_rule(int T, const ConvDesc &d, int *bx, int *by, long *tiles) {
+    if (T != 6 || d.kind != ND_CONVT3 || d.tile_wino || d.nosplit || d.roi_rows > 0 || d.pool || d.in2.base || d.add.base || d.pre) return false;
+    if (d.in.Hb != d.in.Wb) return false;
+    if (d.in.pad != 2) return false;
+    long per_image;
+    return nd_wino_mosaic(d.in.Hb - 2, d.in.B, bx, by, tiles, &per_image) == 1;
+}
+WinoGeo wino_geo_launch(int T, const ConvDesc &d) {
+    WinoGeo g = wino_geo(T, d.in, d.cin, d.cout, d.roi_rows, d.roi_cols);
+    int bx, by;
+    long tiles;
+    if (!wino_mosaic_rule(T, d, &bx, &by, &tiles)) return g;
+    g.mp = g.Hv;
+    g.mbx = bx;
+    g.mby = by;
+    g.TY = (by * g.mp + T - 1) / T;
+    g.TX = (bx * g.mp + T - 1) / T;
+    g.tiles = tiles;
+    wino_strides(T, d.cin, d.cout, g);
     return g;
 }
 }
@@ -430,13 +478,45 @@
     return ND_OK;
 }
 
+extern "C" int nd_wino_mosaic(int p, int B, int *bx, int *by, long *tiles, long *tiles_per_image) {
+    if (p <= 0 || B <= 0 || !bx || !by || !tiles || !tiles_per_image) ND_FAIL(ND_EINVAL, "nd_wino_mosaic: bad arguments");
+    const long T = 6, per = (long)B * ((p + T - 1) / T) * ((p + T - 1) / T);
+    *tiles_per_image = *tiles = per;
+    *bx = *by = 0;
+    if (p < 8 || B < 2) return 0;
+    auto count = [&](int x) { return (((long)x * p + T - 1) / T) * (((long)((B + x - 1) / x) * p + T - 1) / T); };
+    long fewest = count(1);
+    for (int x = 2; x <= B; ++x) fewest = std::min(fewest, count(x));
+    long best = -1;
+    int best_x = 0, best_y = 0, best_skew = 0;
+    for (int x = B; x >= 1; --x) {
+        const int y = (B + x - 1) / x, skew = x > y ? x - y : y - x;
+        const long n = count(x);
+        if (n * 100 > fewest * 101) continue;
+        if (best < 0 || skew < best_skew || (skew == best_skew && n < best)) {
+            best = n;
+            best_x = x;
+            best_y = y;
+            best_skew = skew;
+        }
+    }
+    if (best * 10 > per * 9) return 0;
+    *bx = best_x;
+    *by = best_y;
+    *tiles = best;
+    return 1;
+}
+
 size_t nd_wino_scratch_bytes(int T, const QpBuf &in, int cin, int cout) {
     const WinoGeo g = wino_geo(T, in, cin, cout);
     return ((g.v_bytes + 255) & ~(size_t)255) + ((g.m_bytes + 255) & ~(size_t)255);
 }
 
-void nd_wino_xform_bytes(int T, const QpBuf &in, int cin, int cout, double *bytes_in, double *bytes_out) {
-    const WinoGeo g = wino_geo(T, in, cin, cout);
+long nd_wino_launch_tiles(int T, const ConvDesc &d) { return wino_geo_launch(T, d).tiles; }
+
+void nd_wino_xform_bytes(int T, const QpBuf &in, int cin, int cout, long tiles, double *bytes_in, double *bytes_out) {
+    WinoGeo g = wino_geo(T, in, cin, cout);
+    if (tiles > 0) g.tiles = tiles;
     const double P = positions(T), px_in = (double)in.B * in.Hb * in.Wb, px_out = (double)in.B * g.Hv * g.Wv;
     *bytes_in = 4.0 * cin * px_in + 4.0 * cin * P * (double)g.tiles;
     *bytes_out = 4.0 * cout * P * (double)g.tiles + 4.0 * cout * px_out;
@@ -455,7 +535,9 @@
     const int cin_w = d.w_kb ? 8 * d.w_kb : d.cin;
     ND_TRY(nd_check_roi("winograd", d, d.in.Hb - 2, d.in.Wb - 2, T != 6 || d.pool, "a layer other than an unpooled F(6x6) one"));
     const bool roi = d.roi_rows > 0;
-    const WinoGeo g = wino_geo(T, d.in, d.cin, d.cout, d.roi_rows, d.roi_cols);
+    const WinoGeo g = wino_geo_launch(T, d);
+    const bool mosaic = g.mp > 0;
+    const int gB = mosaic ? 1 : d.in.B;
     const bool src2 = d.in2.base != nullptr;
     if (src2) {
         if (T != 6) ND_FAIL(ND_EINVAL, "winograd: only the F(6x6) form has a second input source");
@@ -467,6 +549,11 @@
     const int vHb = g.Hv + 2, vWb = g.Wv + 2;
     const size_t need = nd_wino_scratch_bytes(T, d.in, d.cin, d.cout);
     if (!scratch || scratch_bytes < need) ND_FAIL(ND_ENOMEM, "winograd: scratch %zu B given, %zu B needed", scratch_bytes, need);
+    if (mosaic) {
+        const size_t mneed = ((g.v_bytes + 255) & ~(size_t)255) + ((g.m_bytes + 255) & ~(size_t)255);
+        if (g.mp < 8 || g.mp != d.in.Wb - 2 || (long)g.mbx * g.mby < d.in.B || (long)g.TY * g.TX != g.tiles || mneed > need)
+            ND_FAIL(ND_EINVAL, "winograd: mosaic %d x %d at pitch %d does not fit %d images / the scratch bound", g.mbx, g.mby, g.mp, d.in.B);
+    }
     if (g.tiles >= (1L << 31)) ND_FAIL(ND_EINVAL, "winograd: %ld tiles exceed the 32-bit tile index", g.tiles);
     const int P = positions(T);
     f32x4 *v = (f32x4 *)scratch;
@@ -478,6 +565,9 @@
     dim3 gi2((unsigned)((g.tiles + kNtl - 1) / kNtl), in_planes);
     if (T == 2)
         hipLaunchKernelGGL(k_wino_input<2>, gi, dim3(256), 0, s, x, d.in.np(), d.in.Hb, d.in.Wb, d.in.B, g.TY, g.TX, v, g.vnp, g.vbs);
+    else if (mosaic)
+        hipLaunchKernelGGL((k_wino_in2<6, kNtl, true>), gi2, dim3(kNtl * 8), 0, s, x, d.in.np(), vHb, vWb, (long)d.in.Hb * d.in.Wb, d.in.Wb, d.in.B, g.TY, g.TX, v, g.vnp,
+                           g.vbs, nullptr, 0L, 0, nullptr, in_planes, g.mp, g.mbx, g.mby);
     else if (T == 6)
         hipLaunchKernelGGL((k_wino_in2<6, kNtl>), gi2, dim3(kNtl * 8), 0, s, x, d.in.np(), vHb, vWb, (long)d.in.Hb * d.in.Wb, d.in.Wb, d.in.B, g.TY, g.TX, v, g.vnp, g.vbs,
                            src2 ? (const f32x4 *)d.in2.base + (long)d.in2_plane0 * d.in2.np() + (roi ? (long)d.roi_r0 * d.in2.Wb + d.roi_c0 : 0) : nullptr,
@@ -495,8 +585,8 @@
     e.bias = d.wpk + nd_bias_offset(ND_CONV1, cin_w, d.cout);
     e.w_kb = d.w_kb;
     e.w_kb0 = d.w_kb0;
-    e.in = {(float *)v, in_planes, d.in.B, g.TY, g.TX, 0, g.vnp, ND_F32};
-    e.out = {(float *)m, out_planes, d.in.B, g.TY, g.TX, 0, g.mnp, ND_F32};
+    e.in = {(float *)v, in_planes, gB, g.TY, g.TX, 0, g.vnp, ND_F32};
+    e.out = {(float *)m, out_planes, gB, g.TY, g.TX, 0, g.mnp, ND_F32};
     e.variant = nd_conv_variant_gemm(d.cin, d.cout);
     e.part = d.part;
     e.part_bytes = d.part_bytes;
@@ -531,6 +621,11 @@
         hipLaunchKernelGGL((k_wino_out2<6, 32, true>), go2, dim3(256), 0, s, (const f32x4 *)m, g.mnp, g.mbs, d.in.B, g.TY, g.TX, g.Hv, g.Wv, bias,
                            d.act, d.slope, d.slope_dev, out, d.out.np(), d.out_plane0, (long)d.out.Hb * d.out.Wb, d.out.Wb, d.out.pad, nullptr, 0L, 0, 0, 0,
                            ap, d.add.np(), d.add_origin, d.add.Wb);
+    } else if (mosaic) {
+        dim3 go2((unsigned)((g.tiles + 31) / 32), out_planes);
+        hipLaunchKernelGGL((k_wino_out2<6, 32, false, true>), go2, dim3(256), 0, s, (const f32x4 *)m, g.mnp, g.mbs, d.in.B, g.TY, g.TX, g.Hv, g.Wv, bias,
+                           d.act, d.slope, d.slope_dev, out, d.out.np(), d.out_plane0, (long)d.out.Hb * d.out.Wb, d.out.Wb, d.out.pad, nullptr, 0L, 0, 0, 0,
+                           nullptr, 0L, nullptr, 0, g.mp, g.mbx, g.mby);
     } else if (T == 6 && kOutNtl == 16) {
         dim3 go2((unsigned)((g.tiles + 15) / 16), out_planes);
         hipLaunchKernelGGL((k_wino_out2<6, 16>), go2, dim3(128), 0, s, (const f32x4 *)m, g.mnp, g.mbs, d.in.B, g.TY, g.TX, g.Hv, g.Wv, bias,
diff --git a/nind_denoise_amd/networks/UtNet.py b/nind_denoise_amd/networks/UtNet.py
--- a/nind_denoise_amd/networks/UtNet.py
+++ b/nind_denoise_amd/networks/UtNet.py
@@ -106,6 +106,7 @@
 
 class UtNet(nn.Module):
     split_k = True
+    mosaic_wino = True
     winograd = True
     w1d_regs = False
     useful_only = True
@@ -162,7 +163,8 @@
     def flags(self):
         return ((0 if self.split_k else _lib.FLAG_NO_SPLITK) | (0 if self.winograd else _lib.FLAG_DIRECT_CONV) |
                 (_lib.FLAG_W1D_REGS if self.w1d_regs else 0) | (0 if self.useful_only else _lib.FLAG_FULL_TILES) |
-                (0 if self.fused_pool else _lib.FLAG_UNFUSED_POOL) | (0 if self.share_encoder else _lib.FLAG_TILE_ENCODER))
+                (0 if self.fused_pool else _lib.FLAG_UNFUSED_POOL) | (0 if self.share_encoder else _lib.FLAG_TILE_ENCODER) |
+                (0 if self.mosaic_wino else _lib.FLAG_TILE_WINO))
 
     @property
     def frame_flags(self):
```

Measured after the change: 89.85 MP/s, median of 6. +2.9%, better.
